# HansiZeng/scaling-retriever

Hardware: AMD Instinct MI355X
Metric: MSMARCO-Dev queries/sec end-to-end (query encode + dense brute-force top-1000) (higher is better)
Workload: dtype f32

## Files before the change

include/sr_hip.h:

```cpp
#ifndef SR_HIP_H
#define SR_HIP_H
#include <stdint.h>
#ifdef __cplusplus
extern "C" {
#endif

#define SR_OK 0
#define SR_ERR_INVALID 1
#define SR_ERR_HIP 2
#define SR_ERR_NOMEM 3
#define SR_ERR_UNSUPPORTED 4

#define SR_DTYPE_F32 0
#define SR_DTYPE_BF16 1
#define SR_DTYPE_F16 2

typedef void* sr_stream;

const char* sr_last_error(void);
int sr_version(void);
int sr_max_topk(void);

typedef struct sr_dense_index sr_dense_index;

int sr_dense_index_create(sr_dense_index** out, int dim);
int sr_dense_index_add(sr_dense_index* idx, const float* d_rows, int64_t n_rows,
                       int64_t id_base, int64_t id_stride);
int sr_dense_index_add_f16(sr_dense_index* idx, const void* d_rows_f16, int64_t n_rows,
                           int64_t id_base, int64_t id_stride);
int sr_dense_index_row_dtype(const sr_dense_index* idx);
int sr_dense_index_owned_bytes(sr_dense_index* idx, int64_t* out);
int64_t sr_dense_index_ntotal(const sr_dense_index* idx);
int sr_dense_search(sr_dense_index* idx, const float* d_queries, int64_t nq, int k,
                    float* d_out_scores, int64_t* d_out_ids, sr_stream stream);
#define SR_PRECISION_FP32 0
#define SR_PRECISION_BF16X3 1
#define SR_PRECISION_BF16X6 2
#define SR_PRECISION_FP32_FILTERED 3
int sr_dense_index_set_precision(sr_dense_index* idx, int mode);
int sr_dense_search_begin(sr_dense_index* idx, const float* d_queries, int64_t nq, int k, int share,
                          float* d_lower, sr_stream stream);
int sr_dense_search_finish(sr_dense_index* idx, const float* d_queries, int64_t nq, int k, const float* d_threshold,
                           float* d_out_scores, int64_t* d_out_ids, sr_stream stream);
int sr_dense_index_filter_stats(sr_dense_index* idx, int64_t* n_filtered, int64_t* n_fallback);
int sr_dense_index_filter_query_stats(sr_dense_index* idx, int64_t* n_certified, int64_t* n_redone);
int sr_dense_index_set_workspace_limit(sr_dense_index* idx, int64_t bytes);
int sr_dense_index_set_batch_invariant(sr_dense_index* idx, int on);
int sr_dense_score_pairs(sr_dense_index* idx, const float* d_queries, int64_t nq, const int64_t* d_cand_indptr,
                         const int64_t* d_cand_ids, float* d_out_scores, sr_stream stream);
int sr_dense_search_subset(sr_dense_index* idx, const float* d_queries, int64_t nq, int k,
                           const int64_t* d_subset, int64_t m,
                           float* d_out_scores, int64_t* d_out_ids, sr_stream stream);
int64_t sr_dense_index_id_end(const sr_dense_index* idx);
int sr_doc_mask_from_list(const int64_t* d_list, int64_t m, uint32_t* d_words, int64_t n_bits, sr_stream stream);
int sr_doc_list_from_mask(const uint32_t* d_words, int64_t n_bits, int64_t* d_list, int64_t capacity,
                          int64_t* d_count, sr_stream stream);
int sr_dense_search_masked(sr_dense_index* idx, const float* d_queries, int64_t nq, int k,
                           const uint32_t* d_mask_words, int64_t n_bits,
                           float* d_out_scores, int64_t* d_out_ids, sr_stream stream);
int sr_dense_range_count(sr_dense_index* idx, const float* d_queries, int64_t nq, const float* d_thresholds,
                         int64_t* d_lims, int64_t* total, sr_stream stream);
int sr_dense_range_fill(sr_dense_index* idx, const float* d_queries, int64_t nq, const float* d_thresholds,
                        const int64_t* d_lims, float* d_out_scores, int64_t* d_out_ids, int64_t capacity, sr_stream stream);
int sr_dense_index_destroy(sr_dense_index* idx);
int sr_dense_index_profile(sr_dense_index* idx, int enable);
int sr_dense_index_profile_read(sr_dense_index* idx, int64_t* n_launches, double* total_ms,
                                double* total_flop, double* total_d_bytes);

typedef struct sr_sparse_index sr_sparse_index;

int sr_sparse_index_create(sr_sparse_index** out, const int64_t* d_indptr,
                           const int32_t* d_doc_ids, const float* d_vals,
                           int64_t n_terms, int64_t n_docs, sr_stream stream);
int sr_sparse_search(sr_sparse_index* idx, const int64_t* d_q_indptr, const int32_t* d_q_cols,
                     const float* d_q_vals, int64_t nq, int k, float threshold,
                     int64_t id_base, int64_t id_stride,
                     float* d_out_scores, int64_t* d_out_ids, int32_t* d_out_counts,
                     sr_stream stream);
int sr_sparse_index_set_workspace_limit(sr_sparse_index* idx, int64_t bytes);
int sr_sparse_score_pairs(sr_sparse_index* idx, const int64_t* d_q_indptr, const int32_t* d_q_cols, const float* d_q_vals,
                          int64_t nq, const int64_t* d_cand_indptr, const int64_t* d_cand_ids, float* d_out_scores,
                          sr_stream stream);
int sr_sparse_search_subset(sr_sparse_index* idx, const int64_t* d_q_indptr, const int32_t* d_q_cols,
                            const float* d_q_vals, int64_t nq, int k, float threshold,
                            const int64_t* d_subset, int64_t m, int64_t id_base, int64_t id_stride,
                            float* d_out_scores, int64_t* d_out_ids, int32_t* d_out_counts, sr_stream stream);
int sr_sparse_search_masked(sr_sparse_index* idx, const int64_t* d_q_indptr, const int32_t* d_q_cols,
                            const float* d_q_vals, int64_t nq, int k, float threshold,
                            const uint32_t* d_mask_words, int64_t n_bits, int64_t id_base, int64_t id_stride,
                            float* d_out_scores, int64_t* d_out_ids, int32_t* d_out_counts, sr_stream stream);
int sr_sparse_range_count(sr_sparse_index* idx, const int64_t* d_q_indptr, const int32_t* d_q_cols, const float* d_q_vals,
                          int64_t nq, const float* d_thresholds, int64_t* d_lims, int64_t* total, sr_stream stream);
int sr_sparse_range_fill(sr_sparse_index* idx, const int64_t* d_q_indptr, const int32_t* d_q_cols, const float* d_q_vals,
                         int64_t nq, const float* d_thresholds, const int64_t* d_lims, int64_t id_base, int64_t id_stride,
                         float* d_out_scores, int64_t* d_out_ids, int64_t capacity, sr_stream stream);
int sr_sparse_index_destroy(sr_sparse_index* idx);
int sr_sparse_index_work_counters(sr_sparse_index* idx, int enable, uint64_t* out6);
int sr_sparse_index_profile(sr_sparse_index* idx, int enable);
int sr_sparse_index_profile_read(sr_sparse_index* idx, int64_t* n_launches, double* total_ms,
                                 double* total_posting_bytes);
int sr_sparse_index_block_stats(sr_sparse_index* idx, int64_t* n_dense_terms, int64_t* n_block_calls,
                                int64_t* n_fallback_calls);

int sr_sparse_index_cert_stats(sr_sparse_index* idx, int64_t* out8);
int sr_sparse_index_cert_debug(sr_sparse_index* idx, int enable, uint16_t* h_keys, int64_t keys_capacity,
                               float* h_consts, int64_t nq_pad, float* vscale, int32_t* T);

int sr_sparse_csr_expand_terms(const int64_t* d_indptr, int64_t n_terms, int64_t nnz, int32_t* d_out_terms,
                               sr_stream stream);
int sr_sparse_csr_build(const int32_t* d_rows, const int32_t* d_cols, const float* d_vals, int64_t nnz,
                        int64_t n_terms, int64_t n_docs, int sort_docs, int64_t* d_indptr,
                        int32_t* d_out_rows, float* d_out_vals, sr_stream stream);

int sr_topk_merge(const float* d_scores, const int64_t* d_ids, int n_lists, int64_t nq, int k,
                  float pad_score, float* d_out_scores, int64_t* d_out_ids, sr_stream stream);

typedef struct sr_model sr_model;

typedef struct {
    int32_t vocab_size, hidden_size, intermediate_size, num_layers;
    int32_t num_heads, num_kv_heads, head_dim;
    float rms_norm_eps;
    float rope_theta;
    int32_t rope_llama3;
    float rope_factor, rope_low_freq_factor, rope_high_freq_factor;
    int32_t rope_original_max_pos;
    int32_t tie_word_embeddings;
    int32_t has_lm_head;
    int32_t max_batch_tokens;
    int32_t max_batch_seqs;
    int32_t fp32_planes;
    int32_t attention_bias;
} sr_model_config;

int sr_model_create(sr_model** out, const sr_model_config* cfg);
int sr_model_set_weight(sr_model* m, const char* name, const void* d_ptr, int dtype,
                        int64_t rows, int64_t cols, sr_stream stream);
int sr_model_finalize(sr_model* m);
int sr_model_weight_segments(sr_model* m, int32_t* out, int64_t capacity, int64_t* n);
int sr_model_fused_act_layers(sr_model* m, int32_t* out, int64_t capacity, int64_t* n);
int sr_encode_dense(sr_model* m, const int64_t* d_input_ids, const int64_t* d_attention_mask,
                    int32_t B, int32_t L, float* d_out, sr_stream stream);
int sr_encode_sparse(sr_model* m, const int64_t* d_input_ids, const int64_t* d_attention_mask,
                     int32_t B, int32_t L, float* d_out, sr_stream stream);
int sr_encode_dense_fp32(sr_model* m, const int64_t* d_input_ids, const int64_t* d_attention_mask,
                         int32_t B, int32_t L, float* d_out, sr_stream stream);
int sr_encode_sparse_fp32(sr_model* m, const int64_t* d_input_ids, const int64_t* d_attention_mask,
                          int32_t B, int32_t L, float* d_out, sr_stream stream);
int sr_encode_both(sr_model* m, const int64_t* d_input_ids, const int64_t* d_attention_mask,
                   int32_t B, int32_t L, int32_t fp32, float* d_out_sparse, float* d_out_dense,
                   sr_stream stream);
int sr_encode_rows(sr_model* m, const int64_t* d_input_ids, const int64_t* d_attention_mask, int32_t B, int32_t L,
                   const int32_t* d_row_shift, int32_t mode, int32_t fp32, float* d_out_sparse, float* d_out_dense,
                   sr_stream stream);
int sr_model_last_hidden(sr_model* m, float* d_out, int64_t capacity_rows, int64_t* n_tokens, sr_stream stream);
int sr_model_destroy(sr_model* m);

int sr_lora_merge(float* d_W, const float* d_A, const float* d_B, int64_t out_features,
                  int64_t in_features, int32_t r, float scale, sr_stream stream);

int sr_sparse_compact(const float* d_reps, int64_t B, int64_t V, int64_t* d_row_ptr,
                      int32_t* d_cols, float* d_vals, int64_t capacity, int64_t* h_nnz,
                      sr_stream stream);
int sr_sparse_compact_topm(const float* d_reps, int64_t B, int64_t V, int64_t max_terms,
                           int64_t* d_row_ptr, int32_t* d_cols, float* d_vals,
                           int64_t capacity, int64_t* h_nnz, sr_stream stream);

int sr_write_run_json(const char* path, int64_t nq, int64_t k, const float* h_scores, const int64_t* h_idx, const int32_t* h_counts,
                      const int64_t* h_qid_i64, const char* h_qid_bytes, const int64_t* h_qid_off, int64_t qid_width,
                      const int64_t* h_doc_i64, const char* h_doc_bytes, const int64_t* h_doc_off, int64_t doc_width,
                      int64_t n_docs, int32_t n_threads, int64_t* bytes_written);
int sr_write_run_json_part(const char* path, int32_t part, int64_t nq, int64_t k, const float* h_scores, const int64_t* h_idx,
                           const int32_t* h_counts, const int64_t* h_qid_i64, const char* h_qid_bytes, const int64_t* h_qid_off,
                           int64_t qid_width, const int64_t* h_doc_i64, const char* h_doc_bytes, const int64_t* h_doc_off,
                           int64_t doc_width, int64_t n_docs, int32_t n_threads, int64_t* bytes_written);
int64_t sr_run_writer_mapped_rounds(void);

int sr_gemm_bf16(const void* d_A, const void* d_W, int32_t M, int32_t N, int32_t K, int32_t epilogue,
                 void* d_C, const int32_t* d_seq_of, sr_stream stream);
int sr_gemm_f16_scaled(const void* d_A, const void* d_W, int32_t M, int32_t N, int32_t K, const float* d_a_scale,
                       const float* d_w_scale, float* d_C, sr_stream stream);
int sr_rows_split_f16(float* d_src, const float* d_embed, const int32_t* d_tok_id, const float* d_norm_w, float eps,
                      int32_t T, int32_t K, int32_t nseg, void* d_planes, float* d_a_inv, const float* d_gu_cmax,
                      float* d_act_sc, float* d_act_inv, sr_stream stream);
int sr_gu_cmax_f16(const void* d_wgu_planes, const float* d_wgu_inv, int32_t I, int32_t K, int32_t nseg, float* d_cmax,
                   sr_stream stream);
int sr_gemm_f16_planes(const void* d_A, const void* d_W, int32_t M, int32_t N, int32_t K, int32_t epilogue, int32_t a_nseg,
                       const float* d_a_scale, const float* d_w_scale, void* d_C, const int32_t* d_pos,
                       const float* d_rope_cos, const float* d_rope_sin, int32_t n_rope, int32_t head_dim,
                       const float* d_bias, const int32_t* d_seq_of, const float* d_out_scale, int32_t out_nseg,
                       sr_stream stream);
int sr_gemm_qkv_rope(const void* d_A, const void* d_W, int32_t M, int32_t N, int32_t K, void* d_C,
                     const int32_t* d_pos, const float* d_rope_cos, const float* d_rope_sin,
                     int32_t n_rope, int32_t head_dim, sr_stream stream);
int sr_gemm_qkv_rope_bias(const void* d_A, const void* d_W, int32_t M, int32_t N, int32_t K, void* d_C,
                          const int32_t* d_pos, const float* d_rope_cos, const float* d_rope_sin,
                          int32_t n_rope, int32_t head_dim, const float* d_bias, int32_t fp32_out, sr_stream stream);
int sr_attention_varlen(const void* d_qkv, void* d_out, const int32_t* d_cu_seqlens, const int32_t* d_pos,
                        const uint8_t* d_key_valid, const float* d_rope_cos, const float* d_rope_sin,
                        int32_t B, int32_t num_heads, int32_t num_kv_heads, int32_t head_dim, sr_stream stream);
int sr_attention_varlen_f32(const float* d_qkv, float* d_out_f32, void* d_out_planes, int32_t fp32_planes,
                            const int32_t* d_cu_seqlens, const uint8_t* d_key_valid, int32_t B, int32_t num_heads,
                            int32_t num_kv_heads, int32_t head_dim, int32_t max_seqlen, sr_stream stream);
int sr_rmsnorm_bf16(float* d_x, const float* d_embed, const int32_t* d_tok_id, const void* d_delta, const float* d_norm_w,
                    void* d_xn, float* d_xn_f32, float eps, int32_t T, int32_t H, sr_stream stream);
int sr_dense_head_pool(const float* d_x, const float* d_norm_w, const int32_t* d_cu_seqlens, const int32_t* d_pos,
                       const int32_t* d_pool_start, float eps, int32_t B, int32_t T, int32_t H, void* d_stats, float* d_out,
                       sr_stream stream);
int sr_sparse_finish(float* d_out, int64_t n, float scale, int32_t round_bf16, sr_stream stream);
int sr_encode_plan(const int64_t* d_input_ids, const int64_t* d_attention_mask, int32_t B, int32_t L, int32_t mode, int32_t vocab,
                   const int32_t* d_row_shift, int32_t* d_span_start, int32_t* d_span_len, int32_t* d_pool_start,
                   int32_t* d_row_len, int32_t* d_cu_seqlens, int32_t* d_tok_id, int32_t* d_pos, uint8_t* d_key_valid,
                   int32_t* d_seq_of, int64_t capacity, int64_t* n_tokens, sr_stream stream);
int sr_split_bf16(const float* d_src, int64_t n, void* d_p0, void* d_p1, void* d_p2, sr_stream stream);

#ifdef __cplusplus
}
#endif
#endif
```

scaling_retriever_amd/_lib.py:

```python
import contextlib
import ctypes
import os
import threading

_HERE = os.path.dirname(os.path.abspath(__file__))
LIB_PATH = os.environ.get("SR_HIP_LIB") or os.path.join(_HERE, "libsr_hip.so")

SR_OK, SR_ERR_INVALID, SR_ERR_HIP, SR_ERR_NOMEM, SR_ERR_UNSUPPORTED = 0, 1, 2, 3, 4
SR_DTYPE_F32, SR_DTYPE_BF16, SR_DTYPE_F16 = 0, 1, 2

c_void_p, c_int, c_int32, c_int64, c_float, c_char_p = (ctypes.c_void_p, ctypes.c_int, ctypes.c_int32,
                                                         ctypes.c_int64, ctypes.c_float, ctypes.c_char_p)


class SrModelConfig(ctypes.Structure):
    _fields_ = [
        ("vocab_size", c_int32), ("hidden_size", c_int32), ("intermediate_size", c_int32), ("num_layers", c_int32),
        ("num_heads", c_int32), ("num_kv_heads", c_int32), ("head_dim", c_int32),
        ("rms_norm_eps", c_float), ("rope_theta", c_float), ("rope_llama3", c_int32),
        ("rope_factor", c_float), ("rope_low_freq_factor", c_float), ("rope_high_freq_factor", c_float),
        ("rope_original_max_pos", c_int32), ("tie_word_embeddings", c_int32), ("has_lm_head", c_int32),
        ("max_batch_tokens", c_int32), ("max_batch_seqs", c_int32), ("fp32_planes", c_int32),
        ("attention_bias", c_int32),
    ]


SIGNATURES = {
    "sr_last_error": (c_char_p, []),
    "sr_version": (c_int, []),
    "sr_max_topk": (c_int, []),
    "sr_dense_index_create": (c_int, [ctypes.POINTER(c_void_p), c_int]),
    "sr_dense_index_add": (c_int, [c_void_p, c_void_p, c_int64, c_int64, c_int64]),
    "sr_dense_index_add_f16": (c_int, [c_void_p, c_void_p, c_int64, c_int64, c_int64]),
    "sr_dense_index_row_dtype": (c_int, [c_void_p]),
    "sr_dense_index_owned_bytes": (c_int, [c_void_p, ctypes.POINTER(c_int64)]),
    "sr_dense_index_ntotal": (c_int64, [c_void_p]),
    "sr_dense_search": (c_int, [c_void_p, c_void_p, c_int64, c_int, c_void_p, c_void_p, c_void_p]),
    "sr_dense_index_set_workspace_limit": (c_int, [c_void_p, c_int64]),
    "sr_dense_index_set_batch_invariant": (c_int, [c_void_p, c_int]),
    "sr_dense_score_pairs": (c_int, [c_void_p, c_void_p, c_int64, c_void_p, c_void_p, c_void_p, c_void_p]),
    "sr_dense_search_subset": (c_int, [c_void_p, c_void_p, c_int64, c_int, c_void_p, c_int64, c_void_p, c_void_p, c_void_p]),
    "sr_dense_index_id_end": (c_int64, [c_void_p]),
    "sr_doc_mask_from_list": (c_int, [c_void_p, c_int64, c_void_p, c_int64, c_void_p]),
    "sr_doc_list_from_mask": (c_int, [c_void_p, c_int64, c_void_p, c_int64, c_void_p, c_void_p]),
    "sr_dense_search_masked": (c_int, [c_void_p, c_void_p, c_int64, c_int, c_void_p, c_int64, c_void_p, c_void_p, c_void_p]),
    "sr_dense_range_count": (c_int, [c_void_p, c_void_p, c_int64, c_void_p, c_void_p, ctypes.POINTER(c_int64), c_void_p]),
    "sr_dense_range_fill": (c_int, [c_void_p, c_void_p, c_int64, c_void_p, c_void_p, c_void_p, c_void_p, c_int64, c_void_p]),
    "sr_dense_index_set_precision": (c_int, [c_void_p, c_int]),
    "sr_dense_search_begin": (c_int, [c_void_p, c_void_p, c_int64, c_int, c_int, c_void_p, c_void_p]),
    "sr_dense_search_finish": (c_int, [c_void_p, c_void_p, c_int64, c_int, c_void_p, c_void_p, c_void_p, c_void_p]),
    "sr_dense_index_filter_stats": (c_int, [c_void_p, ctypes.POINTER(c_int64), ctypes.POINTER(c_int64)]),
    "sr_dense_index_filter_query_stats": (c_int, [c_void_p, ctypes.POINTER(c_int64), ctypes.POINTER(c_int64)]),
    "sr_dense_index_destroy": (c_int, [c_void_p]),
    "sr_dense_index_profile": (c_int, [c_void_p, c_int]),
    "sr_dense_index_profile_read": (c_int, [c_void_p, ctypes.POINTER(c_int64), ctypes.POINTER(ctypes.c_double),
                                            ctypes.POINTER(ctypes.c_double), ctypes.POINTER(ctypes.c_double)]),
    "sr_sparse_index_work_counters": (c_int, [c_void_p, c_int, ctypes.POINTER(ctypes.c_uint64)]),
    "sr_sparse_index_profile": (c_int, [c_void_p, c_int]),
    "sr_sparse_index_profile_read": (c_int, [c_void_p, ctypes.POINTER(c_int64), ctypes.POINTER(ctypes.c_double),
                                             ctypes.POINTER(ctypes.c_double)]),
    "sr_sparse_index_create": (c_int, [ctypes.POINTER(c_void_p), c_void_p, c_void_p, c_void_p, c_int64, c_int64,
                                       c_void_p]),
    "sr_sparse_search": (c_int, [c_void_p, c_void_p, c_void_p, c_void_p, c_int64, c_int, c_float, c_int64, c_int64,
                                 c_void_p, c_void_p, c_void_p, c_void_p]),
    "sr_sparse_index_set_workspace_limit": (c_int, [c_void_p, c_int64]),
    "sr_sparse_score_pairs": (c_int, [c_void_p, c_void_p, c_void_p, c_void_p, c_int64, c_void_p, c_void_p, c_void_p, c_void_p]),
    "sr_sparse_search_subset": (c_int, [c_void_p, c_void_p, c_void_p, c_void_p, c_int64, c_int, c_float, c_void_p, c_int64, c_int64,
                                        c_int64, c_void_p, c_void_p, c_void_p, c_void_p]),
    "sr_sparse_search_masked": (c_int, [c_void_p, c_void_p, c_void_p, c_void_p, c_int64, c_int, c_float, c_void_p, c_int64, c_int64,
                                        c_int64, c_void_p, c_void_p, c_void_p, c_void_p]),
    "sr_sparse_range_count": (c_int, [c_void_p, c_void_p, c_void_p, c_void_p, c_int64, c_void_p, c_void_p, ctypes.POINTER(c_int64), c_void_p]),
    "sr_sparse_range_fill": (c_int, [c_void_p, c_void_p, c_void_p, c_void_p, c_int64, c_void_p, c_void_p, c_int64, c_int64, c_void_p,
                                     c_void_p, c_int64, c_void_p]),
    "sr_sparse_index_block_stats": (c_int, [c_void_p, ctypes.POINTER(c_int64), ctypes.POINTER(c_int64),
                                            ctypes.POINTER(c_int64)]),
    "sr_sparse_index_destroy": (c_int, [c_void_p]),
    "sr_sparse_index_cert_stats": (c_int, [c_void_p, ctypes.POINTER(c_int64)]),
    "sr_sparse_index_cert_debug": (c_int, [c_void_p, c_int, c_void_p, c_int64, c_void_p, c_int64,
                                           ctypes.POINTER(c_float), ctypes.POINTER(ctypes.c_int32)]),
    "sr_sparse_csr_expand_terms": (c_int, [c_void_p, c_int64, c_int64, c_void_p, c_void_p]),
    "sr_sparse_csr_build": (c_int, [c_void_p, c_void_p, c_void_p, c_int64, c_int64, c_int64, c_int, c_void_p, c_void_p,
                                    c_void_p, c_void_p]),
    "sr_topk_merge": (c_int, [c_void_p, c_void_p, c_int, c_int64, c_int, c_float, c_void_p, c_void_p, c_void_p]),
    "sr_model_create": (c_int, [ctypes.POINTER(c_void_p), ctypes.POINTER(SrModelConfig)]),
    "sr_model_set_weight": (c_int, [c_void_p, c_char_p, c_void_p, c_int, c_int64, c_int64, c_void_p]),
    "sr_model_finalize": (c_int, [c_void_p]),
    "sr_model_weight_segments": (c_int, [c_void_p, ctypes.POINTER(ctypes.c_int32), c_int64, ctypes.POINTER(c_int64)]),
    "sr_model_fused_act_layers": (c_int, [c_void_p, ctypes.POINTER(ctypes.c_int32), c_int64, ctypes.POINTER(c_int64)]),
    "sr_encode_dense": (c_int, [c_void_p, c_void_p, c_void_p, c_int32, c_int32, c_void_p, c_void_p]),
    "sr_encode_sparse": (c_int, [c_void_p, c_void_p, c_void_p, c_int32, c_int32, c_void_p, c_void_p]),
    "sr_encode_dense_fp32": (c_int, [c_void_p, c_void_p, c_void_p, c_int32, c_int32, c_void_p, c_void_p]),
    "sr_encode_sparse_fp32": (c_int, [c_void_p, c_void_p, c_void_p, c_int32, c_int32, c_void_p, c_void_p]),
    "sr_encode_both": (c_int, [c_void_p, c_void_p, c_void_p, c_int32, c_int32, c_int32, c_void_p, c_void_p, c_void_p]),
    "sr_encode_rows": (c_int, [c_void_p, c_void_p, c_void_p, c_int32, c_int32, c_void_p, c_int32, c_int32, c_void_p, c_void_p, c_void_p]),
    "sr_model_last_hidden": (c_int, [c_void_p, c_void_p, c_int64, ctypes.POINTER(c_int64), c_void_p]),
    "sr_model_destroy": (c_int, [c_void_p]),
    "sr_lora_merge": (c_int, [c_void_p, c_void_p, c_void_p, c_int64, c_int64, c_int32, c_float, c_void_p]),
    "sr_run_writer_mapped_rounds": (c_int64, []),
    "sr_write_run_json": (c_int, [c_char_p, c_int64, c_int64, c_void_p, c_void_p, c_void_p, c_void_p, c_void_p, c_void_p, c_int64,
                                  c_void_p, c_void_p, c_void_p, c_int64, c_int64, c_int32, ctypes.POINTER(c_int64)]),
    "sr_write_run_json_part": (c_int, [c_char_p, c_int32, c_int64, c_int64, c_void_p, c_void_p, c_void_p, c_void_p, c_void_p, c_void_p, c_int64,
                                       c_void_p, c_void_p, c_void_p, c_int64, c_int64, c_int32, ctypes.POINTER(c_int64)]),
    "sr_gemm_bf16": (c_int, [c_void_p, c_void_p, c_int32, c_int32, c_int32, c_int32, c_void_p, c_void_p, c_void_p]),
    "sr_gemm_f16_scaled": (c_int, [c_void_p, c_void_p, c_int32, c_int32, c_int32, c_void_p, c_void_p, c_void_p, c_void_p]),
    "sr_rows_split_f16": (c_int, [c_void_p, c_void_p, c_void_p, c_void_p, c_float, c_int32, c_int32, c_int32, c_void_p, c_void_p, c_void_p,
                                  c_void_p, c_void_p, c_void_p]),
    "sr_gu_cmax_f16": (c_int, [c_void_p, c_void_p, c_int32, c_int32, c_int32, c_void_p, c_void_p]),
    "sr_gemm_f16_planes": (c_int, [c_void_p, c_void_p, c_int32, c_int32, c_int32, c_int32, c_int32, c_void_p, c_void_p, c_void_p, c_void_p,
                                   c_void_p, c_void_p, c_int32, c_int32, c_void_p, c_void_p, c_void_p, c_int32, c_void_p]),
    "sr_rmsnorm_bf16": (c_int, [c_void_p, c_void_p, c_void_p, c_void_p, c_void_p, c_void_p, c_void_p, c_float, c_int32, c_int32, c_void_p]),
    "sr_dense_head_pool": (c_int, [c_void_p, c_void_p, c_void_p, c_void_p, c_void_p, c_float, c_int32, c_int32, c_int32, c_void_p, c_void_p,
                                   c_void_p]),
    "sr_sparse_finish": (c_int, [c_void_p, c_int64, c_float, c_int32, c_void_p]),
    "sr_encode_plan": (c_int, [c_void_p, c_void_p, c_int32, c_int32, c_int32, c_int32, c_void_p, c_void_p, c_void_p, c_void_p, c_void_p,
                               c_void_p, c_void_p, c_void_p, c_void_p, c_void_p, c_int64, ctypes.POINTER(c_int64), c_void_p]),
    "sr_split_bf16": (c_int, [c_void_p, c_int64, c_void_p, c_void_p, c_void_p, c_void_p]),
    "sr_gemm_qkv_rope": (c_int, [c_void_p, c_void_p, c_int32, c_int32, c_int32, c_void_p, c_void_p, c_void_p, c_void_p,
                                 c_int32, c_int32, c_void_p]),
    "sr_gemm_qkv_rope_bias": (c_int, [c_void_p, c_void_p, c_int32, c_int32, c_int32, c_void_p, c_void_p, c_void_p, c_void_p,
                                      c_int32, c_int32, c_void_p, c_int32, c_void_p]),
    "sr_attention_varlen": (c_int, [c_void_p, c_void_p, c_void_p, c_void_p, c_void_p, c_void_p, c_void_p, c_int32,
                                    c_int32, c_int32, c_int32, c_void_p]),
    "sr_attention_varlen_f32": (c_int, [c_void_p, c_void_p, c_void_p, c_int32, c_void_p, c_void_p, c_int32, c_int32, c_int32,
                                        c_int32, c_int32, c_void_p]),
    "sr_sparse_compact": (c_int, [c_void_p, c_int64, c_int64, c_void_p, c_void_p, c_void_p, c_int64,
                                  ctypes.POINTER(c_int64), c_void_p]),
    "sr_sparse_compact_topm": (c_int, [c_void_p, c_int64, c_int64, c_int64, c_void_p, c_void_p, c_void_p, c_int64,
                                       ctypes.POINTER(c_int64), c_void_p]),
}

_lib = None
_lock = threading.Lock()


class SrHipError(RuntimeError):
    pass


def _bind(path):
    if not os.path.exists(path):
        raise SrHipError(
            f"{path} not found: the HIP extension is not built. There is no CPU fallback; "
            "run `make -C scaling_retriever_amd/csrc` (needs hipcc, targets gfx950).")
    import torch
    lib = ctypes.CDLL(path)
    for name, (res, args) in SIGNATURES.items():
        fn = getattr(lib, name)
        fn.restype = res
        fn.argtypes = args
    return lib


def load():
    global _lib
    with _lock:
        if _lib is None:
            _lib = _bind(LIB_PATH)
        return _lib


@contextlib.contextmanager
def library(path):
    global _lib
    other = _bind(os.path.abspath(path))
    with _lock:
        keep, _lib = _lib, other
    try:
        yield other
    finally:
        with _lock:
            _lib = keep


def check(rc, what=""):
    if rc == SR_OK:
        return
    msg = load().sr_last_error().decode("utf-8", "replace")
    if rc == SR_ERR_INVALID:
        raise ValueError(f"{what}: {msg}" if what else msg)
    if rc == SR_ERR_NOMEM:
        raise MemoryError(f"{what}: {msg}" if what else msg)
    raise SrHipError(f"{what}: [{rc}] {msg}" if what else f"[{rc}] {msg}")


def stream_ptr():
    import torch
    return ctypes.c_void_p(torch.cuda.current_stream().cuda_stream)


def require_gpu():
    import torch
    if not torch.cuda.is_available():
        raise SrHipError("no ROCm device visible: scaling_retriever_amd runs its hot path on MI355X only "
                         "(there is no CPU fallback)")
```

scaling_retriever_amd/csrc/api.hip:

```cpp
#include "kernels.h"
#include <stdlib.h>
#include <string>
#include <vector>

static thread_local std::string g_last_error;

void sr_set_error(const char* fmt, ...) {
    char buf[1024];
    va_list ap;
    va_start(ap, fmt);
    vsnprintf(buf, sizeof(buf), fmt, ap);
    va_end(ap);
    g_last_error = buf;
}

int sr_cu_count() {
    static int per_dev[SR_MAX_DEVICES] = {};
    int d = 0;
    if (hipGetDevice(&d) != hipSuccess || d < 0 || d >= SR_MAX_DEVICES) d = 0;
    if (per_dev[d] == 0) {
        int n = 0;
        if (hipDeviceGetAttribute(&n, hipDeviceAttributeMultiprocessorCount, d) != hipSuccess || n <= 0) { (void)hipGetLastError(); n = 256; }
        per_dev[d] = n;
    }
    return per_dev[d];
}

extern "C" const char* sr_last_error(void) { return g_last_error.c_str(); }
extern "C" int sr_version(void) { return 1; }
extern "C" int sr_max_topk(void) { return SR_MAX_TOPK; }

extern "C" int sr_gemm_bf16(const void* d_A, const void* d_W, int32_t M, int32_t N, int32_t K, int32_t epilogue, void* d_C,
                            const int32_t* d_seq_of, sr_stream stream) {
    SR_REQUIRE(d_A && d_W && d_C, "sr_gemm_bf16: null pointer");
    SR_REQUIRE(epilogue >= 0 && epilogue <= 4, "sr_gemm_bf16: unknown epilogue %d", epilogue);
    SR_REQUIRE(epilogue != EPI_SEGMAX || d_seq_of, "sr_gemm_bf16: epilogue 3 needs d_seq_of");
    GemmArgs g{};
    g.A = (const bf16_t*)d_A; g.W = (const bf16_t*)d_W; g.M = M; g.N = N; g.K = K; g.C = d_C; g.seq_of = d_seq_of; g.out_ld = N;
    if (epilogue != EPI_SEGMAX && d_seq_of && sr_dev_getenv("SR_GEMM_STAMPS")) {
        g.stamps = (unsigned long long*)d_seq_of;
        g.seq_of = nullptr;
    }
    return launch_gemm_bf16((GemmEpilogue)epilogue, g, (hipStream_t)stream);
}

extern "C" int sr_gemm_qkv_rope(const void* d_A, const void* d_W, int32_t M, int32_t N, int32_t K, void* d_C, const int32_t* d_pos,
                                const float* d_rope_cos, const float* d_rope_sin, int32_t n_rope, int32_t head_dim,
                                sr_stream stream) {
    SR_REQUIRE(d_A && d_W && d_C && d_pos && d_rope_cos && d_rope_sin, "sr_gemm_qkv_rope: null pointer");
    GemmArgs g{};
    g.A = (const bf16_t*)d_A; g.W = (const bf16_t*)d_W; g.M = M; g.N = N; g.K = K; g.C = d_C;
    g.pos = d_pos; g.rope_cos = d_rope_cos; g.rope_sin = d_rope_sin; g.n_rope = n_rope; g.head_dim = head_dim;
    return launch_gemm_bf16(EPI_QKV_ROPE, g, (hipStream_t)stream);
}

extern "C" int sr_gemm_qkv_rope_bias(const void* d_A, const void* d_W, int32_t M, int32_t N, int32_t K, void* d_C, const int32_t* d_pos,
                                     const float* d_rope_cos, const float* d_rope_sin, int32_t n_rope, int32_t head_dim,
                                     const float* d_bias, int32_t fp32_out, sr_stream stream) {
    SR_REQUIRE(d_A && d_W && d_C && d_pos && d_rope_cos && d_rope_sin, "sr_gemm_qkv_rope_bias: null pointer");
    SR_REQUIRE(fp32_out == 0 || fp32_out == 1, "sr_gemm_qkv_rope_bias: fp32_out must be 0 or 1");
    GemmArgs g{};
    g.A = (const bf16_t*)d_A; g.W = (const bf16_t*)d_W; g.M = M; g.N = N; g.K = K; g.C = d_C;
    g.pos = d_pos; g.rope_cos = d_rope_cos; g.rope_sin = d_rope_sin; g.n_rope = n_rope; g.head_dim = head_dim;
    g.bias = d_bias;
    return launch_gemm_bf16(fp32_out ? EPI_QKV_ROPE_F32 : EPI_QKV_ROPE, g, (hipStream_t)stream);
}

extern "C" int sr_attention_varlen(const void* d_qkv, void* d_out, const int32_t* d_cu_seqlens, const int32_t* d_pos,
                                   const uint8_t* d_key_valid, const float* d_rope_cos, const float* d_rope_sin, int32_t B,
                                   int32_t num_heads, int32_t num_kv_heads, int32_t head_dim, sr_stream stream) {
    SR_REQUIRE(d_qkv && d_out && d_cu_seqlens && d_key_valid, "sr_attention_varlen: null pointer");
    SR_REQUIRE((d_rope_cos == nullptr) == (d_rope_sin == nullptr), "sr_attention_varlen: pass both rope tables or neither");
    SR_REQUIRE(!d_rope_cos || d_pos, "sr_attention_varlen: rope tables need d_pos");
    SR_REQUIRE(B >= 0 && num_heads > 0 && num_kv_heads > 0, "sr_attention_varlen: bad sizes");
    AttnArgs a{};
    a.qkv = (const bf16_t*)d_qkv; a.out = (bf16_t*)d_out; a.cu_seqlens = d_cu_seqlens; a.pos = d_pos; a.key_valid = d_key_valid;
    a.rope_cos = d_rope_cos; a.rope_sin = d_rope_sin; a.B = B; a.nh = num_heads; a.nkv = num_kv_heads; a.hd = head_dim;
    a.scale = 1.0f / sqrtf((float)head_dim);
    a.apply_rope = d_rope_cos ? 1 : 0;
    a.max_seqlen = 0;
    if (!a.apply_rope && B > 0) {
        std::vector<int> cu((size_t)B + 1);
        SR_CHECK_HIP(hipMemcpyAsync(cu.data(), d_cu_seqlens, sizeof(int) * ((size_t)B + 1), hipMemcpyDeviceToHost, (hipStream_t)stream));
        SR_CHECK_HIP(hipStreamSynchronize((hipStream_t)stream));
        for (int b = 0; b < B; ++b) a.max_seqlen = cu[b + 1] - cu[b] > a.max_seqlen ? cu[b + 1] - cu[b] : a.max_seqlen;
    }
    return launch_attention(a, (hipStream_t)stream);
}

extern "C" int sr_attention_varlen_f32(const float* d_qkv, float* d_out_f32, void* d_out_planes, int32_t fp32_planes,
                                       const int32_t* d_cu_seqlens, const uint8_t* d_key_valid, int32_t B, int32_t num_heads,
                                       int32_t num_kv_heads, int32_t head_dim, int32_t max_seqlen, sr_stream stream) {
    SR_REQUIRE(d_qkv && d_cu_seqlens && d_key_valid, "sr_attention_varlen_f32: null pointer");
    SR_REQUIRE((d_out_f32 != nullptr) != (d_out_planes != nullptr), "sr_attention_varlen_f32: pass exactly one of d_out_f32 / d_out_planes");
    SR_REQUIRE(d_out_f32 || fp32_planes == 2 || fp32_planes == 3, "sr_attention_varlen_f32: fp32_planes %d (2 or 3 for plane output)", fp32_planes);
    SR_REQUIRE(B >= 0 && max_seqlen >= 0 && num_heads > 0 && num_kv_heads > 0 && head_dim > 0, "sr_attention_varlen_f32: bad sizes");
    SR_REQUIRE((uintptr_t)d_qkv % 16 == 0 && (uintptr_t)d_out_f32 % 16 == 0 && (uintptr_t)d_out_planes % 8 == 0,
               "sr_attention_varlen_f32: d_qkv and d_out_f32 must be 16-byte aligned, d_out_planes 8-byte aligned");
    AttnF32Args a{};
    a.qkv = d_qkv; a.out_f32 = d_out_f32; a.out = (bf16_t*)d_out_planes; a.cu_seqlens = d_cu_seqlens; a.key_valid = d_key_valid;
    a.B = B; a.nh = num_heads; a.nkv = num_kv_heads; a.hd = head_dim;
    a.scale = 1.0f / sqrtf((float)head_dim); a.max_seqlen = max_seqlen;
    if (!d_out_f32) a.out_map = split_map_a(fp32_planes);
    return launch_attention_f32(a, (hipStream_t)stream);
}

extern "C" int sr_gemm_f16_scaled(const void* d_A, const void* d_W, int32_t M, int32_t N, int32_t K, const float* d_a_scale,
                                  const float* d_w_scale, float* d_C, sr_stream stream) {
    SR_REQUIRE(d_A && d_W && d_C && d_a_scale && d_w_scale, "sr_gemm_f16_scaled: null pointer");
    GemmArgs g{};
    g.A = (const bf16_t*)d_A; g.W = (const bf16_t*)d_W; g.M = M; g.N = N; g.K = K; g.C = d_C; g.a_scale = d_a_scale; g.w_scale = d_w_scale;
    return launch_gemm_bf16(EPI_RESID_F32_H, g, (hipStream_t)stream);
}

extern "C" int sr_rows_split_f16(float* d_src, const float* d_embed, const int32_t* d_tok_id, const float* d_norm_w, float eps,
                                 int32_t T, int32_t K, int32_t nseg, void* d_planes, float* d_a_inv, const float* d_gu_cmax,
                                 float* d_act_sc, float* d_act_inv, sr_stream stream) {
    SR_REQUIRE(d_src && d_planes && d_a_inv, "sr_rows_split_f16: null pointer");
    SR_REQUIRE((d_embed == nullptr) == (d_tok_id == nullptr), "sr_rows_split_f16: pass both d_embed and d_tok_id or neither");
    SR_REQUIRE(!d_embed || d_norm_w, "sr_rows_split_f16: the embedding gather is part of the norm kernel and needs d_norm_w");
    SR_REQUIRE(!d_gu_cmax || (d_act_sc && d_act_inv), "sr_rows_split_f16: d_gu_cmax needs d_act_sc and d_act_inv");
    SR_REQUIRE(nseg == 2 || nseg == 3, "sr_rows_split_f16: nseg %d is not 2 or 3", nseg);
    SR_REQUIRE(T >= 0 && K > 0 && K % 4 == 0, "sr_rows_split_f16: bad sizes T=%d K=%d (K must be a multiple of 4)", T, K);
    SR_REQUIRE((uintptr_t)d_src % 16 == 0 && (uintptr_t)d_embed % 16 == 0 && (uintptr_t)d_norm_w % 16 == 0 && (uintptr_t)d_planes % 8 == 0,
               "sr_rows_split_f16: d_src, d_embed and d_norm_w must be 16-byte aligned, d_planes 8-byte aligned");
    if (T == 0) return SR_OK;
    return launch_rows_split_f16(d_src, d_embed, d_tok_id, d_norm_w, (bf16_t*)d_planes, d_a_inv, T, K, eps, nseg, d_gu_cmax, d_act_sc,
                                 d_act_inv, (hipStream_t)stream);
}

extern "C" int sr_gu_cmax_f16(const void* d_wgu_planes, const float* d_wgu_inv, int32_t I, int32_t K, int32_t nseg, float* d_cmax,
                              sr_stream stream) {
    SR_REQUIRE(d_wgu_planes && d_wgu_inv && d_cmax, "sr_gu_cmax_f16: null pointer");
    SR_REQUIRE(nseg == 2 || nseg == 3, "sr_gu_cmax_f16: nseg %d is not 2 or 3", nseg);
    SR_REQUIRE(I > 0 && I % 16 == 0 && K > 0, "sr_gu_cmax_f16: bad sizes I=%d K=%d (gate / up rows alternate in blocks of 16)", I, K);
    return launch_gu_cmax((const bf16_t*)d_wgu_planes, d_wgu_inv, I, K, nseg, d_cmax, (hipStream_t)stream);
}

extern "C" int sr_gemm_f16_planes(const void* d_A, const void* d_W, int32_t M, int32_t N, int32_t K, int32_t epilogue, int32_t a_nseg,
                                  const float* d_a_scale, const float* d_w_scale, void* d_C, const int32_t* d_pos,
                                  const float* d_rope_cos, const float* d_rope_sin, int32_t n_rope, int32_t head_dim,
                                  const float* d_bias, const int32_t* d_seq_of, const float* d_out_scale, int32_t out_nseg,
                                  sr_stream stream) {
    SR_REQUIRE(d_A && d_W && d_C && d_a_scale && d_w_scale, "sr_gemm_f16_planes: null pointer");
    SR_REQUIRE(epilogue == EPI_QKV_ROPE_F32_H || epilogue == EPI_RESID_F32_H || epilogue == EPI_SWIGLU_F32_H || epilogue == EPI_SEGMAX_H ||
                   epilogue == EPI_SWIGLU_SPLIT_H, "sr_gemm_f16_planes: unknown epilogue %d (9 .. 13)", epilogue);
    SR_REQUIRE(a_nseg == 2 || a_nseg == 3, "sr_gemm_f16_planes: a_nseg %d is not 2 or 3", a_nseg);
    SR_REQUIRE(M >= 0 && N > 0 && K > 0 && K % 64 == 0 && K % a_nseg == 0,
               "sr_gemm_f16_planes: bad shape M=%d N=%d K=%d (K = a_nseg x features, a multiple of 64)", M, N, K);
    SR_REQUIRE(epilogue != EPI_QKV_ROPE_F32_H || (d_pos && d_rope_cos && d_rope_sin), "sr_gemm_f16_planes: epilogue 9 needs d_pos and both rope tables");
    SR_REQUIRE(epilogue == EPI_QKV_ROPE_F32_H || !d_bias, "sr_gemm_f16_planes: only epilogue 9 takes a bias");
    SR_REQUIRE(epilogue != EPI_SEGMAX_H || d_seq_of, "sr_gemm_f16_planes: epilogue 12 needs d_seq_of");
    SR_REQUIRE(epilogue != EPI_SWIGLU_SPLIT_H || d_out_scale, "sr_gemm_f16_planes: epilogue 13 needs d_out_scale");
    SR_REQUIRE(epilogue != EPI_SWIGLU_SPLIT_H || out_nseg == 2 || out_nseg == 3, "sr_gemm_f16_planes: out_nseg %d is not 2 or 3", out_nseg);
    GemmArgs g{};
    g.A = (const bf16_t*)d_A; g.W = (const bf16_t*)d_W; g.M = M; g.N = N; g.K = K; g.a_nseg = a_nseg; g.C = d_C;
    g.a_scale = d_a_scale; g.w_scale = d_w_scale;
    if (epilogue == EPI_QKV_ROPE_F32_H) {
        g.pos = d_pos; g.rope_cos = d_rope_cos; g.rope_sin = d_rope_sin; g.n_rope = n_rope; g.head_dim = head_dim; g.bias = d_bias;
    }
    if (epilogue == EPI_SEGMAX_H) { g.seq_of = d_seq_of; g.out_ld = N; }
    if (epilogue == EPI_SWIGLU_SPLIT_H) { g.out_scale = d_out_scale; g.out_nseg = out_nseg; }
    return launch_gemm_bf16((GemmEpilogue)epilogue, g, (hipStream_t)stream);
}

extern "C" int sr_rmsnorm_bf16(float* d_x, const float* d_embed, const int32_t* d_tok_id, const void* d_delta, const float* d_norm_w,
                               void* d_xn, float* d_xn_f32, float eps, int32_t T, int32_t H, sr_stream stream) {
    SR_REQUIRE(d_x, "sr_rmsnorm_bf16: null pointer");
    SR_REQUIRE((d_embed == nullptr) == (d_tok_id == nullptr), "sr_rmsnorm_bf16: pass both d_embed and d_tok_id or neither");
    SR_REQUIRE(d_norm_w || (!d_xn && !d_xn_f32), "sr_rmsnorm_bf16: an output needs d_norm_w (without it the call only adds the residual)");
    SR_REQUIRE(T >= 0 && H > 0 && H % 4 == 0, "sr_rmsnorm_bf16: bad sizes T=%d H=%d (H must be a multiple of 4)", T, H);
    SR_REQUIRE((uintptr_t)d_x % 16 == 0 && (uintptr_t)d_embed % 16 == 0 && (uintptr_t)d_norm_w % 16 == 0 && (uintptr_t)d_xn_f32 % 16 == 0 &&
                   (uintptr_t)d_delta % 8 == 0 && (uintptr_t)d_xn % 8 == 0,
               "sr_rmsnorm_bf16: d_x, d_embed, d_norm_w and d_xn_f32 must be 16-byte aligned, d_delta and d_xn 8-byte aligned");
    return launch_rmsnorm(d_x, d_embed, d_tok_id, (const bf16_t*)d_delta, d_norm_w, (bf16_t*)d_xn, d_xn_f32, T, H, eps, (hipStream_t)stream);
}

extern "C" int sr_dense_head_pool(const float* d_x, const float* d_norm_w, const int32_t* d_cu_seqlens, const int32_t* d_pos,
                                  const int32_t* d_pool_start, float eps, int32_t B, int32_t T, int32_t H, void* d_stats, float* d_out,
                                  sr_stream stream) {
    SR_REQUIRE(d_x && d_norm_w && d_cu_seqlens && d_pos && d_pool_start && d_stats && d_out, "sr_dense_head_pool: null pointer");
    SR_REQUIRE(B >= 0 && T >= 0 && H > 0 && H % 4 == 0, "sr_dense_head_pool: bad sizes B=%d T=%d H=%d (H must be a multiple of 4)", B, T, H);
    SR_REQUIRE((uintptr_t)d_x % 16 == 0 && (uintptr_t)d_norm_w % 16 == 0 && (uintptr_t)d_stats % 8 == 0,
               "sr_dense_head_pool: d_x and d_norm_w must be 16-byte aligned, d_stats 8-byte aligned");
    if (B == 0) return SR_OK;
    if (T == 0) {
        SR_CHECK_HIP(hipMemsetAsync(d_out, 0, (size_t)B * H * 4, (hipStream_t)stream));
        return SR_OK;
    }
    return launch_dense_head(d_x, d_norm_w, (float2*)d_stats, d_cu_seqlens, d_pos, d_pool_start, d_out, B, T, H, eps, (hipStream_t)stream);
}

extern "C" int sr_sparse_finish(float* d_out, int64_t n, float scale, int32_t round_bf16, sr_stream stream) {
    SR_REQUIRE(d_out, "sr_sparse_finish: null pointer");
    SR_REQUIRE(n >= 0 && n < ((int64_t)1 << 39), "sr_sparse_finish: bad size n=%lld", (long long)n);
    SR_REQUIRE(round_bf16 == 0 || round_bf16 == 1, "sr_sparse_finish: round_bf16 must be 0 or 1");
    if (n == 0) return SR_OK;
    return launch_sparse_finish(d_out, n, scale, round_bf16, (hipStream_t)stream);
}

extern "C" int sr_encode_plan(const int64_t* d_input_ids, const int64_t* d_attention_mask, int32_t B, int32_t L, int32_t mode, int32_t vocab,
                              const int32_t* d_row_shift, int32_t* d_span_start, int32_t* d_span_len, int32_t* d_pool_start,
                              int32_t* d_row_len, int32_t* d_cu_seqlens, int32_t* d_tok_id, int32_t* d_pos, uint8_t* d_key_valid,
                              int32_t* d_seq_of, int64_t capacity, int64_t* n_tokens, sr_stream stream) {
    SR_REQUIRE(d_input_ids && d_attention_mask && d_span_start && d_span_len && d_pool_start && d_row_len && d_cu_seqlens && n_tokens,
               "sr_encode_plan: null pointer");
    SR_REQUIRE(capacity >= 0 && (capacity == 0 || (d_tok_id && d_pos && d_key_valid && d_seq_of)), "sr_encode_plan: null token array");
    SR_REQUIRE(mode >= 0 && mode <= 2, "sr_encode_plan: mode %d (0 dense, 1 sparse, 2 both)", mode);
    SR_REQUIRE(B >= 1 && B <= 65536 && L >= 1 && vocab >= 1 && (int64_t)B * L < ((int64_t)1 << 31),
               "sr_encode_plan: bad sizes B=%d L=%d vocab=%d", B, L, vocab);
    hipStream_t s = (hipStream_t)stream;
    SR_TRY(launch_plan_rows(d_attention_mask, B, L, mode, d_span_start, d_span_len, d_pool_start, d_row_len, d_row_shift, d_cu_seqlens, s));
    int T = 0;
    SR_CHECK_HIP(hipMemcpyAsync(&T, d_cu_seqlens + B, 4, hipMemcpyDeviceToHost, s));
    SR_CHECK_HIP(hipStreamSynchronize(s));
    *n_tokens = T;
    SR_REQUIRE(T <= capacity, "sr_encode_plan: the batch packs to %d tokens, the token arrays hold %lld", T, (long long)capacity);
    if (T == 0) return SR_OK;
    return launch_plan_tokens(d_input_ids, d_attention_mask, B, L, d_span_start, d_cu_seqlens, d_tok_id, d_pos, d_key_valid, d_seq_of, vocab,
                              mode, d_row_shift, s);
}
```

scaling_retriever_amd/csrc/attention_f32.hip:

```cpp
#include "kernels.h"
#include <math.h>

#define AF_KC 64
#define AF_RPW 4
#define AF_ROWS 16

__device__ inline float af_mul_rn(float a, float b) {
#pragma clang fp contract(off)
    return a * b;
}

template <int HD>
__global__ __launch_bounds__(256) void attention_f32_kernel(AttnF32Args a) {
    constexpr int DPL = HD / 64;
    __shared__ float Ks[AF_KC][HD + 1];
    __shared__ float qs[AF_ROWS][HD];
    __shared__ float ps[AF_ROWS][AF_KC];
    __shared__ unsigned char kval[AF_KC];
    const int b = blockIdx.x, h = blockIdx.y;
    const int tid = threadIdx.x, lane = tid & 63, wave = tid >> 6;
    const int t0 = a.cu_seqlens[b];
    const int S = a.cu_seqlens[b + 1] - t0;
    const int r0 = blockIdx.z * AF_ROWS;
    if (r0 >= S || S <= a.only_gt) return;
    const int G = a.nh / a.nkv, kvh = h / G;
    const int ld = (a.nh + 2 * a.nkv) * HD;
    const int koff = a.nh * HD + kvh * HD, voff = (a.nh + a.nkv) * HD + kvh * HD;
    const int nrows = (S - r0) < AF_ROWS ? (S - r0) : AF_ROWS;

    for (int i = tid; i < nrows * HD; i += 256) {
        const int r = i / HD, d = i % HD;
        qs[r][d] = a.qkv[(int64_t)(t0 + r0 + r) * ld + h * HD + d];
    }
    float m[AF_RPW], l[AF_RPW], o[AF_RPW][DPL];
#pragma unroll
    for (int r = 0; r < AF_RPW; ++r) {
        m[r] = -INFINITY;
        l[r] = 0.f;
#pragma unroll
        for (int e = 0; e < DPL; ++e) o[r][e] = 0.f;
    }
    for (int k0 = 0; k0 < S; k0 += AF_KC) {
        const int nk = (S - k0) < AF_KC ? (S - k0) : AF_KC;
        __syncthreads();
        for (int i = tid; i < nk * HD; i += 256) {
            const int k = i / HD, d = i % HD;
            Ks[k][d] = a.qkv[(int64_t)(t0 + k0 + k) * ld + koff + d];
        }
        if (tid < AF_KC) kval[tid] = (tid < nk) ? a.key_valid[t0 + k0 + tid] : 0;
        __syncthreads();
        const bool valid = kval[lane] != 0;
#pragma unroll
        for (int r = 0; r < AF_RPW; ++r) {
            const int row = wave * AF_RPW + r;
            if (row >= nrows) break;
            float s = 0.f;
            for (int d = 0; d < HD; ++d) s = fmaf(qs[row][d], Ks[lane][d], s);
            s = valid ? s * a.scale : -INFINITY;
            float mx = s;
            for (int off = 32; off > 0; off >>= 1) mx = fmaxf(mx, __shfl_xor(mx, off));
            if (mx == -INFINITY) continue;
            const float m_new = fmaxf(m[r], mx);
            const float corr = expf(m[r] - m_new);
            const float p = valid ? expf(s - m_new) : 0.f;
            float sum = p;
            for (int off = 32; off > 0; off >>= 1) sum += __shfl_xor(sum, off);
            l[r] = fmaf(l[r], corr, sum);
            m[r] = m_new;
            ps[row][lane] = p;
            __builtin_amdgcn_wave_barrier();
            float acc[DPL];
#pragma unroll
            for (int e = 0; e < DPL; ++e) acc[e] = 0.f;
            for (int k = 0; k < nk; ++k) {
                const float pk = ps[row][k];
                const float* vrow = a.qkv + (int64_t)(t0 + k0 + k) * ld + voff;
#pragma unroll
                for (int e = 0; e < DPL; ++e) acc[e] = fmaf(pk, vrow[lane + 64 * e], acc[e]);
            }
#pragma unroll
            for (int e = 0; e < DPL; ++e) o[r][e] = fmaf(o[r][e], corr, acc[e]);
        }
    }
    const int64_t ldo = (int64_t)a.out_map.n_seg * a.nh * HD;
#pragma unroll
    for (int r = 0; r < AF_RPW; ++r) {
        const int row = wave * AF_RPW + r;
        if (row >= nrows) break;
        const float inv = l[r] > 0.f ? 1.0f / l[r] : 0.f;
        if (a.out_f32) {
#pragma unroll
            for (int e = 0; e < DPL; ++e) a.out_f32[(int64_t)(t0 + r0 + row) * a.nh * HD + h * HD + lane + 64 * e] = af_mul_rn(o[r][e], inv);
            continue;
        }
        bf16_t* orow = a.out + (int64_t)(t0 + r0 + row) * ldo;
#pragma unroll
        for (int e = 0; e < DPL; ++e) {
            unsigned short p[3];
            split_bf16x3(af_mul_rn(o[r][e], inv), p[0], p[1], p[2]);
            const int col = h * HD + lane + 64 * e;
            for (int sg = 0; sg < a.out_map.n_seg; ++sg) orow[(int64_t)sg * a.nh * HD + col] = p[a.out_map.plane[sg]];
        }
    }
}

template <int HD, int G>
__global__ __launch_bounds__(64 * G) void attention_f32_gqa_kernel(AttnF32Args a) {
    constexpr int DPL = HD / 64;
    constexpr bool V_LDS = HD <= 64;
    __shared__ float Ks[AF_KC][HD + 1];
    __shared__ float Vs[V_LDS ? AF_KC : 1][V_LDS ? HD : 1];
    __shared__ float qs[G][HD];
    __shared__ float ps[G][AF_KC];
    __shared__ unsigned char kval[AF_KC];
    const int b = blockIdx.x, kvh = blockIdx.y;
    const int tid = threadIdx.x, lane = tid & 63, wave = tid >> 6;
    const int h = kvh * G + wave;
    const int t0 = a.cu_seqlens[b];
    const int S = a.cu_seqlens[b + 1] - t0;
    const int r0 = blockIdx.z * AF_ROWS;
    if (r0 >= S || S <= a.only_gt) return;
    const int ld = (a.nh + 2 * a.nkv) * HD;
    const int koff = a.nh * HD + kvh * HD, voff = (a.nh + a.nkv) * HD + kvh * HD;
    const int nrows = (S - r0) < AF_ROWS ? (S - r0) : AF_ROWS;
    const int64_t ldo = (int64_t)a.out_map.n_seg * a.nh * HD;
    for (int rq = 0; rq < nrows; rq += AF_RPW) {
        float m[AF_RPW], l[AF_RPW], o[AF_RPW][DPL];
#pragma unroll
        for (int r = 0; r < AF_RPW; ++r) {
            m[r] = -INFINITY;
            l[r] = 0.f;
#pragma unroll
            for (int e = 0; e < DPL; ++e) o[r][e] = 0.f;
        }
        for (int k0 = 0; k0 < S; k0 += AF_KC) {
            const int nk = (S - k0) < AF_KC ? (S - k0) : AF_KC;
            __syncthreads();
            for (int i = tid; i < nk * HD; i += 64 * G) {
                const int k = i / HD, d = i % HD;
                Ks[k][d] = a.qkv[(int64_t)(t0 + k0 + k) * ld + koff + d];
                if constexpr (V_LDS) Vs[k][d] = a.qkv[(int64_t)(t0 + k0 + k) * ld + voff + d];
            }
            if (tid < AF_KC) kval[tid] = (tid < nk) ? a.key_valid[t0 + k0 + tid] : 0;
            __syncthreads();
            const bool valid = kval[lane] != 0;
#pragma unroll
            for (int r = 0; r < AF_RPW; ++r) {
                const int row = rq + r;
                if (row >= nrows) break;
#pragma unroll
                for (int e = 0; e < DPL; ++e) qs[wave][lane + 64 * e] = a.qkv[(int64_t)(t0 + r0 + row) * ld + h * HD + lane + 64 * e];
                __builtin_amdgcn_wave_barrier();
                float s = 0.f;
                for (int d = 0; d < HD; ++d) s = fmaf(qs[wave][d], Ks[lane][d], s);
                s = valid ? s * a.scale : -INFINITY;
                float mx = s;
                for (int off = 32; off > 0; off >>= 1) mx = fmaxf(mx, __shfl_xor(mx, off));
                if (mx == -INFINITY) continue;
                const float m_new = fmaxf(m[r], mx);
                const float corr = expf(m[r] - m_new);
                const float p = valid ? expf(s - m_new) : 0.f;
                float sum = p;
                for (int off = 32; off > 0; off >>= 1) sum += __shfl_xor(sum, off);
                l[r] = fmaf(l[r], corr, sum);
                m[r] = m_new;
                ps[wave][lane] = p;
                __builtin_amdgcn_wave_barrier();
                float acc[DPL];
#pragma unroll
                for (int e = 0; e < DPL; ++e) acc[e] = 0.f;
                for (int k = 0; k < nk; ++k) {
                    const float pk = ps[wave][k];
                    if constexpr (V_LDS) {
                        acc[0] = fmaf(pk, Vs[k][lane], acc[0]);
                    } else {
                        const float* vrow = a.qkv + (int64_t)(t0 + k0 + k) * ld + voff;
#pragma unroll
                        for (int e = 0; e < DPL; ++e) acc[e] = fmaf(pk, vrow[lane + 64 * e], acc[e]);
                    }
                }
#pragma unroll
                for (int e = 0; e < DPL; ++e) o[r][e] = fmaf(o[r][e], corr, acc[e]);
            }
        }
#pragma unroll
        for (int r = 0; r < AF_RPW; ++r) {
            const int row = rq + r;
            if (row >= nrows) break;
            const float inv = l[r] > 0.f ? 1.0f / l[r] : 0.f;
            if (a.out_f32) {
#pragma unroll
                for (int e = 0; e < DPL; ++e) a.out_f32[(int64_t)(t0 + r0 + row) * a.nh * HD + h * HD + lane + 64 * e] = af_mul_rn(o[r][e], inv);
                continue;
            }
            bf16_t* orow = a.out + (int64_t)(t0 + r0 + row) * ldo;
#pragma unroll
            for (int e = 0; e < DPL; ++e) {
                unsigned short p[3];
                split_bf16x3(af_mul_rn(o[r][e], inv), p[0], p[1], p[2]);
                const int col = h * HD + lane + 64 * e;
                for (int sg = 0; sg < a.out_map.n_seg; ++sg) orow[(int64_t)sg * a.nh * HD + col] = p[a.out_map.plane[sg]];
            }
        }
    }
}


__device__ __forceinline__ void af_swap32(float& vdst, float& src) {
    const auto r = __builtin_amdgcn_permlane32_swap(__float_as_uint(vdst), __float_as_uint(src), false, false);
    vdst = __uint_as_float(r[0]);
    src = __uint_as_float(r[1]);
}
__device__ __forceinline__ void af_swap16(float& vdst, float& src) {
    const auto r = __builtin_amdgcn_permlane16_swap(__float_as_uint(vdst), __float_as_uint(src), false, false);
    vdst = __uint_as_float(r[0]);
    src = __uint_as_float(r[1]);
}
__device__ __forceinline__ void af_transpose_groups(f32x4& x) {
    float x0 = x[0], x1 = x[1], x2 = x[2], x3 = x[3];
    af_swap32(x0, x2);
    af_swap32(x1, x3);
    af_swap16(x0, x1);
    af_swap16(x2, x3);
    x = f32x4{x0, x1, x2, x3};
}
__device__ __forceinline__ float af_quad_xor(float v, int sel) {
    return sel == 0x4E ? __int_as_float(__builtin_amdgcn_mov_dpp(__float_as_int(v), 0x4E, 0xF, 0xF, true))
                       : __int_as_float(__builtin_amdgcn_mov_dpp(__float_as_int(v), 0xB1, 0xF, 0xF, true));
}
__device__ __forceinline__ void af_transpose_quad(f32x4& x, int i) {
    float x0 = x[0], x1 = x[1], x2 = x[2], x3 = x[3];
    const bool hi2 = (i & 2) != 0, hi1 = (i & 1) != 0;
    const float r0 = af_quad_xor(hi2 ? x0 : x2, 0x4E), r1 = af_quad_xor(hi2 ? x1 : x3, 0x4E);
    if (hi2) { x0 = r0; x1 = r1; } else { x2 = r0; x3 = r1; }
    const float s0 = af_quad_xor(hi1 ? x0 : x1, 0xB1), s1 = af_quad_xor(hi1 ? x2 : x3, 0xB1);
    if (hi1) { x0 = s0; x2 = s1; } else { x1 = s0; x3 = s1; }
    x = f32x4{x0, x1, x2, x3};
}

__host__ __device__ constexpr int af_mfma_waves(int hd, int nkb) {
    return nkb == 0 ? 1 : (hd == 64 ? (nkb == 1 ? 8 : 6) : (nkb <= 2 ? 5 : 4));
}

template <int HD, int NKB>
__global__ __launch_bounds__(256, af_mfma_waves(HD, NKB)) void attention_f32_mfma_kernel(AttnF32Args a) {
    constexpr int LDK = HD + 1, CB = HD / 16;
    constexpr bool OLD = NKB == 0;
    constexpr int MKB = OLD ? 4 : NKB;
    extern __shared__ float af_smem[];
    const int b = blockIdx.x, kvh = blockIdx.y;
    const int tid = threadIdx.x, lane = tid & 63, wave = tid >> 6;
    const int t0 = a.cu_seqlens[b];
    const int S = a.cu_seqlens[b + 1] - t0;
    if (S <= 0 || S > a.only_le) return;
    const int nkb = (S + 15) >> 4;
    if (!OLD && (a.nkb_only ? nkb != a.nkb_only : nkb > NKB)) return;
    const int SP = nkb * 16;
    float* Ks = af_smem;
    float* Vs = Ks + SP * LDK;
    const int G = a.nh / a.nkv;
    const int h = kvh * G + wave;
    const int ld = (a.nh + 2 * a.nkv) * HD;
    const int koff = a.nh * HD + kvh * HD, voff = (a.nh + a.nkv) * HD + kvh * HD;
    const int g = lane >> 4, c = lane & 15;
    f32x4 qv[CB];
    auto load_q = [&](int qb) {
#pragma unroll
        for (int i = 0; i < CB; ++i) {
            qv[i] = f32x4{0.f, 0.f, 0.f, 0.f};
            if (16 * qb + c < S) qv[i] = *reinterpret_cast<const f32x4*>(a.qkv + (int64_t)(t0 + 16 * qb + c) * ld + h * HD + 16 * i + 4 * g);
        }
    };
    if constexpr (OLD) {
        for (int i = tid; i < SP * (HD / 4); i += 256) {
            const int k = i / (HD / 4), d = (i % (HD / 4)) * 4;
            f32x4 kv = {0.f, 0.f, 0.f, 0.f}, vv = {0.f, 0.f, 0.f, 0.f};
            if (k < S) {
                kv = *reinterpret_cast<const f32x4*>(a.qkv + (int64_t)(t0 + k) * ld + koff + d);
                vv = *reinterpret_cast<const f32x4*>(a.qkv + (int64_t)(t0 + k) * ld + voff + d);
            }
#pragma unroll
            for (int e = 0; e < 4; ++e) { Ks[k * LDK + d + e] = kv[e]; Vs[k * LDK + d + e] = vv[e]; }
        }
    }
    constexpr int NIT = OLD ? 1 : NKB * HD / 64;
    constexpr int CHMAX = HD == 64 ? 4 : 2, CH = NIT > CHMAX ? CHMAX : NIT;
    unsigned vmask = 0;
    auto load_vmask = [&]() {
#pragma unroll
        for (int kb = 0; kb < MKB; ++kb)
#pragma unroll
            for (int r = 0; r < 4; ++r) {
                const int key = 16 * kb + 4 * g + r;
                if (key < S && a.key_valid[t0 + key]) vmask |= 1u << (4 * kb + r);
            }
    };
    if constexpr (OLD) {
        load_vmask();
    } else {
#pragma unroll
        for (int it0 = 0; it0 < NIT; it0 += CH) {
            f32x4 kreg[CH], vreg[CH];
#pragma unroll
            for (int it = 0; it < CH; ++it) {
                const int i = tid + 256 * (it0 + it), k = i / (HD / 4), d = (i % (HD / 4)) * 4;
                kreg[it] = f32x4{0.f, 0.f, 0.f, 0.f};
                vreg[it] = f32x4{0.f, 0.f, 0.f, 0.f};
                if (k < S) {
                    kreg[it] = *reinterpret_cast<const f32x4*>(a.qkv + (int64_t)(t0 + k) * ld + koff + d);
                    vreg[it] = *reinterpret_cast<const f32x4*>(a.qkv + (int64_t)(t0 + k) * ld + voff + d);
                }
            }
            if (it0 == 0) {
                load_q(0);
                load_vmask();
            }
#pragma unroll
            for (int it = 0; it < CH; ++it) {
                const int i = tid + 256 * (it0 + it), k = i / (HD / 4), d = (i % (HD / 4)) * 4;
                if (k < SP) {
#pragma unroll
                    for (int e = 0; e < 4; ++e) { Ks[k * LDK + d + e] = kreg[it][e]; Vs[k * LDK + d + e] = vreg[it][e]; }
                }
            }
            if (it0 + CH < NIT) __builtin_amdgcn_sched_barrier(0);
        }
    }
    __syncthreads();
    const int64_t ldo = (int64_t)a.out_map.n_seg * a.nh * HD;
    for (int qb = 0; qb < nkb; ++qb) {
        f32x4 st[MKB];
        if constexpr (OLD) {
            float* Qs = Vs + SP * LDK + wave * 16 * LDK;
            for (int i = lane; i < 16 * (HD / 4); i += 64) {
                const int r = i / (HD / 4), d = (i % (HD / 4)) * 4;
                f32x4 qr = {0.f, 0.f, 0.f, 0.f};
                if (16 * qb + r < S) qr = *reinterpret_cast<const f32x4*>(a.qkv + (int64_t)(t0 + 16 * qb + r) * ld + h * HD + d);
#pragma unroll
                for (int e = 0; e < 4; ++e) Qs[r * LDK + d + e] = qr[e];
            }
            __builtin_amdgcn_fence(__ATOMIC_ACQ_REL, "wavefront");
#pragma unroll
            for (int i = 0; i < CB; ++i)
#pragma unroll
                for (int k = 0; k < 4; ++k) qv[i][k] = Qs[c * LDK + 16 * i + 4 * k + g];
        } else {
            if (HD != 64 && qb > 0) load_q(qb);
#pragma unroll
            for (int i = 0; i < CB; ++i) af_transpose_groups(qv[i]);
        }
#pragma unroll
        for (int kb = 0; kb < MKB; ++kb) {
            st[kb] = f32x4{0.f, 0.f, 0.f, 0.f};
            if (kb < nkb) {
#pragma unroll
                for (int kk = 0; kk < HD / 4; ++kk)
                    st[kb] = __builtin_amdgcn_mfma_f32_16x16x4f32(Ks[(16 * kb + c) * LDK + 4 * kk + g], qv[kk >> 2][kk & 3], st[kb], 0, 0, 0);
            }
        }
        if constexpr (!OLD) {
            __builtin_amdgcn_sched_barrier(0);
            if (HD == 64 && qb + 1 < nkb) load_q(qb + 1);
        }
        float m = -INFINITY;
#pragma unroll
        for (int kb = 0; kb < MKB; ++kb)
#pragma unroll
            for (int r = 0; r < 4; ++r) {
                const bool v = (vmask >> (4 * kb + r)) & 1;
                st[kb][r] = v ? st[kb][r] * a.scale : -INFINITY;
                m = fmaxf(m, st[kb][r]);
            }
        m = fmaxf(m, __shfl_xor(m, 16));
        m = fmaxf(m, __shfl_xor(m, 32));
        float sum = 0.f;
#pragma unroll
        for (int kb = 0; kb < MKB; ++kb)
#pragma unroll
            for (int r = 0; r < 4; ++r) {
                const float p = (m > -INFINITY && st[kb][r] > -INFINITY) ? expf(st[kb][r] - m) : 0.f;
                st[kb][r] = p;
                sum += p;
            }
        sum += __shfl_xor(sum, 16);
        sum += __shfl_xor(sum, 32);
        const float inv = sum > 0.f ? 1.0f / sum : 0.f;
#pragma unroll
        for (int kb = 0; kb < MKB; ++kb)
#pragma unroll
            for (int r = 0; r < 4; ++r) st[kb][r] *= inv;
        if constexpr (!OLD) __builtin_amdgcn_sched_barrier(0);
#pragma unroll
        for (int cb = 0; cb < CB; ++cb) {
            if (!OLD && cb == 4) __builtin_amdgcn_sched_barrier(0);
            f32x4 o = {0.f, 0.f, 0.f, 0.f};
#pragma unroll
            for (int kb = 0; kb < MKB; ++kb) {
                if (kb < nkb) {
#pragma unroll
                    for (int mm = 0; mm < 4; ++mm)
                        o = __builtin_amdgcn_mfma_f32_16x16x4f32(st[kb][mm], Vs[(16 * kb + 4 * g + mm) * LDK + 16 * cb + c], o, 0, 0, 0);
                }
            }
            if constexpr (OLD) {
#pragma unroll
                for (int r = 0; r < 4; ++r) {
                    const int row = 16 * qb + 4 * g + r;
                    if (row >= S) continue;
                    const int col = h * HD + 16 * cb + c;
                    if (a.out_f32) {
                        a.out_f32[(int64_t)(t0 + row) * a.nh * HD + col] = o[r];
                    } else {
                        unsigned short p[3];
                        split_bf16x3(o[r], p[0], p[1], p[2]);
                        bf16_t* orow = a.out + (int64_t)(t0 + row) * ldo;
                        for (int sg = 0; sg < a.out_map.n_seg; ++sg) orow[(int64_t)sg * a.nh * HD + col] = p[a.out_map.plane[sg]];
                    }
                }
            } else {
                af_transpose_quad(o, c & 3);
                const int row = 16 * qb + 4 * g + (c & 3);
                if (row >= S) continue;
                const int col = h * HD + 16 * cb + (c & 12);
                if (a.out_f32) {
                    *reinterpret_cast<f32x4*>(a.out_f32 + (int64_t)(t0 + row) * a.nh * HD + col) = o;
                } else {
                    unsigned short p[4][3];
#pragma unroll
                    for (int e = 0; e < 4; ++e) split_bf16x3(o[e], p[e][0], p[e][1], p[e][2]);
                    bf16_t* orow = a.out + (int64_t)(t0 + row) * ldo;
                    for (int sg = 0; sg < a.out_map.n_seg; ++sg) {
                        const int pl = a.out_map.plane[sg];
                        bf16x4 w;
#pragma unroll
                        for (int e = 0; e < 4; ++e) w[e] = (short)(pl == 0 ? p[e][0] : (pl == 1 ? p[e][1] : p[e][2]));
                        *reinterpret_cast<bf16x4*>(orow + (int64_t)sg * a.nh * HD + col) = w;
                    }
                }
            }
        }
    }
}

template <int HD, int NKB>
static int launch_attention_f32_mfma_cfg(const AttnF32Args& a, size_t lds, hipStream_t s) {
    static DeviceOnce attr_once;
    if (bool* slot = attr_once.pending()) {
        constexpr int max_sp = NKB ? 16 * NKB : 64;
        SR_CHECK_HIP(hipFuncSetAttribute(reinterpret_cast<const void*>(&attention_f32_mfma_kernel<HD, NKB>),
                                         hipFuncAttributeMaxDynamicSharedMemorySize, (int)(sizeof(float) * (2 * max_sp + (NKB ? 0 : 64)) * (HD + 1))));
        *slot = true;
    }
    const dim3 grid((unsigned)a.B, (unsigned)a.nkv), block(256);
    SR_REQUIRE(grid.y <= 65535, "attention(fp32): grid too large");
    hipLaunchKernelGGL((attention_f32_mfma_kernel<HD, NKB>), grid, block, lds, s, a);
    SR_CHECK_LAUNCH();
    return SR_OK;
}

template <int HD>
static int launch_attention_f32_mfma_class(const AttnF32Args& a, int nkb, hipStream_t s) {
    const size_t lds = sizeof(float) * (size_t)(2 * 16 * nkb) * (HD + 1);
    switch (nkb) {
        case 1: return launch_attention_f32_mfma_cfg<HD, 1>(a, lds, s);
        case 2: return launch_attention_f32_mfma_cfg<HD, 2>(a, lds, s);
        case 3: return launch_attention_f32_mfma_cfg<HD, 3>(a, lds, s);
        default: return launch_attention_f32_mfma_cfg<HD, 4>(a, lds, s);
    }
}

template <int HD>
static int launch_attention_f32_mfma(const AttnF32Args& a_in, hipStream_t s) {
    AttnF32Args a = a_in;
    const int top = (int)ceil_div64(a.max_seqlen < 64 ? a.max_seqlen : 64, 16);
    const char* env = sr_dev_getenv("SR_ATTN_F32_LAYOUT");
    if (env && *env == '0') {
        const size_t lds = sizeof(float) * (size_t)(2 * 16 * top + 4 * 16) * (HD + 1);
        return launch_attention_f32_mfma_cfg<HD, 0>(a, lds, s);
    }
    const bool force = env && *env == '2';
    if (!a.have_classes && !force) {
        a.nkb_only = 0;
        return launch_attention_f32_mfma_class<HD>(a, top, s);
    }
    for (int nkb = 1; nkb <= top; ++nkb) {
        if (a.have_classes && a.class_seqs[nkb - 1] == 0) continue;
        a.nkb_only = nkb;
        SR_TRY(launch_attention_f32_mfma_class<HD>(a, nkb, s));
    }
    return SR_OK;
}

int launch_attention_f32(const AttnF32Args& a_in, hipStream_t s) {
    AttnF32Args a = a_in;
    SR_REQUIRE(a.nh % a.nkv == 0, "attention(fp32): num_heads %d not a multiple of num_kv_heads %d", a.nh, a.nkv);
    SR_REQUIRE(a.out_f32 || (a.out_map.n_seg >= 1 && a.out_map.n_seg <= SR_MAX_SEG), "attention(fp32): bad segment map");
    if (a.B == 0 || a.max_seqlen <= 0) return SR_OK;
    const int G = a.nh / a.nkv;
    a.only_le = 0; a.only_gt = 0;
    const char* env_m = sr_dev_getenv("SR_ATTN_F32_MFMA");
    if (G == 4 && (a.hd == 64 || a.hd == 128) && !(env_m && *env_m == '0')) {
        a.only_le = 64;
        SR_TRY(a.hd == 64 ? launch_attention_f32_mfma<64>(a, s) : launch_attention_f32_mfma<128>(a, s));
        if (a.max_seqlen <= 64) return SR_OK;
        a.only_le = 0; a.only_gt = 64;
    }
    const char* env = sr_dev_getenv("SR_ATTN_F32_GQA");
    if (G == 4 && !(env && *env == '0')) {
        const dim3 grid((unsigned)a.B, (unsigned)a.nkv, (unsigned)ceil_div64(a.max_seqlen, AF_ROWS)), block(256);
        SR_REQUIRE(grid.y <= 65535 && grid.z <= 65535, "attention(fp32): grid too large");
        switch (a.hd) {
            case 64: hipLaunchKernelGGL((attention_f32_gqa_kernel<64, 4>), grid, block, 0, s, a); break;
            case 128: hipLaunchKernelGGL((attention_f32_gqa_kernel<128, 4>), grid, block, 0, s, a); break;
            default: sr_set_error("attention(fp32): head_dim %d not supported (64 or 128)", a.hd); return SR_ERR_UNSUPPORTED;
        }
        SR_CHECK_LAUNCH();
        return SR_OK;
    }
    const dim3 grid((unsigned)a.B, (unsigned)a.nh, (unsigned)ceil_div64(a.max_seqlen, AF_ROWS)), block(256);
    SR_REQUIRE(grid.y <= 65535 && grid.z <= 65535, "attention(fp32): grid too large");
    switch (a.hd) {
        case 64: hipLaunchKernelGGL(attention_f32_kernel<64>, grid, block, 0, s, a); break;
        case 128: hipLaunchKernelGGL(attention_f32_kernel<128>, grid, block, 0, s, a); break;
        default: sr_set_error("attention(fp32): head_dim %d not supported (64 or 128)", a.hd); return SR_ERR_UNSUPPORTED;
    }
    SR_CHECK_LAUNCH();
    return SR_OK;
}
```

scaling_retriever_amd/csrc/encoder.hip:

```cpp
#include "kernels.h"
#include <math.h>
#include <algorithm>
#include <mutex>
#include <string>
#include <vector>

__global__ void plan_rows_kernel(const int64_t* __restrict__ mask, int B, int L, int mode, int* __restrict__ span_start,
                                 int* __restrict__ span_len, int* __restrict__ pool_start, int* __restrict__ row_len,
                                 const int* __restrict__ row_shift) {
    const int b = blockIdx.x;
    const int lane = threadIdx.x;
    int len = 0, first = L, last = -1;
    for (int p = lane; p < L; p += 64) {
        if (mask[(int64_t)b * L + p] != 0) {
            ++len;
            first = p < first ? p : first;
            last = p > last ? p : last;
        }
    }
    for (int off = 32; off > 0; off >>= 1) {
        len += __shfl_xor(len, off);
        const int f = __shfl_xor(first, off), l = __shfl_xor(last, off);
        first = f < first ? f : first;
        last = l > last ? l : last;
    }
    if (lane == 0) {
        int st, ln, ps;
        if (len == 0) {
            st = 0; ln = 0; ps = 0;
        } else if (mode != 1) {
            ps = L - len;
            st = first < ps ? first : ps;
            ln = L - st;
        } else {
            ps = first;
            st = first;
            ln = last + 1 - first;
        }
        span_start[b] = st;
        span_len[b] = ln;
        pool_start[b] = ps - (row_shift ? row_shift[b] : 0);
        row_len[b] = len;
    }
}

__global__ void plan_scan_kernel(const int* __restrict__ span_len, int B, int* __restrict__ cu) {
    __shared__ int part[256];
    const int tid = threadIdx.x;
    const int per = (B + 255) / 256;
    const int b0 = tid * per, b1 = (b0 + per) < B ? (b0 + per) : B;
    int s = 0;
    for (int b = b0; b < b1; ++b) s += span_len[b];
    part[tid] = s;
    __syncthreads();
    if (tid == 0) {
        int run = 0;
        for (int i = 0; i < 256; ++i) { const int v = part[i]; part[i] = run; run += v; }
        cu[B] = run;
    }
    __syncthreads();
    int run = part[tid];
    for (int b = b0; b < b1; ++b) { cu[b] = run; run += span_len[b]; }
}

__global__ void plan_tokens_kernel(const int64_t* __restrict__ ids, const int64_t* __restrict__ mask, int L,
                                   const int* __restrict__ span_start, const int* __restrict__ cu, int* __restrict__ tok_id,
                                   int* __restrict__ pos, unsigned char* __restrict__ key_valid, int* __restrict__ seq_of,
                                   int vocab, int mode, const int* __restrict__ row_shift) {
    const int b = blockIdx.x;
    const int t0 = cu[b], n = cu[b + 1] - t0, st = span_start[b];
    const int shift = row_shift ? row_shift[b] : 0;
    for (int j = threadIdx.x; j < n; j += blockDim.x) {
        const int p = st + j;
        int64_t id = ids[(int64_t)b * L + p];
        id = id < 0 ? 0 : (id >= vocab ? vocab - 1 : id);
        tok_id[t0 + j] = (int)id;
        pos[t0 + j] = p - shift < 0 ? 0 : p - shift;
        const bool valid = mask[(int64_t)b * L + p] != 0;
        key_valid[t0 + j] = valid ? 1 : 0;
        seq_of[t0 + j] = (mode != 0 && !valid) ? -2 : b;
    }
}

int launch_plan_rows(const int64_t* mask, int B, int L, int mode, int* span_start, int* span_len, int* pool_start, int* row_len,
                     const int* row_shift, int* cu, hipStream_t s) {
    hipLaunchKernelGGL(plan_rows_kernel, dim3(B), dim3(64), 0, s, mask, B, L, mode, span_start, span_len, pool_start, row_len, row_shift);
    hipLaunchKernelGGL(plan_scan_kernel, dim3(1), dim3(256), 0, s, span_len, B, cu);
    SR_CHECK_LAUNCH();
    return SR_OK;
}
int launch_plan_tokens(const int64_t* ids, const int64_t* mask, int B, int L, const int* span_start, const int* cu, int* tok_id, int* pos,
                       unsigned char* key_valid, int* seq_of, int vocab, int mode, const int* row_shift, hipStream_t s) {
    hipLaunchKernelGGL(plan_tokens_kernel, dim3(B), dim3(128), 0, s, ids, mask, L, span_start, cu, tok_id, pos, key_valid, seq_of, vocab,
                       mode, row_shift);
    SR_CHECK_LAUNCH();
    return SR_OK;
}

template <int NCH>
__global__ __launch_bounds__(256) void rmsnorm_kernel(float* __restrict__ x, const float* __restrict__ embed,
                                                      const int* __restrict__ tok_id, const bf16_t* __restrict__ delta,
                                                      const float* __restrict__ w, bf16_t* __restrict__ xn,
                                                      float* __restrict__ xn_f32, int T, int H, float eps) {
    const int t = blockIdx.x * 4 + (threadIdx.x >> 6);
    const int lane = threadIdx.x & 63;
    if (t >= T) return;
    float* xr = x + (int64_t)t * H;
    const float* src = embed ? embed + (int64_t)tok_id[t] * H : xr;
    const bf16_t* dr = delta ? delta + (int64_t)t * H : nullptr;
    float ss = 0.f;
    if constexpr (NCH > 0) {
        f32x4 v[NCH];
#pragma unroll
        for (int c = 0; c < NCH; ++c) v[c] = *reinterpret_cast<const f32x4*>(src + lane * 4 + c * 256);
        if (dr) {
            bf16x4 d[NCH];
#pragma unroll
            for (int c = 0; c < NCH; ++c) d[c] = *reinterpret_cast<const bf16x4*>(dr + lane * 4 + c * 256);
#pragma unroll
            for (int c = 0; c < NCH; ++c)
#pragma unroll
                for (int e = 0; e < 4; ++e) v[c][e] += bf16_to_f32((unsigned short)d[c][e]);
        }
#pragma unroll
        for (int c = 0; c < NCH; ++c) {
            ss += v[c][0] * v[c][0] + v[c][1] * v[c][1] + v[c][2] * v[c][2] + v[c][3] * v[c][3];
            if (embed || dr) *reinterpret_cast<f32x4*>(xr + lane * 4 + c * 256) = v[c];
        }
        for (int off = 32; off > 0; off >>= 1) ss += __shfl_xor(ss, off);
        const float rs = 1.0f / sqrtf(ss / (float)H + eps);
        if (!w) return;
#pragma unroll
        for (int c = 0; c < NCH; ++c) {
            const int i = lane * 4 + c * 256;
            const f32x4 g = *reinterpret_cast<const f32x4*>(w + i);
            f32x4 y;
#pragma unroll
            for (int e = 0; e < 4; ++e) y[e] = (v[c][e] * rs) * g[e];
            if (xn) {
                bf16x4 o;
#pragma unroll
                for (int e = 0; e < 4; ++e) o[e] = (short)f32_to_bf16(y[e]);
                *reinterpret_cast<bf16x4*>(xn + (int64_t)t * H + i) = o;
            }
            if (xn_f32) *reinterpret_cast<f32x4*>(xn_f32 + (int64_t)t * H + i) = y;
        }
    } else {
        for (int i = lane * 4; i < H; i += 256) {
            f32x4 v = *reinterpret_cast<const f32x4*>(src + i);
            if (dr) {
                const bf16x4 d = *reinterpret_cast<const bf16x4*>(dr + i);
#pragma unroll
                for (int c = 0; c < 4; ++c) v[c] += bf16_to_f32((unsigned short)d[c]);
            }
            ss += v[0] * v[0] + v[1] * v[1] + v[2] * v[2] + v[3] * v[3];
            if (embed || dr) *reinterpret_cast<f32x4*>(xr + i) = v;
        }
        for (int off = 32; off > 0; off >>= 1) ss += __shfl_xor(ss, off);
        const float rs = 1.0f / sqrtf(ss / (float)H + eps);
        if (!w) return;
        for (int i = lane * 4; i < H; i += 256) {
            const f32x4 v = *reinterpret_cast<const f32x4*>(xr + i);
            const f32x4 g = *reinterpret_cast<const f32x4*>(w + i);
            f32x4 y;
#pragma unroll
            for (int c = 0; c < 4; ++c) y[c] = (v[c] * rs) * g[c];
            if (xn) {
                bf16x4 o;
#pragma unroll
                for (int c = 0; c < 4; ++c) o[c] = (short)f32_to_bf16(y[c]);
                *reinterpret_cast<bf16x4*>(xn + (int64_t)t * H + i) = o;
            }
            if (xn_f32) *reinterpret_cast<f32x4*>(xn_f32 + (int64_t)t * H + i) = y;
        }
    }
}

int launch_rmsnorm(float* x, const float* embed, const int* tok_id, const bf16_t* delta, const float* w, bf16_t* xn,
                   float* xn_f32, int T, int H, float eps, hipStream_t s) {
    if (T == 0) return SR_OK;
    const dim3 grid((unsigned)ceil_div64(T, 4)), block(256);
#define SR_RMS(NCH) hipLaunchKernelGGL(rmsnorm_kernel<NCH>, grid, block, 0, s, x, embed, tok_id, delta, w, xn, xn_f32, T, H, eps)
    switch (H) {
        case 256: SR_RMS(1); break;
        case 512: SR_RMS(2); break;
        case 1024: SR_RMS(4); break;
        case 2048: SR_RMS(8); break;
        case 3072: SR_RMS(12); break;
        case 4096: SR_RMS(16); break;
        default: SR_RMS(0); break;
    }
#undef SR_RMS
    SR_CHECK_LAUNCH();
    return SR_OK;
}

__global__ __launch_bounds__(256) void dense_head_stats_kernel(const float* __restrict__ x, const float* __restrict__ w,
                                                               float2* __restrict__ stats, int T, int H, float eps) {
    const int t = blockIdx.x * 4 + (threadIdx.x >> 6);
    const int lane = threadIdx.x & 63;
    if (t >= T) return;
    const float* xr = x + (int64_t)t * H;
    float ss = 0.f;
    for (int i = lane * 4; i < H; i += 256) {
        const f32x4 v = *reinterpret_cast<const f32x4*>(xr + i);
        ss += v[0] * v[0] + v[1] * v[1] + v[2] * v[2] + v[3] * v[3];
    }
    for (int off = 32; off > 0; off >>= 1) ss += __shfl_xor(ss, off);
    const float rs = 1.0f / sqrtf(ss / (float)H + eps);
    float s2 = 0.f;
    for (int i = lane * 4; i < H; i += 256) {
        const f32x4 v = *reinterpret_cast<const f32x4*>(xr + i);
        const f32x4 g = *reinterpret_cast<const f32x4*>(w + i);
#pragma unroll
        for (int c = 0; c < 4; ++c) { const float y = (v[c] * rs) * g[c]; s2 += y * y; }
    }
    for (int off = 32; off > 0; off >>= 1) s2 += __shfl_xor(s2, off);
    if (lane == 0) stats[t] = make_float2(rs, 1.0f / fmaxf(sqrtf(s2), 1e-12f));
}
__global__ __launch_bounds__(256) void dense_head_pool_kernel(const float* __restrict__ x, const float* __restrict__ w,
                                                              const float2* __restrict__ stats, const int* __restrict__ cu,
                                                              const int* __restrict__ pos, const int* __restrict__ pool_start,
                                                              float* __restrict__ out, int H) {
    const int b = blockIdx.x, c = blockIdx.y * 256 + threadIdx.x;
    if (c >= H) return;
    const int t0 = cu[b], n = cu[b + 1] - t0, ps = pool_start[b];
    const float wc = w[c];
    float acc = 0.f;
    int cnt = 0;
    for (int j = 0; j < n; ++j) {
        const int t = t0 + j;
        if (pos[t] < ps) continue;
        const float2 st = stats[t];
        acc += ((x[(int64_t)t * H + c] * st.x) * wc) * st.y;
        ++cnt;
    }
    out[(int64_t)b * H + c] = cnt > 0 ? acc / (float)cnt : 0.f;
}

__global__ void sparse_finish_kernel(float* __restrict__ out, int64_t n, float scale, int round_bf16) {
    const int64_t i = (int64_t)blockIdx.x * blockDim.x + threadIdx.x;
    if (i >= n) return;
    float v = out[i];
    if (round_bf16) v = bf16_to_f32(f32_to_bf16(v));
    v *= scale;
    out[i] = (float)log((double)(fmaxf(v, 0.f) + 1.0f));
}

int launch_dense_head(const float* x, const float* w, float2* stats, const int* cu, const int* pos, const int* pool_start, float* out,
                      int B, int T, int H, float eps, hipStream_t s) {
    hipLaunchKernelGGL(dense_head_stats_kernel, dim3((unsigned)ceil_div64(T, 4)), dim3(256), 0, s, x, w, stats, T, H, eps);
    hipLaunchKernelGGL(dense_head_pool_kernel, dim3((unsigned)B, (unsigned)ceil_div64(H, 256)), dim3(256), 0, s, x, w, stats, cu, pos,
                       pool_start, out, H);
    SR_CHECK_LAUNCH();
    return SR_OK;
}
int launch_sparse_finish(float* out, int64_t n, float scale, int round_bf16, hipStream_t s) {
    hipLaunchKernelGGL(sparse_finish_kernel, dim3((unsigned)ceil_div64(n, 256)), dim3(256), 0, s, out, n, scale, round_bf16);
    SR_CHECK_LAUNCH();
    return SR_OK;
}

__global__ void convert_rows_kernel(const void* __restrict__ src, int src_dtype, int64_t rows, int64_t cols,
                                    bf16_t* __restrict__ dst_bf16, float* __restrict__ dst_f32, int64_t dst_row_base,
                                    int interleave ) {
    const int64_t r = blockIdx.x;
    int64_t dr = r;
    if (interleave) dr = (r / 16) * 32 + (interleave == 2 ? 16 : 0) + (r % 16);
    dr += dst_row_base;
    for (int64_t c = threadIdx.x; c < cols; c += blockDim.x) {
        float v;
        if (src_dtype == SR_DTYPE_F32) v = reinterpret_cast<const float*>(src)[r * cols + c];
        else v = bf16_to_f32(reinterpret_cast<const bf16_t*>(src)[r * cols + c]);
        if (dst_bf16) dst_bf16[dr * cols + c] = f32_to_bf16(v);
        if (dst_f32) dst_f32[dr * cols + c] = v;
    }
}

__global__ void convert_bias_kernel(const void* __restrict__ src, int src_dtype, int64_t n, float* __restrict__ dst_f32,
                                    float* __restrict__ dst_bf16r) {
    const int64_t i = (int64_t)blockIdx.x * blockDim.x + threadIdx.x;
    if (i >= n) return;
    const float v = src_dtype == SR_DTYPE_F32 ? reinterpret_cast<const float*>(src)[i] : bf16_to_f32(reinterpret_cast<const bf16_t*>(src)[i]);
    dst_f32[i] = v;
    dst_bf16r[i] = bf16_to_f32(f32_to_bf16(v));
}

__global__ void convert_rows_split_kernel(const void* __restrict__ src, int src_dtype, int64_t rows, int64_t cols,
                                          bf16_t* __restrict__ dst, int64_t dst_row_base, int interleave, SplitMap map) {
    const int64_t r = blockIdx.x;
    int64_t dr = r;
    if (interleave) dr = (r / 16) * 32 + (interleave == 2 ? 16 : 0) + (r % 16);
    dr += dst_row_base;
    bf16_t* drow = dst + dr * cols * map.n_seg;
    for (int64_t c = threadIdx.x; c < cols; c += blockDim.x) {
        float v;
        if (src_dtype == SR_DTYPE_F32) v = reinterpret_cast<const float*>(src)[r * cols + c];
        else v = bf16_to_f32(reinterpret_cast<const bf16_t*>(src)[r * cols + c]);
        unsigned short p[3];
        split_bf16x3(v, p[0], p[1], p[2]);
        for (int sg = 0; sg < map.n_seg; ++sg) drow[(int64_t)sg * cols + c] = p[map.plane[sg]];
    }
}

__global__ __launch_bounds__(256) void rmsnorm_split_kernel(float* __restrict__ x, const float* __restrict__ embed,
                                                            const int* __restrict__ tok_id, const float* __restrict__ w,
                                                            bf16_t* __restrict__ xs, int T, int H, float eps, SplitMap map) {
    const int t = blockIdx.x * 4 + (threadIdx.x >> 6);
    const int lane = threadIdx.x & 63;
    if (t >= T) return;
    float* xr = x + (int64_t)t * H;
    const float* src = embed ? embed + (int64_t)tok_id[t] * H : xr;
    float ss = 0.f;
    for (int i = lane * 4; i < H; i += 256) {
        const f32x4 v = *reinterpret_cast<const f32x4*>(src + i);
        ss += v[0] * v[0] + v[1] * v[1] + v[2] * v[2] + v[3] * v[3];
        if (embed) *reinterpret_cast<f32x4*>(xr + i) = v;
    }
    for (int off = 32; off > 0; off >>= 1) ss += __shfl_xor(ss, off);
    const float rs = 1.0f / sqrtf(ss / (float)H + eps);
    bf16_t* orow = xs + (int64_t)t * H * map.n_seg;
    for (int i = lane * 4; i < H; i += 256) {
        const f32x4 v = *reinterpret_cast<const f32x4*>(src + i);
        const f32x4 g = *reinterpret_cast<const f32x4*>(w + i);
        bf16x4 pl[3];
#pragma unroll
        for (int c = 0; c < 4; ++c) {
            unsigned short a0, a1, a2;
            split_bf16x3((v[c] * rs) * g[c], a0, a1, a2);
            pl[0][c] = (short)a0; pl[1][c] = (short)a1; pl[2][c] = (short)a2;
        }
        for (int sg = 0; sg < map.n_seg; ++sg) {
            const int pi = map.plane[sg];
            *reinterpret_cast<bf16x4*>(orow + (int64_t)sg * H + i) = pi == 0 ? pl[0] : (pi == 1 ? pl[1] : pl[2]);
        }
    }
}

__global__ __launch_bounds__(256) void convert_rows_split_h_kernel(const void* __restrict__ src, int src_dtype, int64_t rows, int64_t cols,
                                                                   bf16_t* __restrict__ dst, float* __restrict__ w_inv,
                                                                   int64_t dst_row_base, int interleave, int* __restrict__ lo_nz) {
    __shared__ float red[4];
    const int64_t r = blockIdx.x;
    int64_t dr = r;
    if (interleave) dr = (r / 16) * 32 + (interleave == 2 ? 16 : 0) + (r % 16);
    dr += dst_row_base;
    auto at = [&](int64_t c) {
        return src_dtype == SR_DTYPE_F32 ? reinterpret_cast<const float*>(src)[r * cols + c]
                                         : bf16_to_f32(reinterpret_cast<const bf16_t*>(src)[r * cols + c]);
    };
    float mx = 0.f;
    for (int64_t c = threadIdx.x; c < cols; c += 256) mx = fmaxf(mx, fabsf(at(c)));
    for (int off = 32; off > 0; off >>= 1) mx = fmaxf(mx, __shfl_xor(mx, off));
    if ((threadIdx.x & 63) == 0) red[threadIdx.x >> 6] = mx;
    __syncthreads();
    mx = fmaxf(fmaxf(red[0], red[1]), fmaxf(red[2], red[3]));
    const float sc = row_scale_pow2(mx);
    if (threadIdx.x == 0) w_inv[dr] = 1.0f / sc;
    bf16_t* drow = dst + dr * cols * 3;
    bool nz = false;
    for (int64_t c = threadIdx.x; c < cols; c += 256) {
        unsigned short f0, f1;
        split_f16x2(at(c) * sc, f0, f1);
        drow[c] = f0; drow[cols + c] = f1; drow[2 * cols + c] = f0;
        nz |= (f1 & 0x7fff) != 0;
    }
    if (nz) *lo_nz = 1;
}

__global__ __launch_bounds__(256) void pack_rows_2seg_kernel(const bf16_t* __restrict__ src, bf16_t* __restrict__ dst, int64_t K) {
    const int64_t r = blockIdx.x;
    const uint4* s0 = reinterpret_cast<const uint4*>(src + r * 3 * K);
    uint4* d = reinterpret_cast<uint4*>(dst + r * 2 * K);
    const int64_t kv = K / 8;
    for (int64_t i = threadIdx.x; i < kv; i += 256) {
        const uint4 v = s0[i];
        d[i] = v;
        d[kv + i] = v;
    }
}

__global__ __launch_bounds__(256) void rows_split_h_kernel(float* __restrict__ x, const float* __restrict__ embed,
                                                           const int* __restrict__ tok_id, const float* __restrict__ w,
                                                           bf16_t* __restrict__ xs, float* __restrict__ a_inv, int T, int K, float eps,
                                                           const float* __restrict__ gu_cmax, float* __restrict__ act_sc,
                                                           float* __restrict__ act_inv, int nseg) {
    const int t = blockIdx.x * 4 + (threadIdx.x >> 6);
    const int lane = threadIdx.x & 63;
    if (t >= T) return;
    float* xr = x + (int64_t)t * K;
    const float* src = embed ? embed + (int64_t)tok_id[t] * K : xr;
    float rs = 1.f;
    if (w) {
        float ss = 0.f;
        for (int i = lane * 4; i < K; i += 256) {
            const f32x4 v = *reinterpret_cast<const f32x4*>(src + i);
            ss += v[0] * v[0] + v[1] * v[1] + v[2] * v[2] + v[3] * v[3];
            if (embed) *reinterpret_cast<f32x4*>(xr + i) = v;
        }
        for (int off = 32; off > 0; off >>= 1) ss += __shfl_xor(ss, off);
        rs = 1.0f / sqrtf(ss / (float)K + eps);
    }
    float mx = 0.f, s2 = 0.f;
    for (int i = lane * 4; i < K; i += 256) {
        const f32x4 v = *reinterpret_cast<const f32x4*>(src + i);
        f32x4 g = {1.f, 1.f, 1.f, 1.f};
        if (w) g = *reinterpret_cast<const f32x4*>(w + i);
#pragma unroll
        for (int c = 0; c < 4; ++c) {
            const float y = w ? (v[c] * rs) * g[c] : v[c];
            mx = fmaxf(mx, fabsf(y));
            s2 += y * y;
        }
    }
    for (int off = 32; off > 0; off >>= 1) mx = fmaxf(mx, __shfl_xor(mx, off));
    const float sc = row_scale_pow2(mx);
    if (lane == 0) a_inv[t] = 1.0f / sc;
    if (gu_cmax) {
        for (int off = 32; off > 0; off >>= 1) s2 += __shfl_xor(s2, off);
        const float osc = row_scale_pow2(s2 * *gu_cmax * 1.02f);
        if (lane == 0) { act_sc[t] = osc; act_inv[t] = 1.0f / osc; }
    }
    bf16_t* orow = xs + (int64_t)t * K * nseg;
    for (int i = lane * 4; i < K; i += 256) {
        const f32x4 v = *reinterpret_cast<const f32x4*>(src + i);
        f32x4 g = {1.f, 1.f, 1.f, 1.f};
        if (w) g = *reinterpret_cast<const f32x4*>(w + i);
        bf16x4 p0, p1;
#pragma unroll
        for (int c = 0; c < 4; ++c) {
            unsigned short f0, f1;
            split_f16x2((w ? (v[c] * rs) * g[c] : v[c]) * sc, f0, f1);
            p0[c] = (short)f0; p1[c] = (short)f1;
        }
        *reinterpret_cast<bf16x4*>(orow + i) = p1;
        *reinterpret_cast<bf16x4*>(orow + K + i) = p0;
        if (nseg == 3) *reinterpret_cast<bf16x4*>(orow + 2 * K + i) = p0;
    }
}

template <int NV>
__global__ __launch_bounds__(256) void rows_split_h_reg_kernel(float* __restrict__ x, const float* __restrict__ embed,
                                                               const int* __restrict__ tok_id, const float* __restrict__ w,
                                                               bf16_t* __restrict__ xs, float* __restrict__ a_inv, int T, float eps,
                                                               const float* __restrict__ gu_cmax, float* __restrict__ act_sc,
                                                               float* __restrict__ act_inv, int nseg) {
    constexpr int K = 256 * NV;
    const int t = blockIdx.x * 4 + (threadIdx.x >> 6);
    const int lane = threadIdx.x & 63;
    if (t >= T) return;
    float* xr = x + (int64_t)t * K;
    const float* src = embed ? embed + (int64_t)tok_id[t] * K : xr;
    f32x4 v[NV];
#pragma unroll
    for (int j = 0; j < NV; ++j) v[j] = *reinterpret_cast<const f32x4*>(src + lane * 4 + 256 * j);
    if (w) {
        float ss = 0.f;
#pragma unroll
        for (int j = 0; j < NV; ++j) {
            ss += v[j][0] * v[j][0] + v[j][1] * v[j][1] + v[j][2] * v[j][2] + v[j][3] * v[j][3];
            if (embed) *reinterpret_cast<f32x4*>(xr + lane * 4 + 256 * j) = v[j];
        }
        for (int off = 32; off > 0; off >>= 1) ss += __shfl_xor(ss, off);
        const float rs = 1.0f / sqrtf(ss / (float)K + eps);
#pragma unroll
        for (int j = 0; j < NV; ++j) {
            const f32x4 g = *reinterpret_cast<const f32x4*>(w + lane * 4 + 256 * j);
#pragma unroll
            for (int c = 0; c < 4; ++c) v[j][c] = (v[j][c] * rs) * g[c];
        }
    }
    float mx = 0.f;
#pragma unroll
    for (int j = 0; j < NV; ++j)
#pragma unroll
        for (int c = 0; c < 4; ++c) mx = fmaxf(mx, fabsf(v[j][c]));
    for (int off = 32; off > 0; off >>= 1) mx = fmaxf(mx, __shfl_xor(mx, off));
    const float sc = row_scale_pow2(mx);
    if (lane == 0) a_inv[t] = 1.0f / sc;
    if (gu_cmax) {
        float s2 = 0.f;
#pragma unroll
        for (int j = 0; j < NV; ++j) s2 += v[j][0] * v[j][0] + v[j][1] * v[j][1] + v[j][2] * v[j][2] + v[j][3] * v[j][3];
        for (int off = 32; off > 0; off >>= 1) s2 += __shfl_xor(s2, off);
        const float osc = row_scale_pow2(s2 * *gu_cmax * 1.02f);
        if (lane == 0) { act_sc[t] = osc; act_inv[t] = 1.0f / osc; }
    }
    bf16_t* orow = xs + (int64_t)t * K * nseg;
#pragma unroll
    for (int j = 0; j < NV; ++j) {
        bf16x4 p0, p1;
#pragma unroll
        for (int c = 0; c < 4; ++c) {
            unsigned short f0, f1;
            split_f16x2(v[j][c] * sc, f0, f1);
            p0[c] = (short)f0; p1[c] = (short)f1;
        }
        const int i = lane * 4 + 256 * j;
        *reinterpret_cast<bf16x4*>(orow + i) = p1;
        *reinterpret_cast<bf16x4*>(orow + K + i) = p0;
        if (nseg == 3) *reinterpret_cast<bf16x4*>(orow + 2 * K + i) = p0;
    }
}

static void launch_rows_split_h(float* x, const float* embed, const int* tok, const float* w, bf16_t* xs, float* inv, int T, int K,
                                float eps, int nseg, hipStream_t s, const float* gu_cmax = nullptr, float* act_sc = nullptr,
                                float* act_inv = nullptr) {
    const dim3 grid((unsigned)ceil_div64(T, 4)), block(256);
    switch (K) {
        case 2048: hipLaunchKernelGGL(rows_split_h_reg_kernel<8>, grid, block, 0, s, x, embed, tok, w, xs, inv, T, eps, gu_cmax, act_sc, act_inv, nseg); break;
        case 4096: hipLaunchKernelGGL(rows_split_h_reg_kernel<16>, grid, block, 0, s, x, embed, tok, w, xs, inv, T, eps, gu_cmax, act_sc, act_inv, nseg); break;
        case 8192: hipLaunchKernelGGL(rows_split_h_reg_kernel<32>, grid, block, 0, s, x, embed, tok, w, xs, inv, T, eps, gu_cmax, act_sc, act_inv, nseg); break;
        default: hipLaunchKernelGGL(rows_split_h_kernel, grid, block, 0, s, x, embed, tok, w, xs, inv, T, K, eps, gu_cmax, act_sc, act_inv, nseg);
    }
}

__global__ __launch_bounds__(256) void gu_cmax_kernel(const bf16_t* __restrict__ wgu_s, const float* __restrict__ wgu_i, int I, int K,
                                                      int nseg, float* __restrict__ cmax) {
    const int j = blockIdx.x * 4 + (threadIdx.x >> 6);
    const int lane = threadIdx.x & 63;
    if (j >= I) return;
    const int64_t rg = (int64_t)(j / 16) * 32 + (j % 16), ru = rg + 16;
    float n2[2];
#pragma unroll
    for (int h = 0; h < 2; ++h) {
        const bf16_t* row = wgu_s + (h ? ru : rg) * nseg * (int64_t)K;
        float ss = 0.f;
        for (int i = lane; i < K; i += 64) {
            const float v = (float)__builtin_bit_cast(_Float16, row[i]) +
                            (nseg == 3 ? (float)__builtin_bit_cast(_Float16, row[K + i]) : 0.f);
            ss += v * v;
        }
        for (int off = 32; off > 0; off >>= 1) ss += __shfl_xor(ss, off);
        const float inv = wgu_i[h ? ru : rg];
        n2[h] = ss * inv * inv;
    }
    if (lane == 0) atomicMax(reinterpret_cast<unsigned int*>(cmax), __float_as_uint(sqrtf(n2[0]) * sqrtf(n2[1]) * 1.001f));
}

int launch_gu_cmax(const bf16_t* wgu_s, const float* wgu_i, int I, int K, int nseg, float* cmax, hipStream_t s) {
    SR_CHECK_HIP(hipMemsetAsync(cmax, 0, 4, s));
    hipLaunchKernelGGL(gu_cmax_kernel, dim3((unsigned)ceil_div64(I, 4)), dim3(256), 0, s, wgu_s, wgu_i, I, K, nseg, cmax);
    SR_CHECK_LAUNCH();
    return SR_OK;
}

int launch_rows_split_f16(float* x, const float* embed, const int* tok, const float* w, bf16_t* xs, float* inv, int T, int K, float eps,
                          int nseg, const float* gu_cmax, float* act_sc, float* act_inv, hipStream_t s) {
    launch_rows_split_h(x, embed, tok, w, xs, inv, T, K, eps, nseg, s, gu_cmax, act_sc, act_inv);
    SR_CHECK_LAUNCH();
    return SR_OK;
}

__global__ void lora_merge_kernel(float* __restrict__ W, const float* __restrict__ A, const float* __restrict__ Bm,
                                  int64_t out_f, int64_t in_f, int r, float scale) {
    const int64_t o = blockIdx.y;
    const int64_t i = (int64_t)blockIdx.x * blockDim.x + threadIdx.x;
    if (i >= in_f) return;
    float acc = 0.f;
    for (int k = 0; k < r; ++k) acc += Bm[o * r + k] * A[(int64_t)k * in_f + i];
    W[o * in_f + i] += scale * acc;
}

__global__ __launch_bounds__(256) void nnz_count_kernel(const float* __restrict__ reps, int64_t V, int64_t* __restrict__ row_nnz) {
    __shared__ int red[4];
    const int64_t b = blockIdx.x;
    int c = 0;
    for (int64_t i = threadIdx.x; i < V; i += 256) c += reps[b * V + i] != 0.f ? 1 : 0;
    for (int off = 32; off > 0; off >>= 1) c += __shfl_xor(c, off);
    if ((threadIdx.x & 63) == 0) red[threadIdx.x >> 6] = c;
    __syncthreads();
    if (threadIdx.x == 0) row_nnz[b] = red[0] + red[1] + red[2] + red[3];
}
__global__ void nnz_scan_kernel(const int64_t* __restrict__ row_nnz, int64_t B, int64_t* __restrict__ row_ptr) {
    if (threadIdx.x == 0 && blockIdx.x == 0) {
        int64_t run = 0;
        for (int64_t b = 0; b < B; ++b) { row_ptr[b] = run; run += row_nnz[b]; }
        row_ptr[B] = run;
    }
}
__global__ __launch_bounds__(256) void nnz_fill_kernel(const float* __restrict__ reps, int64_t V, const int64_t* __restrict__ row_ptr,
                                                       int32_t* __restrict__ cols, float* __restrict__ vals, int64_t capacity) {
    __shared__ int wtot[4];
    __shared__ int64_t base;
    const int64_t b = blockIdx.x;
    const int tid = threadIdx.x, lane = tid & 63, wave = tid >> 6;
    if (tid == 0) base = row_ptr[b];
    __syncthreads();
    for (int64_t i0 = 0; i0 < V; i0 += 256) {
        const int64_t i = i0 + tid;
        const float v = i < V ? reps[b * V + i] : 0.f;
        const int nz = v != 0.f ? 1 : 0;
        int incl = nz;
        for (int off = 1; off < 64; off <<= 1) { const int o = __shfl_up(incl, off); if (lane >= off) incl += o; }
        if (lane == 63) wtot[wave] = incl;
        __syncthreads();
        int wb = 0, tot = 0;
        for (int w = 0; w < 4; ++w) { if (w < wave) wb += wtot[w]; tot += wtot[w]; }
        const int64_t p = base + wb + incl - nz;
        if (nz && p < capacity) { cols[p] = (int32_t)i; vals[p] = v; }
        __syncthreads();
        if (tid == 0) base += tot;
        __syncthreads();
    }
}

struct LayerW {
    bf16_t* wqkv = nullptr;
    bf16_t* wo = nullptr;
    bf16_t* wgu = nullptr;
    bf16_t* wdown = nullptr;
    float* ln1 = nullptr;
    float* ln2 = nullptr;
    unsigned have = 0;
    bf16_t *wqkv_s = nullptr, *wo_s = nullptr, *wgu_s = nullptr, *wdown_s = nullptr;
    float *wqkv_i = nullptr, *wo_i = nullptr, *wgu_i = nullptr, *wdown_i = nullptr;
    float* gu_cmax = nullptr;
    bool fused_act = true;
    int qkv_seg = 3, o_seg = 3, gu_seg = 3, down_seg = 3;
    float *bqkv = nullptr, *bqkv_r = nullptr;
    unsigned have_bias = 0;
};

struct sr_model {
    sr_model_config cfg;
    int Tm = 0, Bm = 0;
    int max_pos = 0;
    float* embed = nullptr;
    bf16_t* lm_head = nullptr;
    bf16_t* lm_head_s = nullptr;
    float* lm_head_i = nullptr;
    int lm_head_seg = 3;
    int* lo_nz = nullptr;
    float *attn_f = nullptr, *act_f = nullptr;
    float *xs_i = nullptr, *attn_i = nullptr, *act_i = nullptr;
    float* act_sc = nullptr;
    bf16_t* xs = nullptr;
    float* qkv_f = nullptr;
    bf16_t* attn_s = nullptr;
    bf16_t* act_s = nullptr;
    float* norm_w = nullptr;
    std::vector<LayerW> layers;
    bool have_embed = false, have_norm = false, have_lm_head = false, finalized = false;
    float* rope_cos = nullptr;
    float* rope_sin = nullptr;
    float* x = nullptr;
    bf16_t* xn = nullptr;
    bf16_t* qkv = nullptr;
    bf16_t* attn = nullptr;
    bf16_t* act = nullptr;
    bf16_t* delta = nullptr;
    int *span_start = nullptr, *span_len = nullptr, *pool_start = nullptr, *row_len = nullptr, *cu = nullptr;
    int *tok_id = nullptr, *pos = nullptr, *seq_of = nullptr;
    unsigned char* key_valid = nullptr;
    int* h_cu = nullptr;
    int last_T = 0;
    std::mutex mu;
    StreamOrder order;
};

static void model_free(sr_model* m) {
    auto F = [](void* p) { if (p) (void)hipFree(p); };
    F(m->embed); F(m->lm_head); F(m->norm_w); F(m->rope_cos); F(m->rope_sin);
    F(m->lm_head_s); F(m->xs); F(m->qkv_f); F(m->attn_s); F(m->act_s);
    F(m->lm_head_i); F(m->lo_nz); F(m->attn_f); F(m->act_f); F(m->xs_i); F(m->attn_i); F(m->act_i); F(m->act_sc);
    for (auto& l : m->layers) {
        F(l.wqkv); F(l.wo); F(l.wgu); F(l.wdown); F(l.ln1); F(l.ln2); F(l.wqkv_s); F(l.wo_s); F(l.wgu_s); F(l.wdown_s);
        F(l.wqkv_i); F(l.wo_i); F(l.wgu_i); F(l.wdown_i); F(l.gu_cmax); F(l.bqkv); F(l.bqkv_r);
    }
    F(m->x); F(m->xn); F(m->qkv); F(m->attn); F(m->act); F(m->delta);
    F(m->span_start); F(m->span_len); F(m->pool_start); F(m->row_len); F(m->cu);
    F(m->tok_id); F(m->pos); F(m->seq_of); F(m->key_valid);
    if (m->h_cu) (void)hipHostFree(m->h_cu);
}

#define SR_ALLOC(ptr, bytes)                                                                      \
    do {                                                                                          \
        const hipError_t e_ = hipMalloc((void**)&(ptr), (size_t)(bytes));                          \
        if (e_ != hipSuccess) {                                                                   \
            sr_set_error("sr_model_create: hipMalloc of %zu bytes failed: %s", (size_t)(bytes), hipGetErrorString(e_)); \
            model_free(m);                                                                        \
            delete m;                                                                             \
            return SR_ERR_NOMEM;                                                                  \
        }                                                                                         \
    } while (0)

static void rope_tables(const sr_model_config& c, int max_pos, std::vector<float>& cosv, std::vector<float>& sinv) {
    const int hd = c.head_dim, half = hd / 2;
    std::vector<float> inv(half);
    for (int i = 0; i < half; ++i) {
        double f = 1.0 / pow((double)c.rope_theta, (double)(2 * i) / (double)hd);
        if (c.rope_llama3) {
            const double factor = c.rope_factor, lo = c.rope_low_freq_factor, hi = c.rope_high_freq_factor;
            const double old = (double)c.rope_original_max_pos;
            const double low_wl = old / lo, high_wl = old / hi;
            const double wl = 2.0 * M_PI / f;
            const double f_l = wl > low_wl ? f / factor : f;
            if (!(wl < high_wl) && !(wl > low_wl)) {
                const double smooth = (old / wl - lo) / (hi - lo);
                f = (1.0 - smooth) * f_l / factor + smooth * f_l;
            } else {
                f = f_l;
            }
        }
        inv[i] = (float)f;
    }
    cosv.resize((size_t)max_pos * half);
    sinv.resize((size_t)max_pos * half);
    for (int p = 0; p < max_pos; ++p)
        for (int i = 0; i < half; ++i) {
            const float ang = (float)p * inv[i];
            cosv[(size_t)p * half + i] = (float)cos((double)ang);
            sinv[(size_t)p * half + i] = (float)sin((double)ang);
        }
}

extern "C" int sr_model_create(sr_model** out, const sr_model_config* cfg) {
    SR_REQUIRE(out && cfg, "sr_model_create: null argument");
    const sr_model_config& c = *cfg;
    SR_REQUIRE(c.vocab_size > 0 && c.hidden_size > 0 && c.intermediate_size > 0 && c.num_layers > 0,
               "sr_model_create: bad dimensions");
    SR_REQUIRE(c.num_heads > 0 && c.num_kv_heads > 0 && c.num_heads % c.num_kv_heads == 0,
               "sr_model_create: num_heads %d must be a multiple of num_kv_heads %d", c.num_heads, c.num_kv_heads);
    SR_REQUIRE(c.head_dim == 64 || c.head_dim == 128, "sr_model_create: head_dim %d not supported (64 or 128)", c.head_dim);
    SR_REQUIRE(c.hidden_size % 64 == 0 && c.intermediate_size % 64 == 0,
               "sr_model_create: hidden_size and intermediate_size must be multiples of 64");
    SR_REQUIRE(c.vocab_size % 16 == 0 || !c.has_lm_head, "sr_model_create: vocab_size must be a multiple of 16 for the sparse head");
    SR_REQUIRE(c.max_batch_tokens > 0 && c.max_batch_seqs > 0 && c.max_batch_seqs <= 65536, "sr_model_create: bad workspace sizes");
    SR_REQUIRE(c.fp32_planes == 0 || c.fp32_planes == 2 || c.fp32_planes == 3 || c.fp32_planes == SR_FP32_PLANES_F16,
               "sr_model_create: fp32_planes must be 0, 2, 3 or 16");
    SR_REQUIRE(c.attention_bias == 0 || c.attention_bias == 1, "sr_model_create: attention_bias must be 0 or 1");
    sr_model* m = new sr_model();
    m->cfg = c;
    m->Tm = (int)(ceil_div64(c.max_batch_tokens, 128) * 128);
    m->Bm = c.max_batch_seqs;
    m->max_pos = 8192;
    m->layers.resize(c.num_layers);
    const int64_t H = c.hidden_size, I = c.intermediate_size, V = c.vocab_size;
    const int64_t nq = (int64_t)c.num_heads * c.head_dim, nkv = (int64_t)c.num_kv_heads * c.head_dim;
    SR_ALLOC(m->embed, V * H * 4);
    if (c.has_lm_head) SR_ALLOC(m->lm_head, V * H * 2);
    const int64_t nsg = c.fp32_planes ? split_map_w(c.fp32_planes).n_seg : 0;
    const bool f16p = c.fp32_planes == SR_FP32_PLANES_F16;
    if (c.has_lm_head && nsg) SR_ALLOC(m->lm_head_s, V * H * 2 * nsg);
    if (c.has_lm_head && f16p) SR_ALLOC(m->lm_head_i, V * 4);
    if (f16p) {
        SR_ALLOC(m->lo_nz, (4 * (int64_t)c.num_layers + 1) * 4);
        (void)hipMemset(m->lo_nz, 0, (size_t)(4 * c.num_layers + 1) * 4);
    }
    SR_ALLOC(m->norm_w, H * 4);
    for (auto& l : m->layers) {
        SR_ALLOC(l.wqkv, (nq + 2 * nkv) * H * 2);
        SR_ALLOC(l.wo, H * nq * 2);
        SR_ALLOC(l.wgu, 2 * I * H * 2);
        SR_ALLOC(l.wdown, H * I * 2);
        if (nsg) {
            SR_ALLOC(l.wqkv_s, (nq + 2 * nkv) * H * 2 * nsg);
            SR_ALLOC(l.wo_s, H * nq * 2 * nsg);
            SR_ALLOC(l.wgu_s, 2 * I * H * 2 * nsg);
            SR_ALLOC(l.wdown_s, H * I * 2 * nsg);
        }
        if (f16p) {
            SR_ALLOC(l.wqkv_i, (nq + 2 * nkv) * 4);
            SR_ALLOC(l.wo_i, H * 4);
            SR_ALLOC(l.wgu_i, 2 * I * 4);
            SR_ALLOC(l.wdown_i, H * 4);
        }
        SR_ALLOC(l.ln1, H * 4);
        SR_ALLOC(l.ln2, H * 4);
        if (c.attention_bias) {
            SR_ALLOC(l.bqkv, (nq + 2 * nkv) * 4);
            SR_ALLOC(l.bqkv_r, (nq + 2 * nkv) * 4);
        }
    }
    SR_ALLOC(m->rope_cos, (int64_t)m->max_pos * (c.head_dim / 2) * 4);
    SR_ALLOC(m->rope_sin, (int64_t)m->max_pos * (c.head_dim / 2) * 4);
    const int64_t Tm = m->Tm;
    SR_ALLOC(m->x, Tm * H * 4);
    SR_ALLOC(m->xn, Tm * H * 2);
    SR_ALLOC(m->qkv, Tm * (nq + 2 * nkv) * 2);
    SR_ALLOC(m->attn, Tm * nq * 2);
    SR_ALLOC(m->act, Tm * I * 2);
    SR_ALLOC(m->delta, Tm * H * 2);
    SR_ALLOC(m->span_start, m->Bm * 4);
    SR_ALLOC(m->span_len, m->Bm * 4);
    SR_ALLOC(m->pool_start, m->Bm * 4);
    SR_ALLOC(m->row_len, m->Bm * 4);
    SR_ALLOC(m->cu, (m->Bm + 1) * 4);
    SR_ALLOC(m->tok_id, Tm * 4);
    SR_ALLOC(m->pos, Tm * 4);
    SR_ALLOC(m->seq_of, Tm * 4);
    SR_ALLOC(m->key_valid, Tm);
    if (hipHostMalloc((void**)&m->h_cu, (size_t)(2 * m->Bm + 2) * 4) != hipSuccess) {
        sr_set_error("sr_model_create: hipHostMalloc failed");
        model_free(m);
        delete m;
        return SR_ERR_NOMEM;
    }
    (void)hipMemset(m->xn, 0, (size_t)(Tm * H * 2));
    (void)hipMemset(m->attn, 0, (size_t)(Tm * nq * 2));
    (void)hipMemset(m->act, 0, (size_t)(Tm * I * 2));
    std::vector<float> cs, sn;
    rope_tables(c, m->max_pos, cs, sn);
    if (hipMemcpy(m->rope_cos, cs.data(), cs.size() * 4, hipMemcpyHostToDevice) != hipSuccess ||
        hipMemcpy(m->rope_sin, sn.data(), sn.size() * 4, hipMemcpyHostToDevice) != hipSuccess) {
        sr_set_error("sr_model_create: rope table upload failed");
        model_free(m);
        delete m;
        return SR_ERR_HIP;
    }
    *out = m;
    return SR_OK;
}

extern "C" int sr_model_destroy(sr_model* m) {
    if (!m) return SR_OK;
    model_free(m);
    m->order.release();
    delete m;
    return SR_OK;
}

static int convert_rows(const void* src, int dtype, int64_t rows, int64_t cols, bf16_t* dbf, float* df32, int64_t base,
                        int interleave, hipStream_t s, bf16_t* dsplit = nullptr, int planes = 0, float* w_inv = nullptr,
                        int* lo_nz = nullptr) {
    hipLaunchKernelGGL(convert_rows_kernel, dim3((unsigned)rows), dim3(256), 0, s, src, dtype, rows, cols, dbf, df32, base,
                       interleave);
    if (dsplit && planes == SR_FP32_PLANES_F16)
        hipLaunchKernelGGL(convert_rows_split_h_kernel, dim3((unsigned)rows), dim3(256), 0, s, src, dtype, rows, cols, dsplit, w_inv, base,
                           interleave, lo_nz);
    else if (dsplit && planes)
        hipLaunchKernelGGL(convert_rows_split_kernel, dim3((unsigned)rows), dim3(256), 0, s, src, dtype, rows, cols, dsplit, base,
                           interleave, split_map_w(planes));
    SR_CHECK_LAUNCH();
    return SR_OK;
}

extern "C" int sr_model_set_weight(sr_model* m, const char* name, const void* d_ptr, int dtype, int64_t rows, int64_t cols,
                                   sr_stream stream) {
    SR_REQUIRE(m && name && d_ptr, "sr_model_set_weight: null argument");
    SR_REQUIRE(dtype == SR_DTYPE_F32 || dtype == SR_DTYPE_BF16, "sr_model_set_weight: dtype %d not supported", dtype);
    hipStream_t s = (hipStream_t)stream;
    std::lock_guard<std::mutex> lock(m->mu);
    SR_REQUIRE(!m->finalized, "sr_model_set_weight: the model is already finalized; weights are fixed from then on");
    const sr_model_config& c = m->cfg;
    const int64_t H = c.hidden_size, I = c.intermediate_size, V = c.vocab_size;
    int* const lo_nz = m->lo_nz;
    auto lo_flag = [&](int64_t i) { return lo_nz ? lo_nz + i : nullptr; };
    const int64_t lo_lm = 4 * (int64_t)c.num_layers;
    const int64_t nq = (int64_t)c.num_heads * c.head_dim, nkv = (int64_t)c.num_kv_heads * c.head_dim;
    std::string n(name);
    auto shape_is = [&](int64_t r, int64_t cc) { return rows == r && cols == cc; };
#define SHAPE_REQ(r, cc) SR_REQUIRE(shape_is((r), (cc)), "sr_model_set_weight: %s has shape [%lld, %lld], expected [%lld, %lld]", name, (long long)rows, (long long)cols, (long long)(r), (long long)(cc))
    if (n == "model.embed_tokens.weight") {
        SHAPE_REQ(V, H);
        SR_TRY(convert_rows(d_ptr, dtype, V, H, (c.has_lm_head && c.tie_word_embeddings) ? m->lm_head : nullptr, m->embed, 0, 0, s,
                            (c.has_lm_head && c.tie_word_embeddings) ? m->lm_head_s : nullptr, c.fp32_planes, m->lm_head_i,
                            lo_flag(lo_lm)));
        m->have_embed = true;
        if (c.has_lm_head && c.tie_word_embeddings) m->have_lm_head = true;
        return SR_OK;
    }
    if (n == "lm_head.weight") {
        SR_REQUIRE(c.has_lm_head, "sr_model_set_weight: model was created without an lm_head");
        SHAPE_REQ(V, H);
        SR_TRY(convert_rows(d_ptr, dtype, V, H, m->lm_head, nullptr, 0, 0, s, m->lm_head_s, c.fp32_planes, m->lm_head_i, lo_flag(lo_lm)));
        m->have_lm_head = true;
        return SR_OK;
    }
    if (n == "model.norm.weight") {
        SHAPE_REQ(H, 1);
        SR_TRY(convert_rows(d_ptr, dtype, H, 1, nullptr, m->norm_w, 0, 0, s));
        m->have_norm = true;
        return SR_OK;
    }
    int li = -1;
    char rest[128] = {0};
    if (sscanf(name, "model.layers.%d.%127s", &li, rest) == 2 && li >= 0 && li < c.num_layers) {
        LayerW& l = m->layers[li];
        std::string r(rest);
        if (r == "self_attn.q_proj.weight") { SHAPE_REQ(nq, H); SR_TRY(convert_rows(d_ptr, dtype, nq, H, l.wqkv, nullptr, 0, 0, s, l.wqkv_s, c.fp32_planes, l.wqkv_i, lo_flag(4 * li + 0))); l.have |= 1; return SR_OK; }
        if (r == "self_attn.k_proj.weight") { SHAPE_REQ(nkv, H); SR_TRY(convert_rows(d_ptr, dtype, nkv, H, l.wqkv, nullptr, nq, 0, s, l.wqkv_s, c.fp32_planes, l.wqkv_i, lo_flag(4 * li + 0))); l.have |= 2; return SR_OK; }
        if (r == "self_attn.v_proj.weight") { SHAPE_REQ(nkv, H); SR_TRY(convert_rows(d_ptr, dtype, nkv, H, l.wqkv, nullptr, nq + nkv, 0, s, l.wqkv_s, c.fp32_planes, l.wqkv_i, lo_flag(4 * li + 0))); l.have |= 4; return SR_OK; }
        if (r == "self_attn.o_proj.weight") { SHAPE_REQ(H, nq); SR_TRY(convert_rows(d_ptr, dtype, H, nq, l.wo, nullptr, 0, 0, s, l.wo_s, c.fp32_planes, l.wo_i, lo_flag(4 * li + 1))); l.have |= 8; return SR_OK; }
        if (r == "mlp.gate_proj.weight") { SHAPE_REQ(I, H); SR_TRY(convert_rows(d_ptr, dtype, I, H, l.wgu, nullptr, 0, 1, s, l.wgu_s, c.fp32_planes, l.wgu_i, lo_flag(4 * li + 2))); l.have |= 16; return SR_OK; }
        if (r == "mlp.up_proj.weight") { SHAPE_REQ(I, H); SR_TRY(convert_rows(d_ptr, dtype, I, H, l.wgu, nullptr, 0, 2, s, l.wgu_s, c.fp32_planes, l.wgu_i, lo_flag(4 * li + 2))); l.have |= 32; return SR_OK; }
        if (r == "mlp.down_proj.weight") { SHAPE_REQ(H, I); SR_TRY(convert_rows(d_ptr, dtype, H, I, l.wdown, nullptr, 0, 0, s, l.wdown_s, c.fp32_planes, l.wdown_i, lo_flag(4 * li + 3))); l.have |= 64; return SR_OK; }
        if (c.attention_bias && (r == "self_attn.q_proj.bias" || r == "self_attn.k_proj.bias" || r == "self_attn.v_proj.bias")) {
            const int which = r[10] == 'q' ? 0 : (r[10] == 'k' ? 1 : 2);
            const int64_t n_b = which == 0 ? nq : nkv, base = which == 0 ? 0 : (which == 1 ? nq : nq + nkv);
            SHAPE_REQ(n_b, 1);
            hipLaunchKernelGGL(convert_bias_kernel, dim3((unsigned)ceil_div64(n_b, 256)), dim3(256), 0, s, d_ptr, dtype, n_b, l.bqkv + base,
                               l.bqkv_r + base);
            SR_CHECK_LAUNCH();
            l.have_bias |= 1u << which;
            return SR_OK;
        }
        if (r == "input_layernorm.weight") { SHAPE_REQ(H, 1); SR_TRY(convert_rows(d_ptr, dtype, H, 1, nullptr, l.ln1, 0, 0, s)); l.have |= 128; return SR_OK; }
        if (r == "post_attention_layernorm.weight") { SHAPE_REQ(H, 1); SR_TRY(convert_rows(d_ptr, dtype, H, 1, nullptr, l.ln2, 0, 0, s)); l.have |= 256; return SR_OK; }
    }
    sr_set_error("sr_model_set_weight: unknown tensor name '%s'", name);
    return SR_ERR_INVALID;
}

static int pack_f16_weights(bf16_t*& w, int& nseg, bool lo_nz, int64_t rows, int64_t K) {
    if (nseg == 2 || lo_nz) return SR_OK;
    bf16_t* p = nullptr;
    SR_CHECK_HIP(hipMalloc((void**)&p, (size_t)(rows * 2 * K * 2)));
    hipLaunchKernelGGL(pack_rows_2seg_kernel, dim3((unsigned)rows), dim3(256), 0, nullptr, w, p, K);
    hipError_t e = hipGetLastError();
    if (e == hipSuccess) e = hipDeviceSynchronize();
    if (e != hipSuccess) {
        (void)hipFree(p);
        sr_set_error("sr_model_finalize: re-packing a [%lld, %lld] weight matrix failed: %s", (long long)rows, (long long)K,
                     hipGetErrorString(e));
        return SR_ERR_HIP;
    }
    SR_CHECK_HIP(hipFree(w));
    w = p;
    nseg = 2;
    return SR_OK;
}

extern "C" int sr_model_finalize(sr_model* m) {
    SR_REQUIRE(m, "sr_model_finalize: null model");
    SR_REQUIRE(m->have_embed, "sr_model_finalize: model.embed_tokens.weight missing");
    SR_REQUIRE(m->have_norm, "sr_model_finalize: model.norm.weight missing");
    SR_REQUIRE(!m->cfg.has_lm_head || m->have_lm_head, "sr_model_finalize: lm_head.weight missing");
    for (int i = 0; i < m->cfg.num_layers; ++i)
        SR_REQUIRE(m->layers[i].have == 511, "sr_model_finalize: layer %d is missing tensors (mask 0x%x)", i, m->layers[i].have);
    if (m->cfg.attention_bias)
        for (int i = 0; i < m->cfg.num_layers; ++i)
            SR_REQUIRE(m->layers[i].have_bias == 7,
                       "sr_model_finalize: layer %d is missing self_attn.{q,k,v}_proj.bias (attention_bias = 1; mask 0x%x)", i,
                       m->layers[i].have_bias);
    SR_CHECK_HIP(hipDeviceSynchronize());
    if (m->cfg.fp32_planes == SR_FP32_PLANES_F16) {
        const sr_model_config& c = m->cfg;
        const int64_t H = c.hidden_size, I = c.intermediate_size, V = c.vocab_size;
        const int64_t nq = (int64_t)c.num_heads * c.head_dim, nkv = (int64_t)c.num_kv_heads * c.head_dim;
        std::vector<int> nz((size_t)(4 * c.num_layers + 1));
        SR_CHECK_HIP(hipMemcpy(nz.data(), m->lo_nz, nz.size() * 4, hipMemcpyDeviceToHost));
        const char* env_seg = sr_dev_getenv("SR_F16_WEIGHT_SEGS");
        if (!(env_seg && *env_seg == '3')) {
            for (int i = 0; i < c.num_layers; ++i) {
                LayerW& l = m->layers[i];
                SR_TRY(pack_f16_weights(l.wqkv_s, l.qkv_seg, nz[4 * i + 0] != 0, nq + 2 * nkv, H));
                SR_TRY(pack_f16_weights(l.wo_s, l.o_seg, nz[4 * i + 1] != 0, H, nq));
                SR_TRY(pack_f16_weights(l.wgu_s, l.gu_seg, nz[4 * i + 2] != 0, 2 * I, H));
                SR_TRY(pack_f16_weights(l.wdown_s, l.down_seg, nz[4 * i + 3] != 0, H, I));
            }
            if (c.has_lm_head) SR_TRY(pack_f16_weights(m->lm_head_s, m->lm_head_seg, nz[4 * c.num_layers] != 0, V, H));
        }
        const int ns = (int)(I < 256 ? I : 256);
        float* d_p = nullptr;
        SR_CHECK_HIP(hipMalloc((void**)&d_p, (size_t)(ns + 1) * 4));
        std::vector<float> p((size_t)ns + 1);
        auto decide = [&]() -> int {
            for (int i = 0; i < c.num_layers; ++i) {
                LayerW& l = m->layers[i];
                if (!l.gu_cmax) SR_CHECK_HIP(hipMalloc((void**)&l.gu_cmax, 4));
                SR_TRY(launch_gu_cmax(l.wgu_s, l.wgu_i, (int)I, (int)H, l.gu_seg, l.gu_cmax, nullptr));
                SR_CHECK_HIP(hipMemsetAsync(d_p, 0, (size_t)ns * 4, nullptr));
                for (int k = 0; k < ns; ++k) {
                    const int64_t j = (int64_t)k * I / ns, row = (j / 16) * 32 + j % 16;
                    hipLaunchKernelGGL(gu_cmax_kernel, dim3(1), dim3(256), 0, nullptr, l.wgu_s + row * l.gu_seg * H, l.wgu_i + row, 1, (int)H,
                                       l.gu_seg, d_p + k);
                }
                SR_CHECK_LAUNCH();
                SR_CHECK_HIP(hipMemcpyAsync(d_p + ns, l.gu_cmax, 4, hipMemcpyDeviceToDevice, nullptr));
                SR_CHECK_HIP(hipMemcpy(p.data(), d_p, (size_t)(ns + 1) * 4, hipMemcpyDeviceToHost));
                const float cmax = p[(size_t)ns];
                std::nth_element(p.begin(), p.begin() + ns / 2, p.begin() + ns);
                const float med = p[(size_t)(ns / 2)];
                l.fused_act = !(cmax > 0.f) || (float)H * cmax < 65536.f * med;
            }
            return SR_OK;
        };
        const int rc = decide();
        (void)hipFree(d_p);
        SR_TRY(rc);
    }
    SR_CHECK_HIP(hipDeviceSynchronize());
    m->finalized = true;
    return SR_OK;
}

extern "C" int sr_model_weight_segments(sr_model* m, int32_t* out, int64_t capacity, int64_t* n) {
    SR_REQUIRE(m && n, "sr_model_weight_segments: null argument");
    SR_REQUIRE(m->finalized, "sr_model_weight_segments: sr_model_finalize was not called");
    const sr_model_config& c = m->cfg;
    std::vector<int32_t> v;
    const bool f16p = c.fp32_planes == SR_FP32_PLANES_F16;
    const int32_t plain = c.fp32_planes ? split_map_w(c.fp32_planes).n_seg : 0;
    for (const LayerW& l : m->layers) {
        v.push_back(f16p ? l.qkv_seg : plain); v.push_back(f16p ? l.o_seg : plain);
        v.push_back(f16p ? l.gu_seg : plain); v.push_back(f16p ? l.down_seg : plain);
    }
    if (c.has_lm_head) v.push_back(f16p ? m->lm_head_seg : plain);
    *n = (int64_t)v.size();
    SR_REQUIRE(capacity >= 0 && (capacity == 0 || out), "sr_model_weight_segments: bad output buffer");
    for (int64_t i = 0; i < capacity && i < (int64_t)v.size(); ++i) out[i] = v[(size_t)i];
    return SR_OK;
}

extern "C" int sr_model_fused_act_layers(sr_model* m, int32_t* out, int64_t capacity, int64_t* n) {
    SR_REQUIRE(m && n, "sr_model_fused_act_layers: null argument");
    SR_REQUIRE(m->finalized, "sr_model_fused_act_layers: sr_model_finalize was not called");
    const bool f16p = m->cfg.fp32_planes == SR_FP32_PLANES_F16;
    *n = f16p ? (int64_t)m->layers.size() : 0;
    SR_REQUIRE(capacity >= 0 && (capacity == 0 || out), "sr_model_fused_act_layers: bad output buffer");
    for (int64_t i = 0; i < capacity && i < *n; ++i) out[i] = m->layers[(size_t)i].fused_act ? 1 : 0;
    return SR_OK;
}

enum { PREC_BF16 = 0, PREC_FP32 = 1 };

static int ensure_fp32_workspace(sr_model* m) {
    if (m->xs) return SR_OK;
    const sr_model_config& c = m->cfg;
    SR_REQUIRE(c.fp32_planes > 0, "encode(fp32): the model was created with fp32_planes = 0 (bf16 regime only)");
    const int64_t Tm = m->Tm, H = c.hidden_size, I = c.intermediate_size;
    const int64_t nq = (int64_t)c.num_heads * c.head_dim, nkv = (int64_t)c.num_kv_heads * c.head_dim;
    const int64_t nsg = split_map_a(c.fp32_planes).n_seg;
    auto A = [&](void** p, int64_t bytes) {
        if (hipMalloc(p, (size_t)bytes) != hipSuccess) { *p = nullptr; return false; }
        return hipMemset(*p, 0, (size_t)bytes) == hipSuccess;
    };
    const bool f16p = c.fp32_planes == SR_FP32_PLANES_F16;
    bool ok = A((void**)&m->xs, Tm * H * 2 * nsg) && A((void**)&m->qkv_f, Tm * (nq + 2 * nkv) * 4) &&
              A((void**)&m->attn_s, Tm * nq * 2 * nsg) && A((void**)&m->act_s, Tm * I * 2 * nsg);
    if (ok && f16p)
        ok = A((void**)&m->attn_f, Tm * nq * 4) && A((void**)&m->act_f, Tm * I * 4) && A((void**)&m->xs_i, Tm * 4) &&
             A((void**)&m->attn_i, Tm * 4) && A((void**)&m->act_i, Tm * 4) && A((void**)&m->act_sc, Tm * 4);
    if (!ok) {
        auto F = [](void* p) { if (p) (void)hipFree(p); };
        F(m->xs); F(m->qkv_f); F(m->attn_s); F(m->act_s); F(m->attn_f); F(m->act_f); F(m->xs_i); F(m->attn_i); F(m->act_i);
        m->xs = nullptr; m->qkv_f = nullptr; m->attn_s = nullptr; m->act_s = nullptr;
        m->attn_f = nullptr; m->act_f = nullptr; m->xs_i = nullptr; m->attn_i = nullptr; m->act_i = nullptr;
        sr_set_error("encode(fp32): hipMalloc of the fp32-regime workspace failed (%lld tokens)", (long long)Tm);
        return SR_ERR_NOMEM;
    }
    return SR_OK;
}

static int launch_rmsnorm_split(float* x, const float* embed, const int* tok_id, const float* w, bf16_t* xs, int T, int H,
                                float eps, const SplitMap& map, hipStream_t s) {
    if (T == 0) return SR_OK;
    hipLaunchKernelGGL(rmsnorm_split_kernel, dim3((unsigned)ceil_div64(T, 4)), dim3(256), 0, s, x, embed, tok_id, w, xs, T, H, eps,
                       map);
    SR_CHECK_LAUNCH();
    return SR_OK;
}

static int model_forward(sr_model* m, const int64_t* d_ids, const int64_t* d_mask, int B, int L, int mode, int prec,
                         hipStream_t s, int* T_out, const int32_t* d_shift = nullptr) {
    const sr_model_config& c = m->cfg;
    SR_REQUIRE(m->finalized, "encode: sr_model_finalize was not called");
    SR_REQUIRE(B >= 1 && L >= 1, "encode: bad batch shape [%d, %d]", B, L);
    SR_REQUIRE(B <= m->Bm, "encode: batch of %d sequences exceeds max_batch_seqs %d", B, m->Bm);
    SR_REQUIRE(L <= m->max_pos, "encode: sequence length %d exceeds %d", L, m->max_pos);
    SR_REQUIRE(d_ids && d_mask, "encode: null input");
    if (prec == PREC_FP32) SR_TRY(ensure_fp32_workspace(m));
    const int H = c.hidden_size, I = c.intermediate_size;
    const int nq = c.num_heads * c.head_dim, nkv = c.num_kv_heads * c.head_dim;

    SR_TRY(launch_plan_rows(d_mask, B, L, mode, m->span_start, m->span_len, m->pool_start, m->row_len, d_shift, m->cu, s));
    SR_CHECK_HIP(hipMemcpyAsync(m->h_cu, m->cu, (size_t)(B + 1) * 4, hipMemcpyDeviceToHost, s));
    SR_CHECK_HIP(hipStreamSynchronize(s));
    const int T = m->h_cu[B];
    int max_len = 0;
    int attn_class[4] = {0, 0, 0, 0};
    for (int b = 0; b < B; ++b) {
        const int len = m->h_cu[b + 1] - m->h_cu[b];
        max_len = len > max_len ? len : max_len;
        if (len >= 1 && len <= 64) ++attn_class[(len - 1) >> 4];
    }
    SR_REQUIRE(T <= m->Tm, "encode: batch packs to %d tokens, workspace holds %d (raise max_batch_tokens or split the batch)", T, m->Tm);
    *T_out = T;
    m->last_T = T;
    if (T == 0) return SR_OK;
    SR_TRY(launch_plan_tokens(d_ids, d_mask, B, L, m->span_start, m->cu, m->tok_id, m->pos, m->key_valid, m->seq_of, c.vocab_size, mode,
                              d_shift, s));

    if (prec == PREC_FP32 && c.fp32_planes == SR_FP32_PLANES_F16) {
        auto split_rows = [&](float* src, const float* embed, const int* tok, const float* w, bf16_t* dst, float* inv, int K, int nseg) {
            launch_rows_split_h(src, embed, tok, w, dst, inv, T, K, c.rms_norm_eps, nseg, s);
        };
        const char* env_fa = sr_dev_getenv("SR_FP32_FUSED_ACT");
        const bool fused_on = !(env_fa && *env_fa == '0'), fused_all = env_fa && *env_fa == '1';
        for (int li = 0; li < c.num_layers; ++li) {
            LayerW& l = m->layers[li];
            const bool fused_act = fused_on && l.gu_cmax && (l.fused_act || fused_all);
            split_rows(m->x, li == 0 ? m->embed : (const float*)nullptr, li == 0 ? m->tok_id : (const int*)nullptr, l.ln1, m->xs, m->xs_i, H,
                       l.qkv_seg);
            GemmArgs g{};
            g.A = m->xs; g.W = l.wqkv_s; g.M = T; g.N = nq + 2 * nkv; g.K = l.qkv_seg * H; g.a_nseg = l.qkv_seg; g.C = m->qkv_f; g.a_scale = m->xs_i; g.w_scale = l.wqkv_i;
            g.pos = m->pos; g.rope_cos = m->rope_cos; g.rope_sin = m->rope_sin; g.n_rope = nq + nkv; g.head_dim = c.head_dim;
            g.bias = l.bqkv;
            SR_TRY(launch_gemm_bf16(EPI_QKV_ROPE_F32_H, g, s));
            AttnF32Args a{};
            a.qkv = m->qkv_f; a.out_f32 = m->attn_f; a.out = nullptr; a.cu_seqlens = m->cu; a.key_valid = m->key_valid;
            a.B = B; a.nh = c.num_heads; a.nkv = c.num_kv_heads; a.hd = c.head_dim;
            a.scale = 1.0f / sqrtf((float)c.head_dim); a.max_seqlen = max_len;
            a.have_classes = 1;
            for (int n = 0; n < 4; ++n) a.class_seqs[n] = attn_class[n];
            SR_TRY(launch_attention_f32(a, s));
            split_rows(m->attn_f, nullptr, nullptr, nullptr, m->attn_s, m->attn_i, nq, l.o_seg);
            g = GemmArgs{};
            g.A = m->attn_s; g.W = l.wo_s; g.M = T; g.N = H; g.K = l.o_seg * nq; g.a_nseg = l.o_seg; g.C = m->x; g.a_scale = m->attn_i; g.w_scale = l.wo_i;
            SR_TRY(launch_gemm_bf16(EPI_RESID_F32_H, g, s));
            if (fused_act) {
                launch_rows_split_h(m->x, nullptr, nullptr, l.ln2, m->xs, m->xs_i, T, H, c.rms_norm_eps, l.gu_seg, s, l.gu_cmax, m->act_sc,
                                    m->act_i);
                g = GemmArgs{};
                g.A = m->xs; g.W = l.wgu_s; g.M = T; g.N = 2 * I; g.K = l.gu_seg * H; g.a_nseg = l.gu_seg; g.C = m->act_s; g.a_scale = m->xs_i; g.w_scale = l.wgu_i;
                g.out_scale = m->act_sc; g.out_nseg = l.down_seg;
                SR_TRY(launch_gemm_bf16(EPI_SWIGLU_SPLIT_H, g, s));
            } else {
                split_rows(m->x, nullptr, nullptr, l.ln2, m->xs, m->xs_i, H, l.gu_seg);
                g = GemmArgs{};
                g.A = m->xs; g.W = l.wgu_s; g.M = T; g.N = 2 * I; g.K = l.gu_seg * H; g.a_nseg = l.gu_seg; g.C = m->act_f; g.a_scale = m->xs_i; g.w_scale = l.wgu_i;
                SR_TRY(launch_gemm_bf16(EPI_SWIGLU_F32_H, g, s));
                split_rows(m->act_f, nullptr, nullptr, nullptr, m->act_s, m->act_i, I, l.down_seg);
            }
            g = GemmArgs{};
            g.A = m->act_s; g.W = l.wdown_s; g.M = T; g.N = H; g.K = l.down_seg * I; g.a_nseg = l.down_seg; g.C = m->x; g.a_scale = m->act_i; g.w_scale = l.wdown_i;
            SR_TRY(launch_gemm_bf16(EPI_RESID_F32_H, g, s));
        }
        SR_CHECK_LAUNCH();
        return SR_OK;
    }
    if (prec == PREC_FP32) {
        const SplitMap ma = split_map_a(c.fp32_planes);
        const int nsg = ma.n_seg;
        for (int li = 0; li < c.num_layers; ++li) {
            LayerW& l = m->layers[li];
            SR_TRY(launch_rmsnorm_split(m->x, li == 0 ? m->embed : (const float*)nullptr, li == 0 ? m->tok_id : (const int*)nullptr,
                                        l.ln1, m->xs, T, H, c.rms_norm_eps, ma, s));
            GemmArgs g{};
            g.A = m->xs; g.W = l.wqkv_s; g.M = T; g.N = nq + 2 * nkv; g.K = nsg * H; g.C = m->qkv_f;
            g.pos = m->pos; g.rope_cos = m->rope_cos; g.rope_sin = m->rope_sin; g.n_rope = nq + nkv; g.head_dim = c.head_dim;
            g.bias = l.bqkv;
            SR_TRY(launch_gemm_bf16(EPI_QKV_ROPE_F32, g, s));
            AttnF32Args a{};
            a.qkv = m->qkv_f; a.out = m->attn_s; a.cu_seqlens = m->cu; a.key_valid = m->key_valid;
            a.B = B; a.nh = c.num_heads; a.nkv = c.num_kv_heads; a.hd = c.head_dim;
            a.scale = 1.0f / sqrtf((float)c.head_dim); a.max_seqlen = max_len; a.out_map = ma;
            a.have_classes = 1;
            for (int n = 0; n < 4; ++n) a.class_seqs[n] = attn_class[n];
            SR_TRY(launch_attention_f32(a, s));
            g = GemmArgs{};
            g.A = m->attn_s; g.W = l.wo_s; g.M = T; g.N = H; g.K = nsg * nq; g.C = m->x;
            SR_TRY(launch_gemm_bf16(EPI_RESID_F32, g, s));
            SR_TRY(launch_rmsnorm_split(m->x, (const float*)nullptr, (const int*)nullptr, l.ln2, m->xs, T, H, c.rms_norm_eps, ma, s));
            g = GemmArgs{};
            g.A = m->xs; g.W = l.wgu_s; g.M = T; g.N = 2 * I; g.K = nsg * H; g.C = m->act_s; g.out_map = ma;
            SR_TRY(launch_gemm_bf16(EPI_SWIGLU_SPLIT, g, s));
            g = GemmArgs{};
            g.A = m->act_s; g.W = l.wdown_s; g.M = T; g.N = H; g.K = nsg * I; g.C = m->x;
            SR_TRY(launch_gemm_bf16(EPI_RESID_F32, g, s));
        }
        return SR_OK;
    }

    SR_TRY(launch_rmsnorm(m->x, m->embed, m->tok_id, (const bf16_t*)nullptr, m->layers[0].ln1, m->xn,
                       (float*)nullptr, T, H, c.rms_norm_eps, s));
    for (int li = 0; li < c.num_layers; ++li) {
        LayerW& l = m->layers[li];
        if (li > 0) {
            SR_TRY(launch_rmsnorm(m->x, (const float*)nullptr, (const int*)nullptr,
                               (const bf16_t*)m->delta, l.ln1, m->xn, (float*)nullptr, T, H, c.rms_norm_eps, s));
        }
        GemmArgs g{};
        g.A = m->xn; g.W = l.wqkv; g.M = T; g.N = nq + 2 * nkv; g.K = H; g.C = m->qkv;
        g.pos = m->pos; g.rope_cos = m->rope_cos; g.rope_sin = m->rope_sin; g.n_rope = nq + nkv; g.head_dim = c.head_dim;
        g.bias = l.bqkv_r;
        SR_TRY(launch_gemm_bf16(EPI_QKV_ROPE, g, s));
        AttnArgs a{};
        a.qkv = m->qkv; a.out = m->attn; a.cu_seqlens = m->cu; a.pos = m->pos; a.key_valid = m->key_valid;
        a.rope_cos = m->rope_cos; a.rope_sin = m->rope_sin; a.B = B; a.nh = c.num_heads; a.nkv = c.num_kv_heads;
        a.hd = c.head_dim; a.scale = 1.0f / sqrtf((float)c.head_dim);
        a.apply_rope = 0; a.max_seqlen = max_len;
        SR_TRY(launch_attention(a, s));
        g = GemmArgs{};
        g.A = m->attn; g.W = l.wo; g.M = T; g.N = H; g.K = nq; g.C = m->delta;
        SR_TRY(launch_gemm_bf16(EPI_STORE_BF16, g, s));
        SR_TRY(launch_rmsnorm(m->x, (const float*)nullptr, (const int*)nullptr,
                           (const bf16_t*)m->delta, l.ln2, m->xn, (float*)nullptr, T, H, c.rms_norm_eps, s));
        g = GemmArgs{};
        g.A = m->xn; g.W = l.wgu; g.M = T; g.N = 2 * I; g.K = H; g.C = m->act;
        SR_TRY(launch_gemm_bf16(EPI_SWIGLU, g, s));
        g = GemmArgs{};
        g.A = m->act; g.W = l.wdown; g.M = T; g.N = H; g.K = I; g.C = m->delta;
        SR_TRY(launch_gemm_bf16(EPI_STORE_BF16, g, s));
    }
    SR_TRY(launch_rmsnorm(m->x, (const float*)nullptr, (const int*)nullptr,
                       (const bf16_t*)m->delta, (const float*)nullptr, (bf16_t*)nullptr, (float*)nullptr, T, H, c.rms_norm_eps, s));
    return SR_OK;
}

static int head_dense(sr_model* m, int B, int T, int prec, float* d_out, hipStream_t s) {
    const int H = m->cfg.hidden_size;
    if (T == 0) {
        SR_CHECK_HIP(hipMemsetAsync(d_out, 0, (size_t)B * H * 4, s));
        return SR_OK;
    }
    float2* stats = reinterpret_cast<float2*>(prec == PREC_FP32 ? (void*)m->xs : (void*)m->xn);
    return launch_dense_head(m->x, m->norm_w, stats, m->cu, m->pos, m->pool_start, d_out, B, T, H, m->cfg.rms_norm_eps, s);
}

static int head_sparse(sr_model* m, int B, int T, int prec, float* d_out, hipStream_t s) {
    const int H = m->cfg.hidden_size, V = m->cfg.vocab_size;
    SR_CHECK_HIP(hipMemsetAsync(d_out, 0, (size_t)B * V * 4, s));
    if (T == 0) return SR_OK;
    GemmArgs g{};
    GemmEpilogue epi = EPI_SEGMAX;
    if (prec == PREC_FP32 && m->cfg.fp32_planes == SR_FP32_PLANES_F16) {
        launch_rows_split_h(m->x, (const float*)nullptr, (const int*)nullptr, (const float*)m->norm_w, m->xs, m->xs_i, T, H,
                            m->cfg.rms_norm_eps, m->lm_head_seg, s);
        g.A = m->xs; g.W = m->lm_head_s; g.K = m->lm_head_seg * H; g.a_nseg = m->lm_head_seg; g.a_scale = m->xs_i; g.w_scale = m->lm_head_i;
        epi = EPI_SEGMAX_H;
    } else if (prec == PREC_FP32) {
        const SplitMap ma = split_map_a(m->cfg.fp32_planes);
        SR_TRY(launch_rmsnorm_split(m->x, (const float*)nullptr, (const int*)nullptr, m->norm_w, m->xs, T, H, m->cfg.rms_norm_eps,
                                    ma, s));
        g.A = m->xs; g.W = m->lm_head_s; g.K = ma.n_seg * H;
    } else {
        SR_TRY(launch_rmsnorm(m->x, (const float*)nullptr,
                           (const int*)nullptr, (const bf16_t*)nullptr, m->norm_w, m->xn, (float*)nullptr, T, H, m->cfg.rms_norm_eps, s));
        g.A = m->xn; g.W = m->lm_head; g.K = H;
    }
    g.M = T; g.N = V; g.C = d_out; g.seq_of = m->seq_of; g.out_ld = V;
    SR_TRY(launch_gemm_bf16(epi, g, s));
    const int64_t n = (int64_t)B * V;
    return launch_sparse_finish(d_out, n, powf((float)H, -0.25f), prec == PREC_FP32 ? 0 : 1, s);
}

static int encode_any(sr_model* m, const int64_t* d_input_ids, const int64_t* d_attention_mask, int32_t B, int32_t L, int mode,
                      int prec, float* d_dense, float* d_sparse, hipStream_t s, const int32_t* d_shift = nullptr) {
    std::lock_guard<std::mutex> lock(m->mu);
    StreamOrder::Scope in_order(m->order, s);
    int T = 0;
    SR_TRY(model_forward(m, d_input_ids, d_attention_mask, B, L, mode, prec, s, &T, d_shift));
    if (mode != 1) SR_TRY(head_dense(m, B, T, prec, d_dense, s));
    if (mode != 0) SR_TRY(head_sparse(m, B, T, prec, d_sparse, s));
    return SR_OK;
}

static int encode_dense(sr_model* m, const int64_t* d_input_ids, const int64_t* d_attention_mask, int32_t B, int32_t L, int prec,
                        float* d_out, hipStream_t s) {
    return encode_any(m, d_input_ids, d_attention_mask, B, L, 0, prec, d_out, nullptr, s);
}

static int encode_sparse(sr_model* m, const int64_t* d_input_ids, const int64_t* d_attention_mask, int32_t B, int32_t L, int prec,
                         float* d_out, hipStream_t s) {
    return encode_any(m, d_input_ids, d_attention_mask, B, L, 1, prec, nullptr, d_out, s);
}

extern "C" int sr_encode_dense(sr_model* m, const int64_t* d_input_ids, const int64_t* d_attention_mask, int32_t B, int32_t L,
                               float* d_out, sr_stream stream) {
    SR_REQUIRE(m && d_out, "sr_encode_dense: null argument");
    return encode_dense(m, d_input_ids, d_attention_mask, B, L, PREC_BF16, d_out, (hipStream_t)stream);
}

extern "C" int sr_encode_dense_fp32(sr_model* m, const int64_t* d_input_ids, const int64_t* d_attention_mask, int32_t B, int32_t L,
                                    float* d_out, sr_stream stream) {
    SR_REQUIRE(m && d_out, "sr_encode_dense_fp32: null argument");
    return encode_dense(m, d_input_ids, d_attention_mask, B, L, PREC_FP32, d_out, (hipStream_t)stream);
}

extern "C" int sr_encode_sparse(sr_model* m, const int64_t* d_input_ids, const int64_t* d_attention_mask, int32_t B, int32_t L,
                                float* d_out, sr_stream stream) {
    SR_REQUIRE(m && d_out, "sr_encode_sparse: null argument");
    SR_REQUIRE(m->cfg.has_lm_head, "sr_encode_sparse: model was created without an lm_head (LlamaBiModel)");
    return encode_sparse(m, d_input_ids, d_attention_mask, B, L, PREC_BF16, d_out, (hipStream_t)stream);
}

extern "C" int sr_encode_sparse_fp32(sr_model* m, const int64_t* d_input_ids, const int64_t* d_attention_mask, int32_t B, int32_t L,
                                     float* d_out, sr_stream stream) {
    SR_REQUIRE(m && d_out, "sr_encode_sparse_fp32: null argument");
    SR_REQUIRE(m->cfg.has_lm_head, "sr_encode_sparse_fp32: model was created without an lm_head (LlamaBiModel)");
    return encode_sparse(m, d_input_ids, d_attention_mask, B, L, PREC_FP32, d_out, (hipStream_t)stream);
}

extern "C" int sr_encode_both(sr_model* m, const int64_t* d_input_ids, const int64_t* d_attention_mask, int32_t B, int32_t L,
                              int32_t fp32, float* d_out_sparse, float* d_out_dense, sr_stream stream) {
    SR_REQUIRE(m && d_out_sparse && d_out_dense, "sr_encode_both: null argument");
    SR_REQUIRE(m->cfg.has_lm_head, "sr_encode_both: model was created without an lm_head (LlamaBiModel)");
    return encode_any(m, d_input_ids, d_attention_mask, B, L, 2, fp32 ? PREC_FP32 : PREC_BF16, d_out_dense, d_out_sparse,
                      (hipStream_t)stream);
}

extern "C" int sr_encode_rows(sr_model* m, const int64_t* d_input_ids, const int64_t* d_attention_mask, int32_t B, int32_t L,
                              const int32_t* d_row_shift, int32_t mode, int32_t fp32, float* d_out_sparse, float* d_out_dense,
                              sr_stream stream) {
    SR_REQUIRE(m, "sr_encode_rows: null model");
    SR_REQUIRE(mode >= 0 && mode <= 2, "sr_encode_rows: mode %d (0 dense, 1 sparse, 2 both)", mode);
    SR_REQUIRE(mode == 1 || d_out_dense, "sr_encode_rows: null dense output");
    SR_REQUIRE(mode == 0 || d_out_sparse, "sr_encode_rows: null sparse output");
    SR_REQUIRE(mode == 0 || m->cfg.has_lm_head, "sr_encode_rows: model was created without an lm_head (LlamaBiModel)");
    return encode_any(m, d_input_ids, d_attention_mask, B, L, mode, fp32 ? PREC_FP32 : PREC_BF16, d_out_dense, d_out_sparse,
                      (hipStream_t)stream, d_row_shift);
}

extern "C" int sr_model_last_hidden(sr_model* m, float* d_out, int64_t capacity_rows, int64_t* n_tokens, sr_stream stream) {
    SR_REQUIRE(m && d_out && n_tokens, "sr_model_last_hidden: null argument");
    hipStream_t s = (hipStream_t)stream;
    std::lock_guard<std::mutex> lock(m->mu);
    StreamOrder::Scope in_order(m->order, s);
    const int T = m->last_T;
    *n_tokens = T;
    SR_REQUIRE(capacity_rows >= T, "sr_model_last_hidden: capacity %lld < %d tokens", (long long)capacity_rows, T);
    if (T == 0) return SR_OK;
    SR_TRY(launch_rmsnorm(m->x, (const float*)nullptr,
                       (const int*)nullptr, (const bf16_t*)nullptr, m->norm_w, (bf16_t*)nullptr, d_out, T, m->cfg.hidden_size, m->cfg.rms_norm_eps, s));
    return SR_OK;
}

extern "C" int sr_lora_merge(float* d_W, const float* d_A, const float* d_B, int64_t out_features, int64_t in_features,
                             int32_t r, float scale, sr_stream stream) {
    SR_REQUIRE(d_W && d_A && d_B && out_features > 0 && in_features > 0 && r > 0, "sr_lora_merge: bad argument");
    SR_REQUIRE(out_features < 65536 * 32, "sr_lora_merge: out_features too large");
    hipLaunchKernelGGL(lora_merge_kernel, dim3((unsigned)ceil_div64(in_features, 256), (unsigned)out_features), dim3(256), 0,
                       (hipStream_t)stream, d_W, d_A, d_B, out_features, in_features, r, scale);
    SR_CHECK_LAUNCH();
    return SR_OK;
}

extern "C" int sr_sparse_compact(const float* d_reps, int64_t B, int64_t V, int64_t* d_row_ptr, int32_t* d_cols, float* d_vals,
                                 int64_t capacity, int64_t* h_nnz, sr_stream stream) {
    SR_REQUIRE(d_reps && d_row_ptr && h_nnz && B >= 0 && V > 0, "sr_sparse_compact: bad argument");
    hipStream_t s = (hipStream_t)stream;
    if (B == 0) { *h_nnz = 0; return SR_OK; }
    int64_t* d_cnt = nullptr;
    SR_CHECK_HIP(hipMalloc((void**)&d_cnt, (size_t)B * 8));
    hipLaunchKernelGGL(nnz_count_kernel, dim3((unsigned)B), dim3(256), 0, s, d_reps, V, d_cnt);
    hipLaunchKernelGGL(nnz_scan_kernel, dim3(1), dim3(64), 0, s, d_cnt, B, d_row_ptr);
    int64_t total = 0;
    hipError_t e = hipMemcpyAsync(&total, d_row_ptr + B, 8, hipMemcpyDeviceToHost, s);
    if (e == hipSuccess) e = hipStreamSynchronize(s);
    (void)hipFree(d_cnt);
    SR_CHECK_HIP(e);
    *h_nnz = total;
    if (total > capacity || (total > 0 && (!d_cols || !d_vals))) {
        sr_set_error("sr_sparse_compact: %lld non-zeros, capacity %lld", (long long)total, (long long)capacity);
        return SR_ERR_NOMEM;
    }
    if (total > 0) {
        hipLaunchKernelGGL(nnz_fill_kernel, dim3((unsigned)B), dim3(256), 0, s, d_reps, V, d_row_ptr, d_cols, d_vals, capacity);
        SR_CHECK_LAUNCH();
    }
    return SR_OK;
}
```

scaling_retriever_amd/csrc/kernels.h:

```cpp
#pragma once
#include "common.h"

typedef unsigned short bf16_t;

enum GemmEpilogue {
    EPI_STORE_BF16 = 0,
    EPI_RESID_F32 = 1,
    EPI_SWIGLU = 2,
    EPI_SEGMAX = 3,
    EPI_STORE_F32 = 4,
    EPI_QKV_ROPE = 5,
    EPI_QKV_ROPE_F32 = 6,
    EPI_SWIGLU_SPLIT = 7,
    EPI_SWIGLU_F32 = 8,
    EPI_H_FIRST = 9,
    EPI_QKV_ROPE_F32_H = 9, EPI_RESID_F32_H = 10, EPI_SWIGLU_F32_H = 11, EPI_SEGMAX_H = 12,
    EPI_SWIGLU_SPLIT_H = 13,
    EPI_SWIGLU_SPLITH_BASE = 14,
};

#define SR_MAX_SEG 6
struct SplitMap {
    int n_seg;
    int plane[SR_MAX_SEG];
};
#define SR_FP32_PLANES_F16 16
inline SplitMap split_map_a(int planes) {
    if (planes == 3) return SplitMap{6, {2, 0, 1, 1, 0, 0}};
    return SplitMap{3, {1, 0, 0, 0, 0, 0}};
}
inline SplitMap split_map_w(int planes) {
    if (planes == 3) return SplitMap{6, {0, 2, 1, 0, 1, 0}};
    return SplitMap{3, {0, 1, 0, 0, 0, 0}};
}

struct GemmArgs {
    const bf16_t* A;
    const bf16_t* W;
    int M, N, K;
    void* C;
    const int* seq_of;
    int64_t out_ld;
    const int* pos;
    const float* rope_cos;
    const float* rope_sin;
    int n_rope;
    int head_dim;
    const float* bias;
    unsigned long long* stamps;
    const float* a_scale;
    const float* w_scale;
    const float* out_scale;
    int a_nseg;
    int out_nseg;
    SplitMap out_map;
    int m_fastest;
    int xcd_order;
};

int launch_gemm_bf16(GemmEpilogue epi, const GemmArgs& g, hipStream_t s);

int launch_rows_split_f16(float* x, const float* embed, const int* tok, const float* w, bf16_t* xs, float* inv, int T, int K, float eps,
                          int nseg, const float* gu_cmax, float* act_sc, float* act_inv, hipStream_t s);
int launch_gu_cmax(const bf16_t* wgu_s, const float* wgu_i, int I, int K, int nseg, float* cmax, hipStream_t s);

int launch_rmsnorm(float* x, const float* embed, const int* tok_id, const bf16_t* delta, const float* w, bf16_t* xn, float* xn_f32, int T,
                   int H, float eps, hipStream_t s);
int launch_plan_rows(const int64_t* mask, int B, int L, int mode, int* span_start, int* span_len, int* pool_start, int* row_len,
                     const int* row_shift, int* cu, hipStream_t s);
int launch_plan_tokens(const int64_t* ids, const int64_t* mask, int B, int L, const int* span_start, const int* cu, int* tok_id, int* pos,
                       unsigned char* key_valid, int* seq_of, int vocab, int mode, const int* row_shift, hipStream_t s);
int launch_dense_head(const float* x, const float* w, float2* stats, const int* cu, const int* pos, const int* pool_start, float* out,
                      int B, int T, int H, float eps, hipStream_t s);
int launch_sparse_finish(float* out, int64_t n, float scale, int round_bf16, hipStream_t s);

struct AttnArgs {
    const bf16_t* qkv;
    bf16_t* out;
    const int* cu_seqlens;
    const int* pos;
    const unsigned char* key_valid;
    const float* rope_cos;
    const float* rope_sin;
    int B, nh, nkv, hd;
    float scale;
    int apply_rope;
    int max_seqlen;
};
int launch_attention(const AttnArgs& a, hipStream_t s);

struct AttnF32Args {
    const float* qkv;
    float* out_f32;
    bf16_t* out;
    const int* cu_seqlens;
    const unsigned char* key_valid;
    int B, nh, nkv, hd;
    float scale;
    int max_seqlen;
    SplitMap out_map;
    int only_le = 0, only_gt = 0;
    int have_classes = 0, class_seqs[4] = {0, 0, 0, 0};
    int nkb_only = 0;
};
int launch_attention_f32(const AttnF32Args& a, hipStream_t s);
```

Before: 16120.

## Fuse fp16 plane split into fp32 attention and group sequences by length class

```diff
diff --git a/include/sr_hip.h b/include/sr_hip.h
--- a/include/sr_hip.h
+++ b/include/sr_hip.h
@@ -202,6 +202,9 @@
 int sr_attention_varlen_f32(const float* d_qkv, float* d_out_f32, void* d_out_planes, int32_t fp32_planes,
                             const int32_t* d_cu_seqlens, const uint8_t* d_key_valid, int32_t B, int32_t num_heads,
                             int32_t num_kv_heads, int32_t head_dim, int32_t max_seqlen, sr_stream stream);
+int sr_attention_f32_split_f16(const float* d_qkv, const int32_t* d_cu_seqlens, const uint8_t* d_key_valid, int32_t B,
+                               int32_t num_heads, int32_t num_kv_heads, int32_t head_dim, int32_t max_seqlen, int32_t nseg,
+                               void* d_planes, float* d_a_inv, float* d_out_f32_other_rows, sr_stream stream);
 int sr_rmsnorm_bf16(float* d_x, const float* d_embed, const int32_t* d_tok_id, const void* d_delta, const float* d_norm_w,
                     void* d_xn, float* d_xn_f32, float eps, int32_t T, int32_t H, sr_stream stream);
 int sr_dense_head_pool(const float* d_x, const float* d_norm_w, const int32_t* d_cu_seqlens, const int32_t* d_pos,
diff --git a/scaling_retriever_amd/_lib.py b/scaling_retriever_amd/_lib.py
--- a/scaling_retriever_amd/_lib.py
+++ b/scaling_retriever_amd/_lib.py
@@ -123,6 +123,8 @@
                                     c_int32, c_int32, c_int32, c_void_p]),
     "sr_attention_varlen_f32": (c_int, [c_void_p, c_void_p, c_void_p, c_int32, c_void_p, c_void_p, c_int32, c_int32, c_int32,
                                         c_int32, c_int32, c_void_p]),
+    "sr_attention_f32_split_f16": (c_int, [c_void_p, c_void_p, c_void_p, c_int32, c_int32, c_int32, c_int32, c_int32, c_int32,
+                                           c_void_p, c_void_p, c_void_p, c_void_p]),
     "sr_sparse_compact": (c_int, [c_void_p, c_int64, c_int64, c_void_p, c_void_p, c_void_p, c_int64,
                                   ctypes.POINTER(c_int64), c_void_p]),
     "sr_sparse_compact_topm": (c_int, [c_void_p, c_int64, c_int64, c_int64, c_void_p, c_void_p, c_void_p, c_int64,
@@ -137,7 +139,7 @@
     pass
 
 
-def _bind(path):
+def _bind(path, strict=True):
     if not os.path.exists(path):
         raise SrHipError(
             f"{path} not found: the HIP extension is not built. There is no CPU fallback; "
@@ -145,6 +147,8 @@
     import torch
     lib = ctypes.CDLL(path)
     for name, (res, args) in SIGNATURES.items():
+        if not strict and not hasattr(lib, name):
+            continue
         fn = getattr(lib, name)
         fn.restype = res
         fn.argtypes = args
@@ -162,7 +166,7 @@
 @contextlib.contextmanager
 def library(path):
     global _lib
-    other = _bind(os.path.abspath(path))
+    other = _bind(os.path.abspath(path), strict=False)
     with _lock:
         keep, _lib = _lib, other
     try:
diff --git a/scaling_retriever_amd/csrc/api.hip b/scaling_retriever_amd/csrc/api.hip
--- a/scaling_retriever_amd/csrc/api.hip
+++ b/scaling_retriever_amd/csrc/api.hip
@@ -103,6 +103,46 @@
     a.scale = 1.0f / sqrtf((float)head_dim); a.max_seqlen = max_seqlen;
     if (!d_out_f32) a.out_map = split_map_a(fp32_planes);
     return launch_attention_f32(a, (hipStream_t)stream);
+}
+
+extern "C" int sr_attention_f32_split_f16(const float* d_qkv, const int32_t* d_cu_seqlens, const uint8_t* d_key_valid, int32_t B,
+                                          int32_t num_heads, int32_t num_kv_heads, int32_t head_dim, int32_t max_seqlen, int32_t nseg,
+                                          void* d_planes, float* d_a_inv, float* d_out_f32_other_rows, sr_stream stream) {
+    SR_REQUIRE(d_qkv && d_cu_seqlens && d_key_valid && d_planes && d_a_inv && d_out_f32_other_rows, "sr_attention_f32_split_f16: null pointer");
+    SR_REQUIRE(B >= 0 && max_seqlen >= 0 && num_heads > 0 && num_kv_heads > 0 && head_dim > 0, "sr_attention_f32_split_f16: bad sizes");
+    SR_REQUIRE(num_heads % num_kv_heads == 0, "sr_attention_f32_split_f16: num_heads %d not a multiple of num_kv_heads %d", num_heads, num_kv_heads);
+    SR_REQUIRE(head_dim == 64 || head_dim == 128, "sr_attention_f32_split_f16: head_dim %d not supported (64 or 128)", head_dim);
+    SR_REQUIRE(nseg == 2 || nseg == 3, "sr_attention_f32_split_f16: nseg %d is not 2 or 3", nseg);
+    SR_REQUIRE((uintptr_t)d_qkv % 16 == 0 && (uintptr_t)d_out_f32_other_rows % 16 == 0 && (uintptr_t)d_planes % 8 == 0,
+               "sr_attention_f32_split_f16: d_qkv and d_out_f32_other_rows must be 16-byte aligned, d_planes 8-byte aligned");
+    if (B == 0) return SR_OK;
+    hipStream_t s = (hipStream_t)stream;
+    std::vector<int> cu((size_t)B + 1);
+    SR_CHECK_HIP(hipMemcpyAsync(cu.data(), d_cu_seqlens, sizeof(int) * ((size_t)B + 1), hipMemcpyDeviceToHost, s));
+    SR_CHECK_HIP(hipStreamSynchronize(s));
+    std::vector<int2> list((size_t)B);
+    AttnF32Args a{};
+    const int max_len = af_fill_seq_list(cu.data(), B, list.data(), a.list_off, a.class_seqs);
+    SR_REQUIRE(max_len <= max_seqlen, "sr_attention_f32_split_f16: a sequence of %d tokens, max_seqlen %d", max_len, max_seqlen);
+    const int T = cu[B];
+    if (T <= 0 || max_len <= 0) return SR_OK;
+    int2* d_list = nullptr;
+    SR_CHECK_HIP(hipMalloc((void**)&d_list, sizeof(int2) * (size_t)B));
+    int rc = SR_OK;
+    if (hipMemcpyAsync(d_list, list.data(), sizeof(int2) * (size_t)a.list_off[5], hipMemcpyHostToDevice, s) != hipSuccess) {
+        sr_set_error("sr_attention_f32_split_f16: upload of the sequence list failed");
+        rc = SR_ERR_HIP;
+    } else {
+        a.qkv = d_qkv; a.out_f32 = d_out_f32_other_rows; a.out = nullptr; a.cu_seqlens = d_cu_seqlens; a.key_valid = d_key_valid;
+        a.B = B; a.nh = num_heads; a.nkv = num_kv_heads; a.hd = head_dim;
+        a.scale = 1.0f / sqrtf((float)head_dim); a.max_seqlen = max_len;
+        a.have_classes = 1;
+        a.seq_list = d_list;
+        rc = launch_attention_f32_split_f16(a, (bf16_t*)d_planes, d_a_inv, T, nseg, s);
+    }
+    (void)hipStreamSynchronize(s);
+    (void)hipFree(d_list);
+    return rc;
 }
 
 extern "C" int sr_gemm_f16_scaled(const void* d_A, const void* d_W, int32_t M, int32_t N, int32_t K, const float* d_a_scale,
diff --git a/scaling_retriever_amd/csrc/attention_f32.hip b/scaling_retriever_amd/csrc/attention_f32.hip
--- a/scaling_retriever_amd/csrc/attention_f32.hip
+++ b/scaling_retriever_amd/csrc/attention_f32.hip
@@ -8,6 +8,17 @@
 __device__ inline float af_mul_rn(float a, float b) {
 #pragma clang fp contract(off)
     return a * b;
+}
+
+__device__ __forceinline__ void af_sequence(const AttnF32Args& a, int& t0, int& S) {
+    if (a.seq_list) {
+        const int2 e = a.seq_list[a.list_base + blockIdx.x];
+        t0 = e.x;
+        S = e.y;
+    } else {
+        t0 = a.cu_seqlens[blockIdx.x];
+        S = a.cu_seqlens[blockIdx.x + 1] - t0;
+    }
 }
 
 template <int HD>
@@ -17,10 +28,10 @@
     __shared__ float qs[AF_ROWS][HD];
     __shared__ float ps[AF_ROWS][AF_KC];
     __shared__ unsigned char kval[AF_KC];
-    const int b = blockIdx.x, h = blockIdx.y;
+    const int h = blockIdx.y;
     const int tid = threadIdx.x, lane = tid & 63, wave = tid >> 6;
-    const int t0 = a.cu_seqlens[b];
-    const int S = a.cu_seqlens[b + 1] - t0;
+    int t0, S;
+    af_sequence(a, t0, S);
     const int r0 = blockIdx.z * AF_ROWS;
     if (r0 >= S || S <= a.only_gt) return;
     const int G = a.nh / a.nkv, kvh = h / G;
@@ -113,11 +124,11 @@
     __shared__ float qs[G][HD];
     __shared__ float ps[G][AF_KC];
     __shared__ unsigned char kval[AF_KC];
-    const int b = blockIdx.x, kvh = blockIdx.y;
+    const int kvh = blockIdx.y;
     const int tid = threadIdx.x, lane = tid & 63, wave = tid >> 6;
     const int h = kvh * G + wave;
-    const int t0 = a.cu_seqlens[b];
-    const int S = a.cu_seqlens[b + 1] - t0;
+    int t0, S;
+    af_sequence(a, t0, S);
     const int r0 = blockIdx.z * AF_ROWS;
     if (r0 >= S || S <= a.only_gt) return;
     const int ld = (a.nh + 2 * a.nkv) * HD;
@@ -224,22 +235,73 @@
     af_swap16(x2, x3);
     x = f32x4{x0, x1, x2, x3};
 }
-__device__ __forceinline__ float af_quad_xor(float v, int sel) {
-    return sel == 0x4E ? __int_as_float(__builtin_amdgcn_mov_dpp(__float_as_int(v), 0x4E, 0xF, 0xF, true))
-                       : __int_as_float(__builtin_amdgcn_mov_dpp(__float_as_int(v), 0xB1, 0xF, 0xF, true));
-}
-__device__ __forceinline__ void af_transpose_quad(f32x4& x, int i) {
-    float x0 = x[0], x1 = x[1], x2 = x[2], x3 = x[3];
-    const bool hi2 = (i & 2) != 0, hi1 = (i & 1) != 0;
-    const float r0 = af_quad_xor(hi2 ? x0 : x2, 0x4E), r1 = af_quad_xor(hi2 ? x1 : x3, 0x4E);
-    if (hi2) { x0 = r0; x1 = r1; } else { x2 = r0; x3 = r1; }
-    const float s0 = af_quad_xor(hi1 ? x0 : x1, 0xB1), s1 = af_quad_xor(hi1 ? x2 : x3, 0xB1);
-    if (hi1) { x0 = s0; x2 = s1; } else { x1 = s0; x3 = s1; }
-    x = f32x4{x0, x1, x2, x3};
-}
-
 __host__ __device__ constexpr int af_mfma_waves(int hd, int nkb) {
-    return nkb == 0 ? 1 : (hd == 64 ? (nkb == 1 ? 8 : 6) : (nkb <= 2 ? 5 : 4));
+    return nkb == 0 ? (hd == 64 ? 6 : 1) : (hd == 64 ? (nkb == 1 ? 8 : 6) : (nkb <= 2 ? 5 : 4));
+}
+
+template <int HD, int MKB, bool OLD, class NextQ, class Store>
+__device__ __forceinline__ void af_mfma_qblock(const float* Ks, const float* Vs, f32x4 (&qv)[HD / 16], unsigned vmask, int nkb, float scale,
+                                               int g, int c, NextQ&& next_q, Store&& store) {
+    constexpr int LDK = HD + 1, CB = HD / 16;
+    f32x4 st[MKB];
+#pragma unroll
+    for (int kb = 0; kb < MKB; ++kb) {
+        st[kb] = f32x4{0.f, 0.f, 0.f, 0.f};
+        if (kb < nkb) {
+#pragma unroll
+            for (int kk = 0; kk < HD / 4; ++kk)
+                st[kb] = __builtin_amdgcn_mfma_f32_16x16x4f32(Ks[(16 * kb + c) * LDK + 4 * kk + g], qv[kk >> 2][kk & 3], st[kb], 0, 0, 0);
+        }
+    }
+    if constexpr (!OLD) {
+        __builtin_amdgcn_sched_barrier(0);
+        next_q();
+    }
+    float m = -INFINITY;
+#pragma unroll
+    for (int kb = 0; kb < MKB; ++kb)
+#pragma unroll
+        for (int r = 0; r < 4; ++r) {
+            const bool v = (vmask >> (4 * kb + r)) & 1;
+            st[kb][r] = v ? st[kb][r] * scale : -INFINITY;
+            m = fmaxf(m, st[kb][r]);
+        }
+    m = fmaxf(m, __shfl_xor(m, 16));
+    m = fmaxf(m, __shfl_xor(m, 32));
+    float sum = 0.f;
+#pragma unroll
+    for (int kb = 0; kb < MKB; ++kb)
+#pragma unroll
+        for (int r = 0; r < 4; ++r) {
+            const float p = (m > -INFINITY && st[kb][r] > -INFINITY) ? expf(st[kb][r] - m) : 0.f;
+            st[kb][r] = p;
+            sum += p;
+        }
+    sum += __shfl_xor(sum, 16);
+    sum += __shfl_xor(sum, 32);
+    const float inv = sum > 0.f ? 1.0f / sum : 0.f;
+#pragma unroll
+    for (int kb = 0; kb < MKB; ++kb)
+#pragma unroll
+        for (int r = 0; r < 4; ++r) st[kb][r] *= inv;
+    if constexpr (!OLD) __builtin_amdgcn_sched_barrier(0);
+#pragma unroll
+    for (int cb = 0; cb < CB; ++cb) {
+        if (!OLD && cb == 4) __builtin_amdgcn_sched_barrier(0);
+        f32x4 o = {0.f, 0.f, 0.f, 0.f};
+#pragma unroll
+        for (int kb = 0; kb < MKB; ++kb) {
+            if (kb < nkb) {
+#pragma unroll
+                for (int mm = 0; mm < 4; ++mm) {
+                    const float v = Vs[(16 * kb + 4 * g + mm) * LDK + 16 * cb + c];
+                    o = OLD ? __builtin_amdgcn_mfma_f32_16x16x4f32(st[kb][mm], v, o, 0, 0, 0)
+                            : __builtin_amdgcn_mfma_f32_16x16x4f32(v, st[kb][mm], o, 0, 0, 0);
+                }
+            }
+        }
+        store(cb, o);
+    }
 }
 
 template <int HD, int NKB>
@@ -248,10 +310,10 @@
     constexpr bool OLD = NKB == 0;
     constexpr int MKB = OLD ? 4 : NKB;
     extern __shared__ float af_smem[];
-    const int b = blockIdx.x, kvh = blockIdx.y;
+    const int kvh = blockIdx.y;
     const int tid = threadIdx.x, lane = tid & 63, wave = tid >> 6;
-    const int t0 = a.cu_seqlens[b];
-    const int S = a.cu_seqlens[b + 1] - t0;
+    int t0, S;
+    af_sequence(a, t0, S);
     if (S <= 0 || S > a.only_le) return;
     const int nkb = (S + 15) >> 4;
     if (!OLD && (a.nkb_only ? nkb != a.nkb_only : nkb > NKB)) return;
@@ -329,7 +391,6 @@
     __syncthreads();
     const int64_t ldo = (int64_t)a.out_map.n_seg * a.nh * HD;
     for (int qb = 0; qb < nkb; ++qb) {
-        f32x4 st[MKB];
         if constexpr (OLD) {
             float* Qs = Vs + SP * LDK + wave * 16 * LDK;
             for (int i = lane; i < 16 * (HD / 4); i += 64) {
@@ -349,101 +410,158 @@
 #pragma unroll
             for (int i = 0; i < CB; ++i) af_transpose_groups(qv[i]);
         }
-#pragma unroll
-        for (int kb = 0; kb < MKB; ++kb) {
-            st[kb] = f32x4{0.f, 0.f, 0.f, 0.f};
-            if (kb < nkb) {
-#pragma unroll
-                for (int kk = 0; kk < HD / 4; ++kk)
-                    st[kb] = __builtin_amdgcn_mfma_f32_16x16x4f32(Ks[(16 * kb + c) * LDK + 4 * kk + g], qv[kk >> 2][kk & 3], st[kb], 0, 0, 0);
-            }
-        }
-        if constexpr (!OLD) {
-            __builtin_amdgcn_sched_barrier(0);
-            if (HD == 64 && qb + 1 < nkb) load_q(qb + 1);
-        }
-        float m = -INFINITY;
-#pragma unroll
-        for (int kb = 0; kb < MKB; ++kb)
-#pragma unroll
-            for (int r = 0; r < 4; ++r) {
-                const bool v = (vmask >> (4 * kb + r)) & 1;
-                st[kb][r] = v ? st[kb][r] * a.scale : -INFINITY;
-                m = fmaxf(m, st[kb][r]);
-            }
-        m = fmaxf(m, __shfl_xor(m, 16));
-        m = fmaxf(m, __shfl_xor(m, 32));
-        float sum = 0.f;
-#pragma unroll
-        for (int kb = 0; kb < MKB; ++kb)
-#pragma unroll
-            for (int r = 0; r < 4; ++r) {
-                const float p = (m > -INFINITY && st[kb][r] > -INFINITY) ? expf(st[kb][r] - m) : 0.f;
-                st[kb][r] = p;
-                sum += p;
-            }
-        sum += __shfl_xor(sum, 16);
-        sum += __shfl_xor(sum, 32);
-        const float inv = sum > 0.f ? 1.0f / sum : 0.f;
-#pragma unroll
-        for (int kb = 0; kb < MKB; ++kb)
-#pragma unroll
-            for (int r = 0; r < 4; ++r) st[kb][r] *= inv;
-        if constexpr (!OLD) __builtin_amdgcn_sched_barrier(0);
-#pragma unroll
-        for (int cb = 0; cb < CB; ++cb) {
-            if (!OLD && cb == 4) __builtin_amdgcn_sched_barrier(0);
-            f32x4 o = {0.f, 0.f, 0.f, 0.f};
-#pragma unroll
-            for (int kb = 0; kb < MKB; ++kb) {
-                if (kb < nkb) {
-#pragma unroll
-                    for (int mm = 0; mm < 4; ++mm)
-                        o = __builtin_amdgcn_mfma_f32_16x16x4f32(st[kb][mm], Vs[(16 * kb + 4 * g + mm) * LDK + 16 * cb + c], o, 0, 0, 0);
-                }
-            }
-            if constexpr (OLD) {
-#pragma unroll
-                for (int r = 0; r < 4; ++r) {
-                    const int row = 16 * qb + 4 * g + r;
-                    if (row >= S) continue;
-                    const int col = h * HD + 16 * cb + c;
+        af_mfma_qblock<HD, MKB, OLD>(
+            Ks, Vs, qv, vmask, nkb, a.scale, g, c,
+            [&]() { if (HD == 64 && qb + 1 < nkb) load_q(qb + 1); },
+            [&](int cb, f32x4 o) {
+                if constexpr (OLD) {
+#pragma unroll
+                    for (int r = 0; r < 4; ++r) {
+                        const int row = 16 * qb + 4 * g + r;
+                        if (row >= S) continue;
+                        const int col = h * HD + 16 * cb + c;
+                        if (a.out_f32) {
+                            a.out_f32[(int64_t)(t0 + row) * a.nh * HD + col] = o[r];
+                        } else {
+                            unsigned short p[3];
+                            split_bf16x3(o[r], p[0], p[1], p[2]);
+                            bf16_t* orow = a.out + (int64_t)(t0 + row) * ldo;
+                            for (int sg = 0; sg < a.out_map.n_seg; ++sg) orow[(int64_t)sg * a.nh * HD + col] = p[a.out_map.plane[sg]];
+                        }
+                    }
+                } else {
+                    const int row = 16 * qb + c;
+                    if (row >= S) return;
+                    const int col = h * HD + 16 * cb + 4 * g;
                     if (a.out_f32) {
-                        a.out_f32[(int64_t)(t0 + row) * a.nh * HD + col] = o[r];
+                        *reinterpret_cast<f32x4*>(a.out_f32 + (int64_t)(t0 + row) * a.nh * HD + col) = o;
                     } else {
-                        unsigned short p[3];
-                        split_bf16x3(o[r], p[0], p[1], p[2]);
+                        unsigned short p[4][3];
+#pragma unroll
+                        for (int e = 0; e < 4; ++e) split_bf16x3(o[e], p[e][0], p[e][1], p[e][2]);
                         bf16_t* orow = a.out + (int64_t)(t0 + row) * ldo;
-                        for (int sg = 0; sg < a.out_map.n_seg; ++sg) orow[(int64_t)sg * a.nh * HD + col] = p[a.out_map.plane[sg]];
+                        for (int sg = 0; sg < a.out_map.n_seg; ++sg) {
+                            const int pl = a.out_map.plane[sg];
+                            bf16x4 w;
+#pragma unroll
+                            for (int e = 0; e < 4; ++e) w[e] = (short)(pl == 0 ? p[e][0] : (pl == 1 ? p[e][1] : p[e][2]));
+                            *reinterpret_cast<bf16x4*>(orow + (int64_t)sg * a.nh * HD + col) = w;
+                        }
                     }
                 }
-            } else {
-                af_transpose_quad(o, c & 3);
-                const int row = 16 * qb + 4 * g + (c & 3);
-                if (row >= S) continue;
-                const int col = h * HD + 16 * cb + (c & 12);
-                if (a.out_f32) {
-                    *reinterpret_cast<f32x4*>(a.out_f32 + (int64_t)(t0 + row) * a.nh * HD + col) = o;
-                } else {
-                    unsigned short p[4][3];
-#pragma unroll
-                    for (int e = 0; e < 4; ++e) split_bf16x3(o[e], p[e][0], p[e][1], p[e][2]);
-                    bf16_t* orow = a.out + (int64_t)(t0 + row) * ldo;
-                    for (int sg = 0; sg < a.out_map.n_seg; ++sg) {
-                        const int pl = a.out_map.plane[sg];
-                        bf16x4 w;
-#pragma unroll
-                        for (int e = 0; e < 4; ++e) w[e] = (short)(pl == 0 ? p[e][0] : (pl == 1 ? p[e][1] : p[e][2]));
-                        *reinterpret_cast<bf16x4*>(orow + (int64_t)sg * a.nh * HD + col) = w;
-                    }
-                }
-            }
+            });
+    }
+}
+
+#define AFS_WAVES 16
+template <int HPW>
+__global__ __launch_bounds__(64 * AFS_WAVES, 8) void attention_f32_seq_split_kernel(AttnF32Args a) {
+    constexpr int HD = 64, LDK = HD + 1, CB = HD / 16, NT = 64 * AFS_WAVES;
+    extern __shared__ float af_smem[];
+    const int tid = threadIdx.x, lane = tid & 63, wave = tid >> 6;
+    const int2 ent = a.seq_list[a.list_base + blockIdx.x];
+    const int t0 = ent.x, S = ent.y;
+    const int G = a.nh / a.nkv;
+    const int ld = (a.nh + 2 * a.nkv) * HD;
+    const int g = lane >> 4, c = lane & 15;
+    float* red = af_smem + a.nkv * 2 * 16 * LDK;
+    f32x4 qv[CB];
+    const float* seq = a.qkv + (int64_t)t0 * ld;
+    const int qoff = c * ld + 4 * g;
+    auto load_q = [&](int h) {
+#pragma unroll
+        for (int i = 0; i < CB; ++i) {
+            qv[i] = f32x4{0.f, 0.f, 0.f, 0.f};
+            if (h < a.nh && c < S) qv[i] = *reinterpret_cast<const f32x4*>(seq + (qoff + h * HD + 16 * i));
+        }
+    };
+    const int lgP = __builtin_ctz(2 * a.nkv * (HD / 4)), kstep = NT >> lgP;
+    const int j = tid & ((1 << lgP) - 1), kq = tid >> lgP;
+    const int hv = j / (HD / 4);
+    const int koff = kq * ld + a.nh * HD + 4 * j;
+    float* dst = af_smem + ((hv < a.nkv ? 2 * hv : 2 * (hv - a.nkv) + 1) * 16 + kq) * LDK + (j % (HD / 4)) * 4;
+    unsigned vmask = 0;
+    {
+        f32x4 kv[4];
+#pragma unroll
+        for (int it = 0; it < 4; ++it) {
+            kv[it] = f32x4{0.f, 0.f, 0.f, 0.f};
+            if (kq + it * kstep < S) kv[it] = *reinterpret_cast<const f32x4*>(seq + (koff + it * kstep * ld));
+        }
+        load_q(wave);
+#pragma unroll
+        for (int r = 0; r < 4; ++r) {
+            const int key = 4 * g + r;
+            if (key < S && a.key_valid[t0 + key]) vmask |= 1u << r;
+        }
+#pragma unroll
+        for (int it = 0; it < 4; ++it) {
+            if (kq + it * kstep < 16) {
+#pragma unroll
+                for (int e = 0; e < 4; ++e) dst[it * kstep * LDK + e] = kv[it][e];
+            }
+        }
+    }
+    __syncthreads();
+    f32x4 oacc[HPW][CB];
+    float mx = 0.f;
+#pragma unroll
+    for (int hi = 0; hi < HPW; ++hi) {
+        const int h = wave + AFS_WAVES * hi;
+#pragma unroll
+        for (int cb = 0; cb < CB; ++cb) oacc[hi][cb] = f32x4{0.f, 0.f, 0.f, 0.f};
+        if (h >= a.nh) continue;
+        const float* Ks = af_smem + (h / G) * 2 * 16 * LDK;
+#pragma unroll
+        for (int i = 0; i < CB; ++i) af_transpose_groups(qv[i]);
+        af_mfma_qblock<HD, 1, false>(
+            Ks, Ks + 16 * LDK, qv, vmask, 1, a.scale, g, c,
+            [&]() { if (hi + 1 < HPW) load_q(h + AFS_WAVES); },
+            [&](int cb, f32x4 o) {
+                oacc[hi][cb] = o;
+#pragma unroll
+                for (int e = 0; e < 4; ++e) mx = fmaxf(mx, fabsf(o[e]));
+            });
+    }
+    mx = fmaxf(mx, __shfl_xor(mx, 16));
+    mx = fmaxf(mx, __shfl_xor(mx, 32));
+    const int row = c;
+    if (g == 0) red[row * AFS_WAVES + wave] = mx;
+    __syncthreads();
+#pragma unroll
+    for (int w4 = 0; w4 < AFS_WAVES / 4; ++w4) {
+        const f32x4 r = *reinterpret_cast<const f32x4*>(red + row * AFS_WAVES + 4 * w4);
+        mx = fmaxf(fmaxf(mx, fmaxf(r[0], r[1])), fmaxf(r[2], r[3]));
+    }
+    if (row >= S) return;
+    const float sc = row_scale_pow2(mx);
+    if (wave == 0 && g == 0) a.split_inv[t0 + row] = 1.0f / sc;
+    const int K = a.nh * HD;
+    bf16_t* obase = a.split_out + (int64_t)t0 * K * a.split_nseg;
+    const int ooff = row * K * a.split_nseg;
+#pragma unroll
+    for (int hi = 0; hi < HPW; ++hi) {
+        const int h = wave + AFS_WAVES * hi;
+        if (h >= a.nh) continue;
+#pragma unroll
+        for (int cb = 0; cb < CB; ++cb) {
+            bf16x4 p0, p1;
+#pragma unroll
+            for (int e = 0; e < 4; ++e) {
+                unsigned short f0, f1;
+                split_f16x2(oacc[hi][cb][e] * sc, f0, f1);
+                p0[e] = (short)f0; p1[e] = (short)f1;
+            }
+            const int col = h * HD + 16 * cb + 4 * g;
+            *reinterpret_cast<bf16x4*>(obase + (ooff + col)) = p1;
+            *reinterpret_cast<bf16x4*>(obase + (ooff + K + col)) = p0;
+            if (a.split_nseg == 3) *reinterpret_cast<bf16x4*>(obase + (ooff + 2 * K + col)) = p0;
         }
     }
 }
 
 template <int HD, int NKB>
-static int launch_attention_f32_mfma_cfg(const AttnF32Args& a, size_t lds, hipStream_t s) {
+static int launch_attention_f32_mfma_cfg(const AttnF32Args& a_in, size_t lds, hipStream_t s) {
     static DeviceOnce attr_once;
     if (bool* slot = attr_once.pending()) {
         constexpr int max_sp = NKB ? 16 * NKB : 64;
@@ -451,9 +569,42 @@
                                          hipFuncAttributeMaxDynamicSharedMemorySize, (int)(sizeof(float) * (2 * max_sp + (NKB ? 0 : 64)) * (HD + 1))));
         *slot = true;
     }
-    const dim3 grid((unsigned)a.B, (unsigned)a.nkv), block(256);
+    AttnF32Args a = a_in;
+    int n_seq = a.B;
+    if (a.seq_list) {
+        a.list_base = a.nkb_only ? a.list_off[a.nkb_only - 1] : 0;
+        n_seq = (a.nkb_only ? a.list_off[a.nkb_only] : a.list_off[4]) - a.list_base;
+        if (n_seq == 0) return SR_OK;
+    }
+    const dim3 grid((unsigned)n_seq, (unsigned)a.nkv), block(256);
     SR_REQUIRE(grid.y <= 65535, "attention(fp32): grid too large");
     hipLaunchKernelGGL((attention_f32_mfma_kernel<HD, NKB>), grid, block, lds, s, a);
+    SR_CHECK_LAUNCH();
+    return SR_OK;
+}
+
+static size_t af_seq_split_lds(int nkv) { return sizeof(float) * ((size_t)nkv * 2 * 16 * (64 + 1) + 16 * AFS_WAVES); }
+
+bool attention_f32_fused_split_eligible(const AttnF32Args& a) {
+    const char* env_m = sr_dev_getenv("SR_ATTN_F32_MFMA");
+    const char* env_l = sr_dev_getenv("SR_ATTN_F32_LAYOUT");
+    return a.hd == 64 && (a.nkv == 1 || a.nkv == 2 || a.nkv == 4 || a.nkv == 8) && a.nh == 4 * a.nkv && a.nh <= 2 * AFS_WAVES && !(env_m && *env_m == '0') && !(env_l && *env_l == '0') &&
+           a.seq_list && a.have_classes && a.class_seqs[0] > 0 &&
+           2 * af_seq_split_lds(a.nkv) <= 160 * 1024;
+}
+
+template <int HPW>
+static int launch_attention_f32_seq_split(const AttnF32Args& a_in, hipStream_t s) {
+    AttnF32Args a = a_in;
+    const size_t lds = af_seq_split_lds(a.nkv);
+    static DeviceOnce attr_once;
+    if (bool* slot = attr_once.pending()) {
+        SR_CHECK_HIP(hipFuncSetAttribute(reinterpret_cast<const void*>(&attention_f32_seq_split_kernel<HPW>),
+                                         hipFuncAttributeMaxDynamicSharedMemorySize, 80 * 1024));
+        *slot = true;
+    }
+    a.list_base = a.list_off[0];
+    hipLaunchKernelGGL((attention_f32_seq_split_kernel<HPW>), dim3((unsigned)(a.list_off[1] - a.list_off[0])), dim3(64 * AFS_WAVES), lds, s, a);
     SR_CHECK_LAUNCH();
     return SR_OK;
 }
@@ -470,29 +621,41 @@
 }
 
 template <int HD>
-static int launch_attention_f32_mfma(const AttnF32Args& a_in, hipStream_t s) {
+static int launch_attention_f32_mfma(const AttnF32Args& a_in, hipStream_t s, AttnF32Launched* rec) {
     AttnF32Args a = a_in;
     const int top = (int)ceil_div64(a.max_seqlen < 64 ? a.max_seqlen : 64, 16);
     const char* env = sr_dev_getenv("SR_ATTN_F32_LAYOUT");
     if (env && *env == '0') {
         const size_t lds = sizeof(float) * (size_t)(2 * 16 * top + 4 * 16) * (HD + 1);
+        a.nkb_only = 0;
+        if (rec) ++rec->class_launch[top - 1];
         return launch_attention_f32_mfma_cfg<HD, 0>(a, lds, s);
     }
     const bool force = env && *env == '2';
     if (!a.have_classes && !force) {
         a.nkb_only = 0;
+        if (rec) ++rec->class_launch[top - 1];
         return launch_attention_f32_mfma_class<HD>(a, top, s);
     }
     for (int nkb = 1; nkb <= top; ++nkb) {
         if (a.have_classes && a.class_seqs[nkb - 1] == 0) continue;
         a.nkb_only = nkb;
+        if (HD == 64 && nkb == 1 && a.split_out) {
+            if (rec) rec->fused_seqs = a.list_off[1] - a.list_off[0];
+            SR_TRY(a.nh <= AFS_WAVES ? launch_attention_f32_seq_split<1>(a, s) : launch_attention_f32_seq_split<2>(a, s));
+            continue;
+        }
+        if (rec) ++rec->class_launch[nkb - 1];
         SR_TRY(launch_attention_f32_mfma_class<HD>(a, nkb, s));
     }
     return SR_OK;
 }
 
-int launch_attention_f32(const AttnF32Args& a_in, hipStream_t s) {
+int launch_attention_f32(const AttnF32Args& a_in, hipStream_t s, AttnF32Launched* rec) {
     AttnF32Args a = a_in;
+    if (!a.have_classes) a.seq_list = nullptr;
+    SR_REQUIRE(!a.split_out || (attention_f32_fused_split_eligible(a) && a.split_inv && (a.split_nseg == 2 || a.split_nseg == 3)),
+               "attention(fp32): plane output of the whole-sequence kernel asked for where it cannot run");
     SR_REQUIRE(a.nh % a.nkv == 0, "attention(fp32): num_heads %d not a multiple of num_kv_heads %d", a.nh, a.nkv);
     SR_REQUIRE(a.out_f32 || (a.out_map.n_seg >= 1 && a.out_map.n_seg <= SR_MAX_SEG), "attention(fp32): bad segment map");
     if (a.B == 0 || a.max_seqlen <= 0) return SR_OK;
@@ -501,13 +664,20 @@
     const char* env_m = sr_dev_getenv("SR_ATTN_F32_MFMA");
     if (G == 4 && (a.hd == 64 || a.hd == 128) && !(env_m && *env_m == '0')) {
         a.only_le = 64;
-        SR_TRY(a.hd == 64 ? launch_attention_f32_mfma<64>(a, s) : launch_attention_f32_mfma<128>(a, s));
+        SR_TRY(a.hd == 64 ? launch_attention_f32_mfma<64>(a, s, rec) : launch_attention_f32_mfma<128>(a, s, rec));
         if (a.max_seqlen <= 64) return SR_OK;
         a.only_le = 0; a.only_gt = 64;
     }
+    int n_seq = a.B;
+    if (a.seq_list) {
+        a.list_base = a.only_gt ? a.list_off[4] : 0;
+        n_seq = a.list_off[5] - a.list_base;
+        if (n_seq == 0) return SR_OK;
+    }
+    if (rec) ++rec->long_launch;
     const char* env = sr_dev_getenv("SR_ATTN_F32_GQA");
     if (G == 4 && !(env && *env == '0')) {
-        const dim3 grid((unsigned)a.B, (unsigned)a.nkv, (unsigned)ceil_div64(a.max_seqlen, AF_ROWS)), block(256);
+        const dim3 grid((unsigned)n_seq, (unsigned)a.nkv, (unsigned)ceil_div64(a.max_seqlen, AF_ROWS)), block(256);
         SR_REQUIRE(grid.y <= 65535 && grid.z <= 65535, "attention(fp32): grid too large");
         switch (a.hd) {
             case 64: hipLaunchKernelGGL((attention_f32_gqa_kernel<64, 4>), grid, block, 0, s, a); break;
@@ -517,7 +687,7 @@
         SR_CHECK_LAUNCH();
         return SR_OK;
     }
-    const dim3 grid((unsigned)a.B, (unsigned)a.nh, (unsigned)ceil_div64(a.max_seqlen, AF_ROWS)), block(256);
+    const dim3 grid((unsigned)n_seq, (unsigned)a.nh, (unsigned)ceil_div64(a.max_seqlen, AF_ROWS)), block(256);
     SR_REQUIRE(grid.y <= 65535 && grid.z <= 65535, "attention(fp32): grid too large");
     switch (a.hd) {
         case 64: hipLaunchKernelGGL(attention_f32_kernel<64>, grid, block, 0, s, a); break;
@@ -527,3 +697,22 @@
     SR_CHECK_LAUNCH();
     return SR_OK;
 }
+
+int af_fill_seq_list(const int* h_cu, int B, int2* h_list, int off[6], int class_seqs[4]) {
+    int cnt[5] = {0, 0, 0, 0, 0}, max_len = 0;
+    auto group = [](int len) { return len <= 64 ? (len - 1) >> 4 : 4; };
+    for (int b = 0; b < B; ++b) {
+        const int len = h_cu[b + 1] - h_cu[b];
+        max_len = len > max_len ? len : max_len;
+        if (len >= 1) ++cnt[group(len)];
+    }
+    off[0] = 0;
+    for (int n = 0; n < 5; ++n) off[n + 1] = off[n] + cnt[n];
+    for (int n = 0; n < 4; ++n) class_seqs[n] = cnt[n];
+    int at[5] = {off[0], off[1], off[2], off[3], off[4]};
+    for (int b = 0; b < B; ++b) {
+        const int len = h_cu[b + 1] - h_cu[b];
+        if (len >= 1) h_list[at[group(len)]++] = make_int2(h_cu[b], len);
+    }
+    return max_len;
+}
diff --git a/scaling_retriever_amd/csrc/encoder.hip b/scaling_retriever_amd/csrc/encoder.hip
--- a/scaling_retriever_amd/csrc/encoder.hip
+++ b/scaling_retriever_amd/csrc/encoder.hip
@@ -380,14 +380,25 @@
     }
 }
 
+__device__ __forceinline__ int rows_split_row(const int2* __restrict__ seqs, int T) {
+    const int wave = threadIdx.x >> 6;
+    if (seqs) {
+        const int2 e = seqs[blockIdx.x];
+        const int r = blockIdx.y * 4 + wave;
+        return r < e.y ? e.x + r : -1;
+    }
+    const int t = blockIdx.x * 4 + wave;
+    return t < T ? t : -1;
+}
+
 __global__ __launch_bounds__(256) void rows_split_h_kernel(float* __restrict__ x, const float* __restrict__ embed,
                                                            const int* __restrict__ tok_id, const float* __restrict__ w,
                                                            bf16_t* __restrict__ xs, float* __restrict__ a_inv, int T, int K, float eps,
                                                            const float* __restrict__ gu_cmax, float* __restrict__ act_sc,
-                                                           float* __restrict__ act_inv, int nseg) {
-    const int t = blockIdx.x * 4 + (threadIdx.x >> 6);
+                                                           float* __restrict__ act_inv, int nseg, const int2* __restrict__ seqs) {
     const int lane = threadIdx.x & 63;
-    if (t >= T) return;
+    const int t = rows_split_row(seqs, T);
+    if (t < 0) return;
     float* xr = x + (int64_t)t * K;
     const float* src = embed ? embed + (int64_t)tok_id[t] * K : xr;
     float rs = 1.f;
@@ -444,11 +455,11 @@
                                                                const int* __restrict__ tok_id, const float* __restrict__ w,
                                                                bf16_t* __restrict__ xs, float* __restrict__ a_inv, int T, float eps,
                                                                const float* __restrict__ gu_cmax, float* __restrict__ act_sc,
-                                                               float* __restrict__ act_inv, int nseg) {
+                                                               float* __restrict__ act_inv, int nseg, const int2* __restrict__ seqs) {
     constexpr int K = 256 * NV;
-    const int t = blockIdx.x * 4 + (threadIdx.x >> 6);
     const int lane = threadIdx.x & 63;
-    if (t >= T) return;
+    const int t = rows_split_row(seqs, T);
+    if (t < 0) return;
     float* xr = x + (int64_t)t * K;
     const float* src = embed ? embed + (int64_t)tok_id[t] * K : xr;
     f32x4 v[NV];
@@ -505,13 +516,13 @@
 
 static void launch_rows_split_h(float* x, const float* embed, const int* tok, const float* w, bf16_t* xs, float* inv, int T, int K,
                                 float eps, int nseg, hipStream_t s, const float* gu_cmax = nullptr, float* act_sc = nullptr,
-                                float* act_inv = nullptr) {
-    const dim3 grid((unsigned)ceil_div64(T, 4)), block(256);
+                                float* act_inv = nullptr, const int2* seqs = nullptr, int n_seqs = 0, int max_rows = 0) {
+    const dim3 grid = seqs ? dim3((unsigned)n_seqs, (unsigned)ceil_div64(max_rows, 4)) : dim3((unsigned)ceil_div64(T, 4)), block(256);
     switch (K) {
-        case 2048: hipLaunchKernelGGL(rows_split_h_reg_kernel<8>, grid, block, 0, s, x, embed, tok, w, xs, inv, T, eps, gu_cmax, act_sc, act_inv, nseg); break;
-        case 4096: hipLaunchKernelGGL(rows_split_h_reg_kernel<16>, grid, block, 0, s, x, embed, tok, w, xs, inv, T, eps, gu_cmax, act_sc, act_inv, nseg); break;
-        case 8192: hipLaunchKernelGGL(rows_split_h_reg_kernel<32>, grid, block, 0, s, x, embed, tok, w, xs, inv, T, eps, gu_cmax, act_sc, act_inv, nseg); break;
-        default: hipLaunchKernelGGL(rows_split_h_kernel, grid, block, 0, s, x, embed, tok, w, xs, inv, T, K, eps, gu_cmax, act_sc, act_inv, nseg);
+        case 2048: hipLaunchKernelGGL(rows_split_h_reg_kernel<8>, grid, block, 0, s, x, embed, tok, w, xs, inv, T, eps, gu_cmax, act_sc, act_inv, nseg, seqs); break;
+        case 4096: hipLaunchKernelGGL(rows_split_h_reg_kernel<16>, grid, block, 0, s, x, embed, tok, w, xs, inv, T, eps, gu_cmax, act_sc, act_inv, nseg, seqs); break;
+        case 8192: hipLaunchKernelGGL(rows_split_h_reg_kernel<32>, grid, block, 0, s, x, embed, tok, w, xs, inv, T, eps, gu_cmax, act_sc, act_inv, nseg, seqs); break;
+        default: hipLaunchKernelGGL(rows_split_h_kernel, grid, block, 0, s, x, embed, tok, w, xs, inv, T, K, eps, gu_cmax, act_sc, act_inv, nseg, seqs);
     }
 }
 
@@ -549,6 +560,36 @@
                           int nseg, const float* gu_cmax, float* act_sc, float* act_inv, hipStream_t s) {
     launch_rows_split_h(x, embed, tok, w, xs, inv, T, K, eps, nseg, s, gu_cmax, act_sc, act_inv);
     SR_CHECK_LAUNCH();
+    return SR_OK;
+}
+
+int launch_attention_f32_split_f16(const AttnF32Args& a_in, bf16_t* planes, float* a_inv, int T, int nseg, hipStream_t s) {
+    AttnF32Args a = a_in;
+    SR_REQUIRE(a.out_f32 && !a.out && !a.split_out, "attention + split (fp16 planes): the attention writes fp32 rows");
+    const int K = a.nh * a.hd;
+    const char* env = sr_dev_getenv("SR_ATTN_F32_FUSED_SPLIT");
+    const bool fused = !(env && *env == '0') && attention_f32_fused_split_eligible(a);
+    AttnF32Launched rec;
+    if (fused) { a.split_out = planes; a.split_inv = a_inv; a.split_nseg = nseg; }
+    SR_TRY(launch_attention_f32(a, s, &rec));
+    if (!fused) {
+        if (T > 0) {
+            launch_rows_split_h(a.out_f32, nullptr, nullptr, nullptr, planes, a_inv, T, K, 0.f, nseg, s);
+            rec.split_launch = 1;
+            rec.split_seqs = a.seq_list ? a.list_off[5] : a.B;
+        }
+    } else {
+        const int n_mid = a.list_off[4] - a.list_off[1], n_long = a.list_off[5] - a.list_off[4];
+        if (n_mid) launch_rows_split_h(a.out_f32, nullptr, nullptr, nullptr, planes, a_inv, T, K, 0.f, nseg, s, nullptr, nullptr, nullptr, a.seq_list + a.list_off[1], n_mid, 64);
+        if (n_long) launch_rows_split_h(a.out_f32, nullptr, nullptr, nullptr, planes, a_inv, T, K, 0.f, nseg, s, nullptr, nullptr, nullptr, a.seq_list + a.list_off[4], n_long, a.max_seqlen);
+        rec.split_launch = (n_mid != 0) + (n_long != 0);
+        rec.split_seqs = n_mid + n_long;
+    }
+    SR_CHECK_LAUNCH();
+    if (const char* e = getenv("SR_LOG")) if (atoi(e) >= 1)
+        fprintf(stderr, "sr attention(fp32) + split: whole-sequence kernel %d sequences; class launches %d %d %d %d; long launches %d; "
+                        "row-split launches %d over %d sequences\n", rec.fused_seqs, rec.class_launch[0], rec.class_launch[1],
+                rec.class_launch[2], rec.class_launch[3], rec.long_launch, rec.split_launch, rec.split_seqs);
     return SR_OK;
 }
 
@@ -654,6 +695,8 @@
     int *tok_id = nullptr, *pos = nullptr, *seq_of = nullptr;
     unsigned char* key_valid = nullptr;
     int* h_cu = nullptr;
+    int2* h_seq_list = nullptr;
+    int2* seq_list = nullptr;
     int last_T = 0;
     std::mutex mu;
     StreamOrder order;
@@ -672,6 +715,8 @@
     F(m->span_start); F(m->span_len); F(m->pool_start); F(m->row_len); F(m->cu);
     F(m->tok_id); F(m->pos); F(m->seq_of); F(m->key_valid);
     if (m->h_cu) (void)hipHostFree(m->h_cu);
+    if (m->h_seq_list) (void)hipHostFree(m->h_seq_list);
+    F(m->seq_list);
 }
 
 #define SR_ALLOC(ptr, bytes)                                                                      \
@@ -791,7 +836,9 @@
     SR_ALLOC(m->pos, Tm * 4);
     SR_ALLOC(m->seq_of, Tm * 4);
     SR_ALLOC(m->key_valid, Tm);
-    if (hipHostMalloc((void**)&m->h_cu, (size_t)(2 * m->Bm + 2) * 4) != hipSuccess) {
+    SR_ALLOC(m->seq_list, (m->Bm + 1) * sizeof(int2));
+    if (hipHostMalloc((void**)&m->h_cu, (size_t)(2 * m->Bm + 2) * 4) != hipSuccess ||
+        hipHostMalloc((void**)&m->h_seq_list, (size_t)(m->Bm + 1) * sizeof(int2)) != hipSuccess) {
         sr_set_error("sr_model_create: hipHostMalloc failed");
         model_free(m);
         delete m;
@@ -1070,16 +1117,13 @@
     SR_CHECK_HIP(hipStreamSynchronize(s));
     const int T = m->h_cu[B];
     int max_len = 0;
-    int attn_class[4] = {0, 0, 0, 0};
-    for (int b = 0; b < B; ++b) {
-        const int len = m->h_cu[b + 1] - m->h_cu[b];
-        max_len = len > max_len ? len : max_len;
-        if (len >= 1 && len <= 64) ++attn_class[(len - 1) >> 4];
-    }
+    int attn_class[4] = {0, 0, 0, 0}, attn_off[6];
+    max_len = af_fill_seq_list(m->h_cu, B, m->h_seq_list, attn_off, attn_class);
     SR_REQUIRE(T <= m->Tm, "encode: batch packs to %d tokens, workspace holds %d (raise max_batch_tokens or split the batch)", T, m->Tm);
     *T_out = T;
     m->last_T = T;
     if (T == 0) return SR_OK;
+    if (prec == PREC_FP32) SR_CHECK_HIP(hipMemcpyAsync(m->seq_list, m->h_seq_list, (size_t)attn_off[5] * sizeof(int2), hipMemcpyHostToDevice, s));
     SR_TRY(launch_plan_tokens(d_ids, d_mask, B, L, m->span_start, m->cu, m->tok_id, m->pos, m->key_valid, m->seq_of, c.vocab_size, mode,
                               d_shift, s));
 
@@ -1105,8 +1149,9 @@
             a.scale = 1.0f / sqrtf((float)c.head_dim); a.max_seqlen = max_len;
             a.have_classes = 1;
             for (int n = 0; n < 4; ++n) a.class_seqs[n] = attn_class[n];
-            SR_TRY(launch_attention_f32(a, s));
-            split_rows(m->attn_f, nullptr, nullptr, nullptr, m->attn_s, m->attn_i, nq, l.o_seg);
+            a.seq_list = m->seq_list;
+            for (int n = 0; n < 6; ++n) a.list_off[n] = attn_off[n];
+            SR_TRY(launch_attention_f32_split_f16(a, m->attn_s, m->attn_i, T, l.o_seg, s));
             g = GemmArgs{};
             g.A = m->attn_s; g.W = l.wo_s; g.M = T; g.N = H; g.K = l.o_seg * nq; g.a_nseg = l.o_seg; g.C = m->x; g.a_scale = m->attn_i; g.w_scale = l.wo_i;
             SR_TRY(launch_gemm_bf16(EPI_RESID_F32_H, g, s));
@@ -1149,6 +1194,8 @@
             a.scale = 1.0f / sqrtf((float)c.head_dim); a.max_seqlen = max_len; a.out_map = ma;
             a.have_classes = 1;
             for (int n = 0; n < 4; ++n) a.class_seqs[n] = attn_class[n];
+            a.seq_list = m->seq_list;
+            for (int n = 0; n < 6; ++n) a.list_off[n] = attn_off[n];
             SR_TRY(launch_attention_f32(a, s));
             g = GemmArgs{};
             g.A = m->attn_s; g.W = l.wo_s; g.M = T; g.N = H; g.K = nsg * nq; g.C = m->x;
diff --git a/scaling_retriever_amd/csrc/kernels.h b/scaling_retriever_amd/csrc/kernels.h
--- a/scaling_retriever_amd/csrc/kernels.h
+++ b/scaling_retriever_amd/csrc/kernels.h
@@ -102,5 +102,20 @@
     int only_le = 0, only_gt = 0;
     int have_classes = 0, class_seqs[4] = {0, 0, 0, 0};
     int nkb_only = 0;
+    const int2* seq_list = nullptr;
+    int list_off[6] = {0, 0, 0, 0, 0, 0};
+    int list_base = 0;
+    bf16_t* split_out = nullptr;
+    float* split_inv = nullptr;
+    int split_nseg = 0;
 };
-int launch_attention_f32(const AttnF32Args& a, hipStream_t s);
+struct AttnF32Launched {
+    int fused_seqs = 0;
+    int class_launch[4] = {0, 0, 0, 0};
+    int long_launch = 0;
+    int split_launch = 0, split_seqs = 0;
+};
+int launch_attention_f32(const AttnF32Args& a, hipStream_t s, AttnF32Launched* rec = nullptr);
+int af_fill_seq_list(const int* h_cu, int B, int2* h_list, int off[6], int class_seqs[4]);
+bool attention_f32_fused_split_eligible(const AttnF32Args& a);
+int launch_attention_f32_split_f16(const AttnF32Args& a, bf16_t* planes, float* a_inv, int T, int nseg, hipStream_t s);
```

Result: no change. 16130, median of 6 (+0.1%).
